# grantsrb/PyTorch-A2C

Measured on AMD Instinct MI355X. Metric: env-steps/sec (rollout+update), higher is better.
Workload: dtype f32

## Files before the change

### include/a2c_mi355x.h

```cpp
#ifndef A2C_MI355X_H
#define A2C_MI355X_H

#include <stddef.h>
#include <stdint.h>

#ifdef __cplusplus
extern "C" {
#endif

#define A2C_OK 0
#define A2C_ERR_ARG (-1)
#define A2C_ERR_LAUNCH (-2)
#define A2C_ERR_WORKSPACE (-3)

typedef void *a2c_stream_t;

int a2c_version(void);
const char *a2c_error_string(int code);

int a2c_discount_scan(const float *x, const float *dones, float *y, int64_t n_seg,
                      int64_t T, float g, int *err_flag, a2c_stream_t stream);
int a2c_gae_returns_fused(const float *deltas, const float *rewards, const float *dones,
                          float *advs, float *rets, int64_t n_seg, int64_t T, float g_adv,
                          float g_ret, int *err_flag, a2c_stream_t stream);
// ... 76 lines not shown
typedef struct {
  int B, C, H, W, n_actions;
  const float *prev; int64_t prev_stride;
  const float *frame_new;
  const float *reset_mask;
  float *out; int64_t out_stride;
  const float *wfrag1, *bias1, *wfrag2, *bias2, *Wc, *bc;
  float *heads; int64_t ldh;
  const float *u;
  int64_t *actions; int64_t act_stride;
  const float *rew, *done;
  float *val_prev, *rewards, *dones, *deltas;
  int64_t T, t_rec, slot0;
  float gamma;
  int pong, bootstrap;
  const uint8_t *frame_u8;
  int64_t frame_stride;
  float *a1_out; int64_t a1_stride;
  float *a2_out; int64_t a2_stride;
  float *heads_out; int64_t heads_out_stride;
} a2c_a3c_step_args;
int a2c_a3c_step_supported(int C, int H, int W, int n_actions);
int a2c_a3c_step(const a2c_a3c_step_args *args, a2c_stream_t stream);

typedef struct {
  int B, C, H, W, n_actions;
  float *states;
  float *bookmark;
  const float *wfrag1, *bias1, *wfrag2, *bias2, *Wc, *bc;
  float *heads; int64_t ldh;
  const float *u; int64_t u_stride;
  int64_t *actions;
  float *val_prev, *rewards, *dones, *deltas;
  int64_t T, slot0;
  float gamma;
  int pong;
  uint64_t *cmd;
  const uint64_t *rec;
  const uint8_t *frames; int64_t frame_stride;
  uint32_t seq0;
  int env0;
  int *err;
  int64_t timeout_ticks;
  float *a1_rows, *a2_rows;
  float *heads_rows; int64_t heads_rows_ld;
  uint8_t *frame_store; int64_t frame_store_slot_stride;
  int32_t *nvalid_rows, *nvalid_carry;
  int frame_bits;
  const float *conv1_weight;
  int states_lazy;
  const uint8_t *tagged; int64_t tagged_stride; int tagged_chunks;
  uint64_t *a1_lanemask_rows;
  uint8_t *a2_maskbit_rows;
} a2c_a3c_rollout_args;
int a2c_a3c_rollout(const a2c_a3c_rollout_args *args, a2c_stream_t stream);
int a2c_a3c_ring_supported(int B, int C, int H, int W, int n_actions, const float *conv1_weight);

int a2c_rollout_buffer_create(const char *shm_name, size_t bytes, void **host_out, void **dev_out);
int a2c_rollout_buffer_destroy(const char *shm_name, void *host, size_t bytes);
int a2c_pinned_register(void *host, size_t bytes, void **dev_out);
int a2c_pinned_unregister(void *host);
int a2c_push_buffer_alloc(size_t bytes, void **ptr_out);
int a2c_push_buffer_free(void *ptr);
int a2c_set_blocking_sync(int on);
int a2c_device_pci_bus_id(char *out, int len);
int a2c_store_u32_system(uint32_t *dev_ptr, uint32_t value, a2c_stream_t stream);
int a2c_memcpy_async(void *dst, const void *src, size_t bytes, int kind, a2c_stream_t stream);
int a2c_copy_rows(const float *src, int64_t src_stride, float *dst, int64_t dst_stride, int B,
                  int64_t n, a2c_stream_t stream);
int a2c_mask_rows(float *x, int64_t ld, const float *dones, int64_t done_stride, int B, int n,
                  a2c_stream_t stream);
int a2c_permute_rows(const float *src, float *dst, int64_t R, int64_t T, int64_t n,
                     a2c_stream_t stream);

int a2c_loss_fwd_bwd(const float *logits, int64_t ld_logits, const float *vals, int64_t val_stride,
                     const int64_t *actions, const float *advs, const float *returns,
                     const double *adv_sums, int64_t n_local, int64_t n_global, int A,
                     float pi_coef, float val_coef, float entr_coef, float *dlogits, int64_t ldd,
                     float *dvals, int64_t dval_stride, double *loss_sums, double *reduce_scratch,
                     a2c_stream_t stream);

#define A2C_GAUSS_MAX_N 64
int a2c_gauss_head(const float *heads, int64_t ld_heads, const float *eps, int64_t ld_eps, float *sigma,
                   int64_t ld_sigma, float *actions, int64_t ld_act, int64_t B, int n, a2c_stream_t stream);
int a2c_gauss_loss_sums(const float *heads, int64_t ld_heads, const float *vals, int64_t val_stride,
                        const float *actions, int64_t ld_act, const float *advs, const float *returns,
                        const double *adv_sums, int64_t n_local, int64_t n_global, int n, double *sums,
                        double *reduce_scratch, a2c_stream_t stream);
int a2c_gauss_loss_fwd_bwd(const float *heads, int64_t ld_heads, const float *vals, int64_t val_stride,
                           const float *actions, int64_t ld_act, const float *advs, const float *returns,
                           const double *adv_sums, const double *sums, int64_t n_local, int64_t n_global, int n,
                           float pi_coef, float val_coef, float entr_coef, float *dheads, int64_t ldd, float *dvals,
                           int64_t dval_stride, double *loss_sums, a2c_stream_t stream);

size_t a2c_gemm_ws_bytes(int64_t M, int64_t N, int splitk);
size_t a2c_gemm_x9_ws_bytes(int64_t M, int64_t N, int64_t K);
int a2c_gemm_f32(int transA, int transB, int64_t M, int64_t N, int64_t K, const float *A,
                 int64_t lda, const float *B, int64_t ldb, float *C, int64_t ldc,
                 const float *bias, int relu, const float *mask, int64_t ldmask, int accumulate,
                 int splitk, void *ws, size_t ws_bytes, a2c_stream_t stream);
size_t a2c_gemm_x6_image_bytes(int64_t rows, int64_t K);
int a2c_gemm_x6_split(const float *src, int64_t ld, int64_t rows, int64_t K, int k_contiguous, void *image,
                      a2c_stream_t stream);
int a2c_gemm_x6_images(int64_t M, int64_t N, int64_t K, const void *image_a, const void *image_b, float *C, int64_t ldc,
                       const float *bias, int relu, const float *mask, int64_t ldmask, int accumulate, int splitk, void *ws,
                       size_t ws_bytes, a2c_stream_t stream);
// ... 9 lines not shown
                    const float *W, const float *b, float *heads, int64_t ldh, int64_t M, int N,
                    int K, const float *u, int n_logits, int64_t *actions, int64_t act_stride,
                    a2c_stream_t stream);
int a2c_heads_fused_publish(const float *xs, int nslab, int64_t slab_stride, int64_t ldx,
                            const float *bias_in, int relu_in, float *emb_out, int64_t ld_emb,
                            const float *W, const float *b, float *heads, int64_t ldh, int64_t M,
                            int N, int K, const float *u, int n_logits, int64_t *actions,
                            int64_t act_stride, uint64_t *cmd, const uint32_t *seq_base,
                            uint32_t seq_off, a2c_stream_t stream);
int a2c_gemm_f32_nt(int64_t M, int64_t N, int64_t K, const float *A, int64_t lda, const float *B,
                    int64_t ldb, float *C, int64_t ldc, const float *bias, int relu,
                    a2c_stream_t stream);
int a2c_gemm_f32_nn(int64_t M, int64_t N, int64_t K, const float *A, int64_t lda, const float *B,
                    int64_t ldb, float *C, int64_t ldc, const float *mask, int64_t ldmask,
                    a2c_stream_t stream);
int a2c_gemm_f32_tn(int64_t M, int64_t N, int64_t K, const float *A, int64_t lda, const float *B,
                    int64_t ldb, float *C, int64_t ldc, int splitk, void *ws, size_t ws_bytes,
                    a2c_stream_t stream);
int a2c_compose_heads(const float *Wh, const float *bh, const float *Wp, const float *bp, float *Wc,
                      float *bc, int N, int H, int F, a2c_stream_t stream);
size_t a2c_colsum_ws_bytes(int64_t N);
int a2c_colsum(const float *x, int64_t ld, int64_t M, int64_t N, float *out, void *ws,
               size_t ws_bytes, a2c_stream_t stream);

typedef struct {
  int Cin, H, W;
  int Cout, ks, stride, pad;
  int OH, OW;
} a2c_conv_desc;
size_t a2c_conv2d_prep_floats(const a2c_conv_desc *d, int kind);
int a2c_conv2d_prep_weights(const a2c_conv_desc *d, int kind, const float *weight, float *wprep,
                            a2c_stream_t stream);
int a2c_conv2d_fwd(const a2c_conv_desc *d, const float *in, int64_t in_bstride,
                   const float *wprep_fwd, const float *bias, int relu, float *out,
                   int64_t out_bstride, int B, a2c_stream_t stream);
int a2c_conv2d_bwd_data(const a2c_conv_desc *d, const float *dout, const float *wprep_bwd,
                        const float *mask, float *din, int B, a2c_stream_t stream);
int64_t a2c_conv2d_sign_words(const a2c_conv_desc *d);
int a2c_conv2d_fwd_signs(const a2c_conv_desc *d, const float *in, int64_t in_bstride, const float *wprep_fwd,
                         const float *bias, int relu, float *out, int64_t out_bstride, uint32_t *signs,
                         int64_t signs_bstride, int B, a2c_stream_t stream);
int a2c_conv2d_bwd_data_signs_supported(const a2c_conv_desc *d);
int a2c_lanemask_from_act(const float *act, uint64_t *lanemask, int64_t n_floats, a2c_stream_t stream);
int a2c_conv2d_bwd_data_lanemask_supported(const a2c_conv_desc *d, int B);
int a2c_conv2d_bwd_data_lanemask(const a2c_conv_desc *d, const float *dout, const float *wprep_bwd, const uint64_t *lanemask,
                                 float *din, int B, a2c_stream_t stream);
int a2c_conv2d_bwd_rank_supported(const a2c_conv_desc *d, int n_logits, int B);
int a2c_conv2d_bwd_data_lanemask_rank(const a2c_conv_desc *d, const float *dl, int64_t ld_dl, int n_logits, const float *Wc,
                                      const uint8_t *maskbits, int64_t mask_row_bytes, const float *wprep_bwd,
                                      const uint64_t *lanemask, float *din, int B, a2c_stream_t stream);
int a2c_conv2d_bwd_weight_rank(const a2c_conv_desc *d, const float *in, int64_t in_bstride, const float *dl, int64_t ld_dl,
                               int n_logits, const float *Wc, const uint8_t *maskbits, int64_t mask_row_bytes, float *dW,
                               float *db, int B, void *ws, size_t ws_bytes, a2c_stream_t stream);
int a2c_conv2d_bwd_data_signs(const a2c_conv_desc *d, const float *dout, const float *wprep_bwd, const uint32_t *signs,
                              int64_t signs_bstride, float *din, int B, a2c_stream_t stream);
size_t a2c_conv2d_bwd_data_w1_frames_ws_bytes(const a2c_conv_desc *d2, const a2c_conv_desc *d1, int B);
int a2c_conv2d_bwd_data_w1_frames(const a2c_conv_desc *d2, const float *dout, const float *wprep_bwd, const uint32_t *signs,
                                  int64_t signs_bstride, const a2c_conv_desc *d1, const uint8_t *frame_store,
                                  int64_t slot_stride, int64_t T, const int32_t *nvalid, float *dW1, float *db1, int B,
                                  void *ws, size_t ws_bytes, a2c_stream_t stream);
size_t a2c_conv2d_bwd_data_w1_ws_bytes(const a2c_conv_desc *d2, const a2c_conv_desc *d1, int B);
int a2c_conv2d_bwd_data_w1(const a2c_conv_desc *d2, const float *dout, const float *wprep_bwd,
                           const float *mask, const a2c_conv_desc *d1, const float *x, int64_t x_bstride,
                           float *dW1, float *db1, int B, void *ws, size_t ws_bytes, a2c_stream_t stream);
size_t a2c_conv2d_bwd_weight_ws_bytes(const a2c_conv_desc *d, int B);
int a2c_conv2d_bwd_weight(const a2c_conv_desc *d, const float *in, int64_t in_bstride,
                          const float *dout, float *dW, float *db, int B, void *ws,
                          size_t ws_bytes, a2c_stream_t stream);
int a2c_conv2d_bwd_weight_frames(const a2c_conv_desc *d, const uint8_t *frame_store, int64_t slot_stride,
                                 int64_t T, const int32_t *nvalid, const float *dout, float *dW,
                                 float *db, int B, void *ws, size_t ws_bytes, a2c_stream_t stream);
#define A2C_CONV_CHAIN_MAX 8
int a2c_conv2d_fwd_chain_supported(const a2c_conv_desc *d, int n_layers);
int a2c_conv2d_fwd_chain(const a2c_conv_desc *d, int n_layers, const float *in, int64_t in_bstride,
                         const float *const *wprep_fwd, const float *const *bias, int relu, float *const *out,
                         const int64_t *out_bstride, uint32_t *const *signs, const int64_t *signs_bstride, int B,
                         a2c_stream_t stream);
int a2c_conv2d_fwd_frames_supported(const a2c_conv_desc *d);
int a2c_conv2d_fwd_frames(const a2c_conv_desc *d, const uint8_t *frame_store, int64_t sample_stride, int64_t T,
                          const int32_t *nvalid, int64_t nvalid_stride, const float *wprep_fwd, const float *bias,
                          int relu, float *out, int64_t out_bstride, uint32_t *signs, int64_t signs_bstride, int B,
                          a2c_stream_t stream);

int a2c_gru_gates(const float *gx, const float *gh, const float *b, const float *h, float *z,
                  float *r, float *rh, int B, int hdim, a2c_stream_t stream);
int a2c_gru_out(const float *gx, const float *rh_u, const float *b, const float *h,
                const float *z, float *c, float *h_new, int B, int hdim, a2c_stream_t stream);
int a2c_gru_cell_fwd(const float *x, int64_t ldx, const float *h, const float *WxC, const float *WhC,
                     const float *Wh2, const float *b, float *gx, float *z, float *r, float *rh, float *c,
                     float *h_new, int B, int xs, int hdim, a2c_stream_t stream);
int a2c_gru_out_bwd(const float *dh_new, const float *h, const float *z, const float *c,
                    float *dc_pre, float *dz, float *dh, int B, int hdim, a2c_stream_t stream);
int a2c_gru_out_bwd_carry(const float *dh_new, const float *carry, const float *dones, int64_t done_stride,
                          const float *h, const float *z, const float *c, float *dc_pre, float *dz, float *dh,
                          int B, int hdim, a2c_stream_t stream);
int a2c_gru_gates_bwd(const float *d_rh, const float *dz, const float *h, const float *z,
                      const float *r, float *dz_pre, float *dr_pre, float *dh, int B, int hdim,
                      a2c_stream_t stream);
int a2c_gru_cell_bwd(const float *dh_new, const float *carry, const float *dones, int64_t done_stride,
                     const float *h, const float *z, const float *r, const float *c, const float *Wh,
                     float *dc_pre, float *dz, float *dz_pre, float *dr_pre, float *dh, int B, int hdim,
                     a2c_stream_t stream);
int a2c_layernorm_fwd(const float *x, const float *w, const float *b, float *y, float *mean,
                      float *rstd, int64_t rows, int n, a2c_stream_t stream);
int a2c_layernorm_bwd(const float *dy, const float *x, const float *w, const float *mean,
                      const float *rstd, float *dx, float *dw_rows, int64_t rows, int n,
// ... 50 lines not shown
```

### pytorch-a2c_amd/a2c_amd/_lib.py

```python
import ctypes
import os
from ctypes import POINTER, Structure, c_char_p, c_double, c_float, c_int, c_int64, c_size_t, c_uint32, c_void_p

_HERE = os.path.dirname(os.path.abspath(__file__))
LIB_PATH = os.path.join(_HERE, "liba2c_mi355x.so")


class ConvDesc(Structure):
    _fields_ = [("Cin", c_int), ("H", c_int), ("W", c_int), ("Cout", c_int), ("ks", c_int),
                ("stride", c_int), ("pad", c_int), ("OH", c_int), ("OW", c_int)]


P = c_void_p
PD = POINTER(ConvDesc)


class A3CStepArgs(Structure):
    _fields_ = [("B", c_int), ("C", c_int), ("H", c_int), ("W", c_int), ("n_actions", c_int),
                ("prev", P), ("prev_stride", c_int64), ("frame_new", P), ("reset_mask", P),
                ("out", P), ("out_stride", c_int64),
                ("wfrag1", P), ("bias1", P), ("wfrag2", P), ("bias2", P), ("Wc", P), ("bc", P),
                ("heads", P), ("ldh", c_int64), ("u", P), ("actions", P), ("act_stride", c_int64),
                ("rew", P), ("done", P), ("val_prev", P), ("rewards", P), ("dones", P), ("deltas", P),
                ("T", c_int64), ("t_rec", c_int64), ("slot0", c_int64), ("gamma", c_float),
                ("pong", c_int), ("bootstrap", c_int), ("frame_u8", P), ("frame_stride", c_int64),
                ("a1_out", P), ("a1_stride", c_int64), ("a2_out", P), ("a2_stride", c_int64),
                ("heads_out", P), ("heads_out_stride", c_int64)]


class A3CRolloutArgs(Structure):
    _fields_ = [("B", c_int), ("C", c_int), ("H", c_int), ("W", c_int), ("n_actions", c_int),
                ("states", P), ("bookmark", P),
                ("wfrag1", P), ("bias1", P), ("wfrag2", P), ("bias2", P), ("Wc", P), ("bc", P),
                ("heads", P), ("ldh", c_int64), ("u", P), ("u_stride", c_int64), ("actions", P),
                ("val_prev", P), ("rewards", P), ("dones", P), ("deltas", P),
                ("T", c_int64), ("slot0", c_int64), ("gamma", c_float), ("pong", c_int),
                ("cmd", P), ("rec", P), ("frames", P), ("frame_stride", c_int64),
                ("seq0", c_uint32), ("env0", c_int), ("err", P), ("timeout_ticks", c_int64), ("a1_rows", P), ("a2_rows", P), ("heads_rows", P), ("heads_rows_ld", c_int64),
                ("frame_store", P), ("frame_store_slot_stride", c_int64), ("nvalid_rows", P), ("nvalid_carry", P),
                ("frame_bits", c_int), ("conv1_weight", P), ("states_lazy", c_int),
                ("tagged", P), ("tagged_stride", c_int64), ("tagged_chunks", c_int), ("a1_lanemask_rows", P),
                ("a2_maskbit_rows", P)]


PS = POINTER(A3CStepArgs)
PR = POINTER(A3CRolloutArgs)

SIGNATURES = {
    "a2c_version": (c_int, []),
    "a2c_error_string": (c_char_p, [c_int]),
    "a2c_discount_scan": (c_int, [P, P, P, c_int64, c_int64, c_float, P, P]),
    "a2c_gae_returns_fused": (c_int, [P, P, P, P, P, c_int64, c_int64, c_float, c_float, P, P]),
    "a2c_moments": (c_int, [P, c_int64, P, P, P]),
    "a2c_normalize": (c_int, [P, P, c_int64, P, c_int64, c_float, P]),
    "a2c_add": (c_int, [P, P, P, c_int64, P]),
    "a2c_frame_stack_push": (c_int, [P, P, P, c_int64, P, c_int64, c_int, c_int, c_int, P]),
    "a2c_frame_stack_push_u8": (c_int, [P, c_int64, P, P, c_int64, P, c_int64, c_int, c_int, c_int, P]),
    "a2c_pool_publish_actions": (c_int, [P, P, c_int64, c_int, P, ctypes.c_uint32, P]),
    "a2c_pool_ingest": (c_int, [P, P, c_int64, c_int, c_int, P, ctypes.c_uint32, c_int64, P, P, P, P, c_int64, P]),
    "a2c_pool_ingest_bits": (c_int, [P, P, c_int64, c_int, c_int, P, ctypes.c_uint32, c_int64, P, P, P, P, c_int64, P]),
    "a2c_unpack_bits": (c_int, [P, c_int64, P, c_int64, c_int, c_int, P]),
    "a2c_pool_ingest_post": (c_int, [c_int, P, P, c_int64, c_int, c_int, P, ctypes.c_uint32, c_int64, P, P, P, P, c_int64,
                                     P, c_int64, P, P, P, P, c_int64, c_int64, c_int64, c_float, c_int, P, P, c_int, P, c_int64, P,
                                     P, P, P]),
    "a2c_store_u32_system": (c_int, [P, ctypes.c_uint32, P]),
    "a2c_softmax_sample": (c_int, [P, c_int64, P, P, c_int64, P, c_int, c_int, P]),
    "a2c_sample_probs": (c_int, [P, P, P, c_int64, c_int, P]),
    "a2c_rollout_record": (c_int, [P, P, P, c_int64, P, P, P, P, P, P, c_int, c_int, c_int64, c_int64, c_int64,
                                    c_float, c_int, P]),
    "a2c_rollout_post": (c_int, [P, P, P, c_int64, P, P, P, P, c_int64, c_int64, c_int64, c_float, c_int, P, P, P, c_int64,
                                  P, c_int64, c_int, c_int, c_int, P]),
    "a2c_rollout_post_rec": (c_int, [P, P, P, c_int64, P, P, P, P, c_int64, c_int64, c_int64, c_float, c_int, P, P, c_int64, P, P,
                             c_int64, P, c_int64, c_int, c_int, c_int, P, P, c_int, P, c_int64, P, P]),
    "a2c_rollout_post_u8": (c_int, [P, P, P, c_int64, P, P, P, P, c_int64, c_int64, c_int64, c_float, c_int, P, c_int64, P, P,
                                     c_int64, P, c_int64, c_int, c_int, c_int, P]),
    "a2c_rollout_bootstrap": (c_int, [P, c_int64, P, P, P, P, c_int, c_int64, c_int64, c_float, P]),
    "a2c_copy_rows": (c_int, [P, c_int64, P, c_int64, c_int, c_int64, P]),
    "a2c_mask_rows": (c_int, [P, c_int64, P, c_int64, c_int, c_int, P]),
    "a2c_permute_rows": (c_int, [P, P, c_int64, c_int64, c_int64, P]),
    "a2c_loss_fwd_bwd": (c_int, [P, c_int64, P, c_int64, P, P, P, P, c_int64, c_int64, c_int, c_float, c_float,
                                  c_float, P, c_int64, P, c_int64, P, P, P]),
    "a2c_gauss_head": (c_int, [P, c_int64, P, c_int64, P, c_int64, P, c_int64, c_int64, c_int, P]),
    "a2c_gauss_loss_sums": (c_int, [P, c_int64, P, c_int64, P, c_int64, P, P, P, c_int64, c_int64, c_int, P, P, P]),
    "a2c_gauss_loss_fwd_bwd": (c_int, [P, c_int64, P, c_int64, P, c_int64, P, P, P, P, c_int64, c_int64, c_int, c_float,
                                        c_float, c_float, P, c_int64, P, c_int64, P, P]),
    "a2c_gemm_ws_bytes": (c_size_t, [c_int64, c_int64, c_int]),
    "a2c_gemm_x9_ws_bytes": (c_size_t, [c_int64, c_int64, c_int64]),
    "a2c_gemm_x6_image_bytes": (c_size_t, [c_int64, c_int64]),
    "a2c_gemm_x6_split": (c_int, [P, c_int64, c_int64, c_int64, c_int, P, P]),
    "a2c_gemm_x6_images": (c_int, [c_int64, c_int64, c_int64, P, P, P, c_int64, P, c_int, P, c_int64, c_int, c_int, P, c_size_t, P]),
    "a2c_gemm_f32": (c_int, [c_int, c_int, c_int64, c_int64, c_int64, P, c_int64, P, c_int64, P, c_int64,
                              P, c_int, P, c_int64, c_int, c_int, P, c_size_t, P]),
    "a2c_gemm_splits": (c_int, [c_int64, c_int]),
    "a2c_small_n_bwd_data_bits": (c_int, [P, c_int64, P, P, c_int64, P, c_int64, c_int64, c_int, c_int64, P]),
    "a2c_gemm_f32_partial": (c_int, [c_int, c_int, c_int64, c_int64, c_int64, P, c_int64, P, c_int64, c_int, P, c_size_t, P]),
    "a2c_heads_fused": (c_int, [P, c_int, c_int64, c_int64, P, c_int, P, c_int64, P, P, P, c_int64, c_int64, c_int, c_int,
                                 P, c_int, P, c_int64, P]),
    "a2c_heads_fused_publish": (c_int, [P, c_int, c_int64, c_int64, P, c_int, P, c_int64, P, P, P, c_int64, c_int64, c_int, c_int,
                                         P, c_int, P, c_int64, P, P, ctypes.c_uint32, P]),
    "a2c_gemm_f32_nt": (c_int, [c_int64, c_int64, c_int64, P, c_int64, P, c_int64, P, c_int64, P, c_int, P]),
    "a2c_gemm_f32_nn": (c_int, [c_int64, c_int64, c_int64, P, c_int64, P, c_int64, P, c_int64, P, c_int64, P]),
    "a2c_gemm_f32_tn": (c_int, [c_int64, c_int64, c_int64, P, c_int64, P, c_int64, P, c_int64, c_int, P,
                                 c_size_t, P]),
    "a2c_colsum_ws_bytes": (c_size_t, [c_int64]),
    "a2c_colsum": (c_int, [P, c_int64, c_int64, c_int64, P, P, c_size_t, P]),
    "a2c_conv2d_prep_floats": (c_size_t, [PD, c_int]),
    "a2c_compose_heads": (c_int, [P, P, P, P, P, P, c_int, c_int, c_int, P]),
    "a2c_a3c_step_supported": (c_int, [c_int, c_int, c_int, c_int]),
    "a2c_a3c_ring_supported": (c_int, [c_int, c_int, c_int, c_int, c_int, c_void_p]),
    "a2c_a3c_step": (c_int, [PS, P]),
    "a2c_a3c_rollout": (c_int, [PR, P]),
    "a2c_rollout_buffer_create": (c_int, [c_char_p, c_size_t, POINTER(c_void_p), POINTER(c_void_p)]),
    "a2c_rollout_buffer_destroy": (c_int, [c_char_p, P, c_size_t]),
    "a2c_pinned_register": (c_int, [P, c_size_t, POINTER(c_void_p)]),
    "a2c_pinned_unregister": (c_int, [P]),
    "a2c_push_buffer_alloc": (c_int, [c_size_t, POINTER(c_void_p)]),
    "a2c_push_buffer_free": (c_int, [P]),
    "a2c_memcpy_async": (c_int, [P, P, c_size_t, c_int, P]),
    "a2c_device_pci_bus_id": (c_int, [c_char_p, c_int]),
    "a2c_set_blocking_sync": (c_int, [c_int]),
    "a2c_pack_update_scalars": (c_int, [P, P, P, P, P]),
    "a2c_conv2d_prep_weights": (c_int, [PD, c_int, P, P, P]),
    "a2c_conv2d_fwd": (c_int, [PD, P, c_int64, P, P, c_int, P, c_int64, c_int, P]),
    "a2c_conv2d_bwd_data": (c_int, [PD, P, P, P, P, c_int, P]),
    "a2c_conv2d_sign_words": (c_int64, [PD]),
    "a2c_conv2d_fwd_signs": (c_int, [PD, P, c_int64, P, P, c_int, P, c_int64, P, c_int64, c_int, P]),
    "a2c_conv2d_bwd_data_signs_supported": (c_int, [PD]),
    "a2c_conv2d_bwd_data_w1_frames_ws_bytes": (c_size_t, [PD, PD, c_int]),
    "a2c_conv2d_bwd_data_w1_frames": (c_int, [PD, P, P, P, c_int64, PD, P, c_int64, c_int64, P, P, P, c_int, P, c_size_t, P]),
    "a2c_lanemask_from_act": (c_int, [P, P, c_int64, P]),
    "a2c_conv2d_bwd_data_lanemask_supported": (c_int, [PD, c_int]),
    "a2c_conv2d_bwd_rank_supported": (c_int, [PD, c_int, c_int]),
    "a2c_conv2d_bwd_data_lanemask_rank": (c_int, [PD, P, c_int64, c_int, P, P, c_int64, P, P, P, c_int, P]),
    "a2c_conv2d_bwd_weight_rank": (c_int, [PD, P, c_int64, P, c_int64, c_int, P, P, c_int64, P, P, c_int, P, c_size_t, P]),
    "a2c_conv2d_bwd_data_lanemask": (c_int, [PD, P, P, P, P, c_int, P]),
    "a2c_conv2d_bwd_data_signs": (c_int, [PD, P, P, P, c_int64, P, c_int, P]),
    "a2c_conv2d_bwd_weight_ws_bytes": (c_size_t, [PD, c_int]),
    "a2c_conv2d_bwd_data_w1_ws_bytes": (c_size_t, [PD, PD, c_int]),
    "a2c_conv2d_bwd_data_w1": (c_int, [PD, P, P, P, PD, P, c_int64, P, P, c_int, P, c_size_t, P]),
    "a2c_conv2d_bwd_weight": (c_int, [PD, P, c_int64, P, P, P, c_int, P, c_size_t, P]),
    "a2c_conv2d_bwd_weight_frames": (c_int, [PD, P, c_int64, c_int64, P, P, P, P, c_int, P, c_size_t, P]),
    "a2c_conv2d_fwd_frames_supported": (c_int, [PD]),
    "a2c_conv2d_fwd_chain_supported": (c_int, [PD, c_int]),
    "a2c_conv2d_fwd_chain": (c_int, [PD, c_int, P, c_int64, P, P, c_int, P, P, P, P, c_int, P]),
    "a2c_conv2d_fwd_frames": (c_int, [PD, P, c_int64, c_int64, P, c_int64, P, P, c_int, P, c_int64, P, c_int64, c_int, P]),
    "a2c_frame_prep_u8": (c_int, [P, c_int64, c_int, c_int, c_int, c_int, c_int, c_int, c_int, c_int, c_int, P, c_int64, c_int, P]),
    "a2c_frame_store_begin": (c_int, [P, c_int64, c_int64, c_int, c_int, P, P, c_int, P]),
    "a2c_rollout_post_frames": (c_int, [P, P, P, c_int64, P, P, P, P, c_int64, c_int64, c_int64, c_float, c_int, c_int, P, P,
                                        c_int, P, c_int64, P, P, P, P]),
    "a2c_frames_to_states": (c_int, [P, c_int64, P, c_int64, P, c_int64, c_int, c_int, c_int, c_int, P]),
    "a2c_gru_gates": (c_int, [P, P, P, P, P, P, P, c_int, c_int, P]),
    "a2c_gru_out": (c_int, [P, P, P, P, P, P, P, c_int, c_int, P]),
    "a2c_gru_cell_bwd": (c_int, [P, P, P, c_int64, P, P, P, P, P, P, P, P, P, P, c_int, c_int, P]),
    "a2c_gru_cell_fwd": (c_int, [P, c_int64, P, P, P, P, P, P, P, P, P, P, P, c_int, c_int, c_int, P]),
    "a2c_gru_out_bwd": (c_int, [P, P, P, P, P, P, P, c_int, c_int, P]),
    "a2c_gru_out_bwd_carry": (c_int, [P, P, P, c_int64, P, P, P, P, P, P, c_int, c_int, P]),
    "a2c_gru_gates_bwd": (c_int, [P, P, P, P, P, P, P, P, c_int, c_int, P]),
    "a2c_layernorm_fwd": (c_int, [P, P, P, P, P, P, c_int64, c_int, P]),
    "a2c_layernorm_bwd": (c_int, [P, P, P, P, P, P, P, c_int64, c_int, c_int, P]),
    "a2c_gradnorm_sq": (c_int, [P, c_int64, P, P, P]),
    "a2c_clip_rmsprop": (c_int, [P, P, P, c_int64, P, c_double, c_double, c_double, c_double, P, P]),
    "a2c_clip_adam": (c_int, [P, P, P, P, c_int64, P, c_double, c_double, c_double, c_double, c_double,
                               c_int64, P, P]),
    "a2c_clip_sgd": (c_int, [P, P, c_int64, P, c_double, c_double, P, P]),
    "a2c_clip_adagrad": (c_int, [P, P, P, c_int64, P, c_double, c_double, c_double, c_double, c_int64, P, P]),
    "a2c_clip_adadelta": (c_int, [P, P, P, P, c_int64, P, c_double, c_double, c_double, c_double, P, P]),
    "a2c_clip_rprop": (c_int, [P, P, P, P, c_int64, P, c_double, c_double, c_double, c_double, c_double, P, P]),
    "a2c_clip_adamw": (c_int, [P, P, P, P, c_int64, P, c_double, c_double, c_double, c_double, c_double, c_double,
                                c_int64, P, P]),
    "a2c_clip_adamax": (c_int, [P, P, P, P, c_int64, P, c_double, c_double, c_double, c_double, c_double, c_int64,
                                 P, P]),
    "a2c_clip_nadam": (c_int, [P, P, P, P, c_int64, P, c_double, c_double, c_double, c_double, c_double, c_double,
                                c_int64, c_double, P, P]),
    "a2c_clip_radam": (c_int, [P, P, P, P, c_int64, P, c_double, c_double, c_double, c_double, c_double, c_int64,
                                P, P]),
    "a2c_clip_asgd": (c_int, [P, P, P, c_int64, P, c_double, c_double, c_double, c_double, P, P]),
    "a2c_snake_state_bytes": (c_size_t, [c_int, c_int]),
    "a2c_snake_reset": (c_int, [P, c_int, c_int, c_uint32, c_int, c_int, c_int, P, P, P]),
    "a2c_snake_step": (c_int, [P, P, c_int64, c_int, c_int, c_int, c_uint32, c_int, c_int, c_int, P, P, P, P, P, P, P]),
}

_lib = None


class A2CKernelError(RuntimeError):
    pass

# ... 23 lines not shown
```

### pytorch-a2c_amd/a2c_amd/models.py

```python
import os

import numpy as np
import torch
import torch.nn as nn

from . import ops
from .engine import Arena, ConvLayer, linear_bwd_data, linear_bwd_weight, linear_fwd


def _conv_block(cin, cout, ks, stride, pad):
    return nn.Sequential(nn.Conv2d(cin, cout, ks, stride=stride, padding=pad), nn.ReLU())


def _sampler(sampler):
    return (*sampler[:3], sampler[3] if len(sampler) > 3 else None)


class _HipNet(nn.Module):

    is_recurrent = False
    _unused_params = ()
    _packed_after = ()

    def _post_init(self):
        self._arena = None
        self._ws = {}
        self._dirty = True
        self._saved = {}
        self._stash = None
        self._stash_frames = None

    def _arena_order(self):
        return [n for n, _ in self.named_parameters()]

    @property
    def _n_pi(self):
        return self.output_space if self.is_discrete else 2 * self.output_space

    def _ensure_device(self):
        if self._arena is not None:
            return
        if not torch.cuda.is_available():
            raise RuntimeError("a2c_amd models need a HIP device: there is no CPU fallback")
        named = dict(self.named_parameters())
        dev = torch.device("cuda", torch.cuda.current_device())
        for b_name, b in self.named_buffers():
            b.data = b.data.to(dev)
        order = self._arena_order()
        trainable = [n for n in order if n not in self._unused_params]
        self._arena = Arena([(n, named[n]) for n in order], set(trainable), dev, set(self._packed_after))
        self._dev = dev
        self._dirty = True
        self._bind_params()

    def _apply(self, fn, *a, **k):
        out = super()._apply(fn, *a, **k)
        self._arena = None
        self._ws = {}
        self.mark_dirty()
        return out

    def load_state_dict(self, *a, **k):
        out = super().load_state_dict(*a, **k)
        self.mark_dirty()
        return out

    def mark_dirty(self):
        self._dirty = True
        self._stash = None
        self._stash_frames = None
        self._stash_lm = False

    def _conv_chain(self):
        ch = getattr(self, "_chain", 0)
        if ch == 0:
            ch = None
            if len(self._cl) >= 2 and not any(l.padded for l in self._cl[1:]):
                c = ops.ConvChain([l.d for l in self._cl[1:]])
                ch = c if c.ok else None
            self._chain = ch
        if ch is not None and os.environ.get("A2C_NO_CHAIN") == "1":
            return None
        return ch

    def stash_rows(self, states, n_rows, T=None):
        return None

    def stash_commit(self, states, n_rows, frames=None):
        self._stash = (states.data_ptr(), int(n_rows))
        self._stash_frames = frames

    def _stash_valid(self, x_ptr, n_rows):
        return getattr(self, "_stash", None) == (x_ptr, int(n_rows))

    _ROUTE_SWITCHES = ("A2C_NO_STASH", "A2C_NO_LANEMASK", "A2C_NO_EMB_STASH", "A2C_NO_CELL_STASH", "A2C_NO_HEADS_STASH",
                       "A2C_NO_FRAME_STORE")

    def _route_state(self):
        return (self._stash, self._stash_frames, getattr(self, "_stash_lm", False), getattr(self, "_cells_done", None))

    def _set_route_state(self, rs):
        self._stash, self._stash_frames, self._stash_lm, cells = rs
        if cells is not None:
            self._cells_done = cells

    def _route_sig(self):
        st, fr, lm, cells = self._route_state()
        return (st, None if fr is None else (fr[0].data_ptr(), fr[1].data_ptr(), int(fr[2])), bool(lm), cells,
                tuple(os.environ.get(k) == "1" for k in self._ROUTE_SWITCHES))

    def _need_states(self):
        cb = getattr(self, "_materialize_states", None)
        if cb is not None:
            cb()

    def ws(self, tag):
        w = self._ws.get(tag)
        if w is None:
            w = self._ws[tag] = ops.Workspace(self._dev)
        return w

    def _refresh(self, st):
        if self._dirty:
            self._prep(st)
            self._dirty = False

    def _prep(self, st):
        pass

    def _prep_sig(self):
        return ""

    def P(self, name):
        return self._pd[name]

    def _bind_params(self):
        self._pd = dict(self.named_parameters())

    def G(self, name):
        return self._arena.grad(name)

    def req_grads(self, calc_bool):
        for p in self.parameters():
            p.requires_grad = calc_bool

    def check_grads(self):
        for p in self.parameters():
            if torch.sum(p.data != p.data) > 0:
                print("NaNs in Grad!")

    def _to_dev(self, t):
        self._ensure_device()
        return t.detach().to(device=self._dev, dtype=torch.float32).contiguous()

    def forward(self, x, old_h=None):
        self._ensure_device()
        need_grad = torch.is_grad_enabled() and any(p.requires_grad for p in self.parameters())
        xd = self._to_dev(x)
        hd = self._to_dev(old_h) if self.is_recurrent else None
        if self.is_recurrent and old_h is None:
            raise TypeError("recurrent model: forward(x, old_h)")
# ... 93 lines not shown
        self.input_space, self.output_space, self.h_size, self.is_discrete = input_space, output_space, h_size, True
        C, H, W = input_space[-3:]
        self.convs = nn.ModuleList([])
        self.conv1 = _conv_block(C, 16, 8, 4, 0)
        self.convs.append(self.conv1)
        self.conv2 = _conv_block(16, 32, 4, 2, 0)
        self.convs.append(self.conv2)
        self.features = nn.Sequential(*self.convs)
        self._c1 = ConvLayer(C, H, W, 16, 8, 4, 0, need_bwd_data=False, name="conv1")
        _, h1, w1 = self._c1.out_shape
        self._c2 = ConvLayer(16, h1, w1, 32, 4, 2, 0, need_bwd_data=True, name="conv2")
        self.flat_size = int(np.prod(self._c2.out_shape))
        self.proj_matrx = nn.Linear(self.flat_size, h_size)
        self.emb_bnorm = nn.BatchNorm1d(h_size)
        self.pi = nn.Linear(h_size, output_space)
        self.value = nn.Linear(h_size, 1)
        self._post_init()

    def _arena_order(self):
        return ["convs.0.0.weight", "convs.0.0.bias", "convs.1.0.weight", "convs.1.0.bias", "proj_matrx.weight",
                "proj_matrx.bias", "pi.weight", "value.weight", "pi.bias", "value.bias", "emb_bnorm.weight",
                "emb_bnorm.bias"]

    def _prep(self, st):
        with ops.side_branch(1):
            self._c1.prep(self.P("convs.0.0.weight"), ops.stream())
            self._c2.prep(self.P("convs.1.0.weight"), ops.stream())
        try:
            self._prep_heads(st)
        finally:
            ops.join_branches()

    def _prep_heads(self, st):
        A, h, F = self.output_space, self.h_size, self.flat_size
        ar = self._arena
        Wh = ar.params[ar.offsets["pi.weight"][0]:][:(A + 1) * h].view(A + 1, h)
        bh = ar.params[ar.offsets["pi.bias"][0]:][:A + 1]
        if A + 1 > 8:
            return
        if getattr(self, "_Wc", None) is None:
            self._Wc = torch.empty(A + 1, F, device=self._dev)
            self._bc = torch.empty(A + 1, device=self._dev)
        ops.compose_heads(Wh, bh, self.P("proj_matrx.weight").data, self.P("proj_matrx.bias").data, self._Wc, self._bc, st)

    @property
    def _fused_sampling(self):
        return self.output_space + 1 <= 8

    def stash_rows(self, states, n_rows, T=None):
        if os.environ.get("A2C_NO_STASH") == "1" or not self._step_supported():
            return None
        ws = self.ws("train")
        return (ws.get("a1", (n_rows,) + self._c1.out_shape), ws.get("a2", (n_rows,) + self._c2.out_shape),
                self._heads("train", n_rows)[0], self._a1_lanemask_rows(n_rows), self._a2_maskbit_rows(n_rows))

    def _a2_maskbit_rows(self, n_rows):
        F = self.flat_size
        if os.environ.get("A2C_NO_LANEMASK") == "1" or F % 8 or self.output_space + 1 > 8:
            return None
        return self.ws("train").get("a2_mb", (n_rows, F // 8), dtype=torch.uint8)

    def _a1_lanemask_rows(self, n_rows):
        n = int(np.prod(self._c1.out_shape))
        if os.environ.get("A2C_NO_LANEMASK") == "1" or n % 256 or not ops.conv_bwd_data_lanemask_supported(self._c2.d, n_rows):
            return None
        return self.ws("train").get("a1_lm", (n_rows, n // 64), dtype=torch.int64)

    def stash_commit(self, states, n_rows, frames=None, lanemask=False):
        super().stash_commit(states, n_rows, frames=frames)
        self._stash_lm = bool(lanemask)

    def _fwd(self, x_ptr, bstride, B, tag, st, save, sampler=None):
        ws, P = self.ws(tag), self.P
        A, h = self.output_space, self.h_size
        a1 = ws.get("a1", (B,) + self._c1.out_shape)
        a2 = ws.get("a2", (B,) + self._c2.out_shape)
        emb = ws.get("emb", (B, h))
        stashed = save and tag == "train" and self._stash_valid(x_ptr, B)
        hb, logits, vals = self._heads(tag, B)
        self._emb_free = False
        self._bwd_frames = self._stash_frames if (stashed and os.environ.get("A2C_NO_FRAME_STORE") != "1") else None
        if stashed and os.environ.get("A2C_NO_HEADS_STASH") != "1":
            self._emb_free = True
            return dict(logits=logits, vals=vals, sampled=False)
        if not stashed:
            if save and tag == "train":
                self._need_states()
            self._c1.fwd(x_ptr, bstride, P("convs.0.0.bias"), a1, B, st)
            self._c2.fwd(a1.data_ptr(), a1[0].numel(), P("convs.1.0.bias"), a2, B, st)
        Wh = self._arena.params[self._arena.offsets["pi.weight"][0]:][:(A + 1) * h].view(A + 1, h)
        bh = self._arena.params[self._arena.offsets["pi.bias"][0]:][:A + 1]
        u, a_ptr, a_stride, pub = _sampler(sampler) if sampler is not None else (None, 0, 0, None)
        if A + 1 > 8:
            linear_fwd(ws, a2.data_ptr(), self.flat_size, P("proj_matrx.weight"), P("proj_matrx.bias"), emb, B, st)
            linear_fwd(ws, emb.data_ptr(), h, Wh, bh, hb, B, st)
            return dict(logits=logits, vals=vals, sampled=False)
        if sampler is not None and not save and os.environ.get("A2C_NO_COMPOSED_HEADS") != "1":
            ops.heads_fused(a2.data_ptr(), 1, 0, self.flat_size, None, False, None, self._Wc, self._bc, hb, B, u, A,
                            a_ptr, a_stride, st, publish=pub)
            return dict(logits=logits, vals=vals, sampled=True, published=pub is not None)
        Wp = P("proj_matrx.weight")
        sk = ops.pick_splitk(B, h, self.flat_size)
        if sk > 1 and os.environ.get("A2C_NO_FUSED_TAIL") != "1":
            buf = ws.bytes("gemm_ws", ops.gemm_ws_bytes(B, h, sk))
            with ops.span(f"linear.fwd {h}x{self.flat_size}"):
                nslab = ops.gemm_partial(0, 1, B, h, self.flat_size, a2.data_ptr(), self.flat_size, Wp.data_ptr(),
                                         self.flat_size, sk, buf, st)
            ops.heads_fused(buf.data_ptr(), nslab, B * h, h, P("proj_matrx.bias"), False, emb, Wh, bh, hb, B, u, A,
                            a_ptr, a_stride, st, publish=pub if u is not None else None)
        else:
            linear_fwd(ws, a2.data_ptr(), self.flat_size, Wp, P("proj_matrx.bias"), emb, B, st)
            if u is None:
                linear_fwd(ws, emb.data_ptr(), h, Wh, bh, hb, B, st)
            else:
                ops.heads_fused(emb.data_ptr(), 1, 0, h, None, False, None, Wh, bh, hb, B, u, A, a_ptr, a_stride, st, publish=pub)
        return dict(logits=logits, vals=vals, sampled=u is not None, published=u is not None and pub is not None)

    def _step_supported(self):
        if os.environ.get("A2C_NO_FUSED_STEP") == "1" or os.environ.get("A2C_NO_COMPOSED_HEADS") == "1":
            return False
        C, H, W = self.input_space[-3:]
        return self.output_space + 1 <= 8 and ops.a3c_step_supported(C, H, W, self.output_space)

# ... 19 lines not shown
        dbh = ar.grads[ar.offsets["pi.bias"][0]:][:A + 1]
        F = self.flat_size
        Wp = P("proj_matrx.weight")
        emb_free = getattr(self, "_emb_free", False)
        rank_bwd = A + 1 <= 8 and getattr(self, "_Wc", None) is not None and os.environ.get("A2C_NO_RANK_BWD") != "1"
        da2 = ws.get("da2", (B,) + self._c2.out_shape)

        def head_grads(st):
            if emb_free or rank_bwd:
                S = ws.get("dWh_S", (A + 1, F))
                linear_bwd_weight(ws, db, a2.data_ptr(), F, S, dbh if emb_free else None, B, st)
            if emb_free:
                nch = next(n for n in range(max(1, -(-F // 1024)), F + 1) if F % n == 0 and (F // n) % 8 == 0)
                Kc = F // nch
                for c in range(nch):
                    ops.gemm(0, 1, A + 1, h, Kc, S.data_ptr() + 4 * c * Kc, F, Wp.data_ptr() + 4 * c * Kc, F, dWh.data_ptr(), h,
                             accumulate=(c > 0), st=st)
                ops.gemm(0, 0, A + 1, h, 1, dbh.data_ptr(), 1, P("proj_matrx.bias").data_ptr(), h, dWh.data_ptr(), h,
                         accumulate=True, st=st)
            else:
                linear_bwd_weight(ws, db, emb.data_ptr(), h, dWh, dbh, B, st)
            if rank_bwd:
                Wpi, dWp = P("pi.weight"), G("proj_matrx.weight")
                with ops.span("rank_bwd proj_matrx grads"):
                    ops.gemm(1, 0, h, F, A, Wpi.data_ptr(), h, S.data_ptr(), F, dWp.data_ptr(), F, st=st)
                    ops.gemm(1, 0, h, 1, A, Wpi.data_ptr(), h, dbh.data_ptr(), 1, G("proj_matrx.bias").data_ptr(), 1, st=st)

        fuse_da2, mb = False, None
        try:
            if rank_bwd:
                with ops.side_branch(0):
                    head_grads(ops.stream())
                mb = None
                if (tag == "train" and getattr(self, "_stash_lm", False) and self._stash_valid(x_ptr, B)
                        and os.environ.get("A2C_NO_LANEMASK") != "1"):
                    mb = self._a2_maskbit_rows(B)
                fuse_da2 = (mb is not None and os.environ.get("A2C_NO_RANK_FUSE") != "1" and a1[0].numel() % 4 == 0
                            and ops.conv_bwd_rank_supported(self._c2.d, A, B))
                if not fuse_da2:
                    with ops.span("rank_bwd da2"):
                        if mb is not None:
                            ops.small_n_bwd_data_bits(dl, dl.stride(0), self._Wc, da2, F, mb, B, A, F, st)
                        else:
                            ops.gemm(0, 0, B, F, A, dl.data_ptr(), dl.stride(0), self._Wc.data_ptr(), F, da2.data_ptr(), F,
                                     mask_ptr=a2.data_ptr(), ldmask=F, st=st)
            else:
                head_grads(st)
                demb = ws.get("demb", (B, h))
                linear_bwd_data(ws, db, P("pi.weight"), demb, B, st, n_cols=A)
                linear_bwd_weight(ws, demb, a2.data_ptr(), F, G("proj_matrx.weight"), G("proj_matrx.bias"), B, st)
                linear_bwd_data(ws, demb, Wp, da2.view(B, -1), B, st, mask=a2)
            if fuse_da2:
                buf = ws.bytes("conv_wgrad_ws", ops.conv_bwd_weight_ws_bytes(self._c2.d, B))
                with ops.span("conv2.bwd_weight"):
                    ops.conv_bwd_weight_rank(self._c2.d, a1.data_ptr(), a1[0].numel(), dl, dl.stride(0), A, self._Wc, mb, mb.stride(0),
                                             G("convs.1.0.weight"), G("convs.1.0.bias"), B, buf, st)
            else:
                self._c2.bwd_weight(a1.data_ptr(), a1[0].numel(), da2, G("convs.1.0.weight"), G("convs.1.0.bias"), B, ws, st)
            da1 = ws.get("da1", (B,) + self._c1.out_shape)
            lm = None
            if tag == "train" and getattr(self, "_stash_lm", False) and self._stash_valid(x_ptr, B) and os.environ.get("A2C_NO_LANEMASK") != "1":
                lm = self._a1_lanemask_rows(B)
            if fuse_da2 and lm is not None:
                with ops.span("conv2.bwd_data"):
                    ops.conv_bwd_data_lanemask_rank(self._c2.d, dl, dl.stride(0), A, self._Wc, mb, mb.stride(0), self._c2.wb, lm, da1, B, st)
            else:
                if fuse_da2:
                    ops.small_n_bwd_data_bits(dl, dl.stride(0), self._Wc, da2, F, mb, B, A, F, st)
                self._c2.bwd_data(da2, a1, da1, B, st, lanemask=lm)
            fr = getattr(self, "_bwd_frames", None)
            if fr is not None:
                fstore, nvalid, T = fr
                buf = ws.bytes("conv_wgrad_ws", ops.conv_bwd_weight_ws_bytes(self._c1.d, B))
                with ops.span("conv1.bwd_weight"):
                    ops.conv_bwd_weight_frames(self._c1.d, fstore, fstore.stride(0), T, nvalid, da1, G("convs.0.0.weight"),
                                               G("convs.0.0.bias"), B, buf, st)
            else:
                if tag == "train":
                    self._need_states()
                self._c1.bwd_weight(x_ptr, bstride, da1, G("convs.0.0.weight"), G("convs.0.0.bias"), B, ws, st)
        finally:
            ops.join_branches()


def h_is_lockstep(stash, B, R, T):
    return B == R and stash[2] == T and 0 <= stash[1] < T


class _ConvStackNet(_HipNet):

    def _build_convs(self, input_space, specs):
        C, H, W = input_space[-3:]
        self.convs = nn.ModuleList([])
        self._cl = []
        for i, (co, ks, s, p) in enumerate(specs):
            self.convs.append(_conv_block(C, co, ks, s, p))
            layer = ConvLayer(C, H, W, co, ks, s, p, need_bwd_data=(i > 0), name=f"conv{i+1}")
            self._cl.append(layer)
            C, H, W = layer.out_shape
        self.features = nn.Sequential(*self.convs)
        self.flat_size = C * H * W

    def _prep(self, st):
        for i, l in enumerate(self._cl):
            l.prep(self.P(f"convs.{i}.0.weight"), st)
        if hasattr(self, "gru"):
            self._gru_prep(st)

    def _sign_layers(self):
# ... 802 lines not shown
```

### pytorch-a2c_amd/a2c_amd/ops.py

```python
import ctypes
import os

import torch

from . import _lib
from ._lib import ConvDesc, check

_F32 = torch.float32


def lib():
    if _TORCH_ABI_ON():
        return torch_abi()
    return _lib.load()


def _TORCH_ABI_ON():
    import os
    return os.environ.get("A2C_TORCH_OPS") == "1"


class TorchAbi:

    def __init__(self):
# ... 772 lines not shown
                                             st if st is not None else stream()), "a2c_conv2d_bwd_data_lanemask")


def conv_bwd_data_w1_frames_ws_bytes(d2, d1, B):
    return lib().a2c_conv2d_bwd_data_w1_frames_ws_bytes(ctypes.byref(d2), ctypes.byref(d1), B)


def conv_bwd_data_w1_frames(d2, dout, wprep_bwd, signs, d1, fstore, slot_stride, T, nvalid, dW1, db1, B, ws, st=None):
    _chk(fstore, "frame_store", torch.uint8); _chk(nvalid, "nvalid", torch.int32); _chk(signs, "signs", torch.int32)
    check(lib().a2c_conv2d_bwd_data_w1_frames(ctypes.byref(d2), _p(dout), _p(wprep_bwd), _p(signs), signs.stride(0), ctypes.byref(d1),
                                              _p(fstore), slot_stride, T, _p(nvalid), _p(dW1), _p(db1), B, ws.data_ptr(),
                                              ws.numel() * ws.element_size(), st if st is not None else stream()),
          "a2c_conv2d_bwd_data_w1_frames")


def conv_bwd_weight_ws_bytes(d, B):
    return lib().a2c_conv2d_bwd_weight_ws_bytes(ctypes.byref(d), B)


def conv_bwd_data_w1_ws_bytes(d2, d1, B):
    return lib().a2c_conv2d_bwd_data_w1_ws_bytes(ctypes.byref(d2), ctypes.byref(d1), B)


def conv_bwd_data_w1(d2, dout, wprep_bwd, mask, d1, x_ptr, x_bstride, dW1, db1, B, ws, st=None):
    check(lib().a2c_conv2d_bwd_data_w1(ctypes.byref(d2), _p(dout), _p(wprep_bwd), _p(mask), ctypes.byref(d1), x_ptr,
                                       x_bstride, _p(dW1), _p(db1), B, ws.data_ptr(), ws.numel() * ws.element_size(),
                                       st if st is not None else stream()), "a2c_conv2d_bwd_data_w1")


def conv_bwd_weight(d, in_ptr, in_bstride, dout, dW, db, B, ws, st=None):
    check(lib().a2c_conv2d_bwd_weight(ctypes.byref(d), in_ptr, in_bstride, _p(dout), _p(dW), _p(db), B,
                                      ws.data_ptr(), ws.numel() * ws.element_size(),
                                      st if st is not None else stream()), "a2c_conv2d_bwd_weight")


def conv_bwd_rank_supported(d, n_logits, B):
    return bool(lib().a2c_conv2d_bwd_rank_supported(ctypes.byref(d), n_logits, B))


def conv_bwd_data_lanemask_rank(d, dl, ld_dl, n_logits, Wc, maskbits, mask_row_bytes, wprep_bwd, lanemask, din, B, st=None):
    _chk(maskbits, "maskbits", torch.uint8); _chk(lanemask, "lanemask", torch.int64)
    check(lib().a2c_conv2d_bwd_data_lanemask_rank(ctypes.byref(d), _p(dl), ld_dl, n_logits, _p(Wc), _p(maskbits), mask_row_bytes,
                                                  _p(wprep_bwd), _p(lanemask), _p(din), B, st if st is not None else stream()),
          "a2c_conv2d_bwd_data_lanemask_rank")


def conv_bwd_weight_rank(d, in_ptr, in_bstride, dl, ld_dl, n_logits, Wc, maskbits, mask_row_bytes, dW, db, B, ws, st=None):
    _chk(maskbits, "maskbits", torch.uint8)
    check(lib().a2c_conv2d_bwd_weight_rank(ctypes.byref(d), in_ptr, in_bstride, _p(dl), ld_dl, n_logits, _p(Wc), _p(maskbits),
                                           mask_row_bytes, _p(dW), _p(db), B, ws.data_ptr(), ws.numel() * ws.element_size(),
                                           st if st is not None else stream()), "a2c_conv2d_bwd_weight_rank")


def conv_bwd_weight_frames(d, fstore, slot_stride, T, nvalid, dout, dW, db, B, ws, st=None):
    _chk(fstore, "frame_store", torch.uint8); _chk(nvalid, "nvalid", torch.int32)
    check(lib().a2c_conv2d_bwd_weight_frames(ctypes.byref(d), _p(fstore), slot_stride, T, _p(nvalid), _p(dout), _p(dW), _p(db),
                                             B, ws.data_ptr(), ws.numel() * ws.element_size(),
                                             st if st is not None else stream()), "a2c_conv2d_bwd_weight_frames")


def conv_fwd_frames_supported(d):
    return bool(lib().a2c_conv2d_fwd_frames_supported(ctypes.byref(d)))


def conv_fwd_frames(d, fstore_ptr, sample_stride, T, nvalid_ptr, nvalid_stride, wprep, bias, relu, out, B, st=None,
                    out_bstride=None, signs=None):
    out_ptr = out if isinstance(out, int) else _p(out)
    sg, sgs = signs if signs is not None else (0, 0)
    check(lib().a2c_conv2d_fwd_frames(ctypes.byref(d), fstore_ptr, sample_stride, T, nvalid_ptr, nvalid_stride, _p(wprep), _p(bias),
                                      int(bool(relu)), out_ptr, d.Cout * d.OH * d.OW if out_bstride is None else out_bstride,
                                      sg, sgs, B, st if st is not None else stream()), "a2c_conv2d_fwd_frames")


class ConvChain:

    def __init__(self, descs):
        n = len(descs)
        self.n = n
        self.descs = (ConvDesc * n)(*descs)
        self.ok = bool(lib().a2c_conv2d_fwd_chain_supported(self.descs, n))
        self.wprep, self.bias, self.out = (ctypes.c_void_p * n)(), (ctypes.c_void_p * n)(), (ctypes.c_void_p * n)()
        self.obs, self.sg, self.sgs = (ctypes.c_int64 * n)(), (ctypes.c_void_p * n)(), (ctypes.c_int64 * n)()

    def fwd(self, in_ptr, in_bstride, wpreps, biases, outs, out_bstrides, B, st=None, relu=True, signs=None):
        for i in range(self.n):
            self.wprep[i], self.bias[i], self.out[i], self.obs[i] = _p(wpreps[i]), _p(biases[i]), outs[i], out_bstrides[i]
            self.sg[i], self.sgs[i] = (signs or {}).get(i, (0, 0))
        check(lib().a2c_conv2d_fwd_chain(self.descs, self.n, in_ptr, in_bstride, self.wprep, self.bias, int(bool(relu)), self.out,
                                         self.obs, self.sg, self.sgs, B, st if st is not None else stream()), "a2c_conv2d_fwd_chain")


PREP_SPECS = {"pong_prep": (35, 195, 0, None, 2, 1), "breakout_prep": (35, 195, 8, -8, 2, 0)}


def prep_out_shape(name, H, W):
    y0, y1, x0, x1, step, _ = PREP_SPECS[name]
    x1 = W if x1 is None else (W + x1 if x1 < 0 else x1)
    return (1, (y1 - y0 + step - 1) // step, (x1 - x0 + step - 1) // step)


def frame_prep_u8(name, raw_ptr, raw_stride, H, W, C, out_ptr, out_stride, n, st=None):
    y0, y1, x0, x1, step, binarise = PREP_SPECS[name]
    x1 = W if x1 is None else (W + x1 if x1 < 0 else x1)
    check(lib().a2c_frame_prep_u8(raw_ptr, raw_stride, H, W, C, y0, y1, x0, x1, step, binarise, out_ptr, out_stride, n,
                                  st if st is not None else stream()), "a2c_frame_prep_u8")

# ... 167 lines not shown
```

### pytorch-a2c_amd/a2c_amd/runner.py

```python
import os
import queue
import warnings
import time
from collections import deque

import numpy as np
import torch
import torch.nn.functional as F

from . import ops
from .utils import cuda_if, next_state, sample_action, try_key


class SequentialEnvironment:

    def __init__(self, env_type, preprocessor, seed=time.time(), float_params=dict(), env_fn=None, **kwargs):
        self.env_type, self.preprocessor, self.seed, self.float_params = env_type, preprocessor, seed, float_params
        if env_fn is not None:
            self.env = env_fn()
        else:
            try:
                import gym
                self.env = gym.make(env_type)
                self.env.seed(self.seed)
# ... 202 lines not shown
                    idxs.append(tok)
                self.rollout(net, sorted(idxs), self.hyps)
                self.finish()
                for i in idxs:
                    self.stop_q.put(i)
                if stop:
                    return
        except BaseException as e:
            self.error = e
            for _ in range(int(try_key(self.hyps, "n_rollouts", 1))):
                try:
                    self.stop_q.put_nowait(None)
                except Exception:
                    break
            raise

    def finish(self):
        torch.cuda.current_stream().synchronize()
        if getattr(self, "proc_pool", False):
            if not (self.env_pool.dev_phase and self.datas["actions"].is_cuda):
                self.env_pool.set_phase(0)
            self.check()
            if self.rew_q is not None:
                self.rew_q.get()
                self.rew_q.put(self.env_pool.rew_ema())
        elif getattr(self, "device_pool", False) and self.rew_q is not None and hasattr(self.env_pool, "episode_stats"):
            k, total = self.env_pool.episode_stats()
            if k:
                self.rew_q.put(.99 ** k * self.rew_q.get() + (1 - .99 ** k) * total / k)

    def check(self):
        if getattr(self, "proc_pool", False) and int(self.rollout_err.item()):
            self.env_pool._check_workers()
            raise TimeoutError("a2c_a3c_rollout: an env worker did not answer within the time-out")

    def close(self):
        if getattr(self, "proc_pool", False):
            self.env_pool.close()

    def rollout(self, net, idx, hyps):
        if not self._ready:
            self.start(net)
        idxs = [idx] if isinstance(idx, int) else list(idx)
        N = self.datas["states"].shape[0]
        T_ = int(hyps["n_tsteps"])
        if getattr(self, "_states_stale", False):
            if idxs == list(range(N // T_)):
                self._states_stale = False
            else:
                self.materialize_states()
        net._stash = None
        net._stash_frames = None
        net._stash_lm = False
        self._lm_written = False
        if hasattr(net, "_cells_done"):
            net._cells_done = -1
        self._stash_bufs = None
        self._frames_written = None
        if idxs == list(range(N // T_)) and N % T_ == 0:
            self._stash_bufs = net.stash_rows(self.datas["states"], N, T=T_)
        stash_all = self._stash_bufs is not None
        seqs = self.env_pool.seq_env if self.proc_pool else None
        dev_phase = self.env_pool.dev_phase if (self.proc_pool and self.datas["actions"].is_cuda) else 0
        if dev_phase:
            ops.store_u32_system(dev_phase, 1)
        elif self.proc_pool:
            self.env_pool.set_phase(1)
        try:
            for r0 in range(0, len(idxs), self.B):
                rnd = idxs[r0:r0 + self.B]
                j = 0
                while j < len(rnd):
                    k = j
                    while k + 1 < len(rnd) and rnd[k + 1] == rnd[k] + 1 and (seqs is None or seqs[k + 1] == seqs[j]):
                        k += 1
                    self._rollout_block(net, rnd[j], j, k - j + 1, hyps)
                    stash_all = stash_all and self._stash_used
                    if self.proc_pool:
                        self.env_pool.advance(j, k - j + 1, T_)
                    j = k + 1
        except BaseException:
            if self.proc_pool:
                try:
                    self.env_pool.set_phase(0)
                except Exception:
                    pass
            raise
        if dev_phase:
            ops.store_u32_system(dev_phase, 0)
        if stash_all:
            if getattr(self, "_lm_written", False):
                net.stash_commit(self.datas["states"], N, frames=getattr(self, "_frames_written", None), lanemask=True)
            else:
                net.stash_commit(self.datas["states"], N, frames=getattr(self, "_frames_written", None))

    def _uniforms(self, t, B, env0):
        if self.uniform_fn is not None:
            return self.uniform_fn(t, B, env0)
        return torch.rand(B, device=self.net._dev, dtype=torch.float32)

    def _normals(self, t, B, env0):
        if self.normal_fn is not None:
            return self.normal_fn(t, B, env0).reshape(B, self.n_act)
        return torch.randn((B, self.n_act), device=self.net._dev, dtype=torch.float32)

    def _act_row(self, slot0, T, t):
        if self.cont:
            n = self.n_act
            return self.datas["actions"].data_ptr() + 4 * n * (slot0 * T + t), T * n
        return self.datas["actions"].data_ptr() + 8 * (slot0 * T + t), T

    def _sample(self, net, logits, u, eps, a_ptr, a_stride, B, st):
        if self.cont:
            ops.gauss_head(logits, self.n_act, B, eps=eps, actions_ptr=a_ptr, act_ld=a_stride, st=st)
        else:
            ops.softmax_sample(logits, u, a_ptr, a_stride, B, net.output_space, st=st)

    def _env_action(self, na_j, shift):
        if self.cont:
            return na_j + np.float32(shift)
        return int(na_j) + shift

    def _forward(self, net, x_ptr, bstride, B, env0, st, sampler=None, stash=None):
        kw = dict(stash=stash) if (stash is not None and isinstance(stash[0], list)) else {}
        if sampler is not None and getattr(net, "_fused_sampling", False):
            kw["sampler"] = sampler
        if net.is_recurrent:
            return net._fwd(x_ptr, bstride, B, "roll", st, False, h_in=self.h[env0:env0 + B], **kw)
        return net._fwd(x_ptr, bstride, B, "roll", st, False, **kw)

    def _zero_copy_ok(self, net):
        if not self.proc_pool or self.h is not None or self.ingest in ("memcpy", "relay") or getattr(self, "dev_prep", None):
            return False
        ok = (getattr(net, "_step_supported", lambda: False)() and self.u8 and self.HW % 16 == 0 and self.HW <= 8192
              and self.env_pool.dev_ptr != 0)
        if self.ingest == "zero-copy" and not ok:
            raise ValueError("ingest='zero-copy' needs an A3CModel-shaped net (a2c_a3c_step_supported) and a registered "
                             "process env pool with uint8 frames")
        return ok

    def _rollout_block(self, net, slot0, env0, B, hyps):
        D, pool = self.datas, self.env_pool
        T, S, C, HW = int(hyps["n_tsteps"]), self.S, self.C, self.HW
        gamma = hyps["gamma"]
        pong = "Pong" in hyps["env_type"]
# ... 419 lines not shown

    def _host_env_step(self, pool, env0, B, t, slot0, T, shift, acts_host_out, pong):
        na = self.np_act[env0:env0 + B]
        if acts_host_out is not None:
            acts_host_out[slot0 * T + t:(slot0 + B) * T:T] = self.h_act[env0:env0 + B]
        if self.proc_pool:
            k = pool.seq_of(env0, B) + t
            pool.post_actions(na, env0=env0, seq=k)
            pool.wait_frames(k + 1, env0=env0, n=B, timeout=float(try_key(self.hyps, "env_timeout_s", 20.0)))
            pool.unpack(self.np_rew[env0:env0 + B], self.np_done[env0:env0 + B], env0=env0)
            return
        nf, nr, nd = (x[env0:env0 + B] for x in (self.np_frames, self.np_rew, self.np_done))
        for j in range(B):
            obs, rew, done = pool.step(env0 + j, self._env_action(na[j], shift))
            self.ep_rew[env0 + j] += rew
            reset = done
            if pong and rew != 0:
                done = True
            if done and self.rew_q is not None:
                self.rew_q.put(.99 * self.rew_q.get() + .01 * self.ep_rew[env0 + j])
            if done:
                self.ep_rew[env0 + j] = 0
            if reset:
                obs = pool.reset(env0 + j)
            nf[j] = np.asarray(obs, dtype=np.float32).reshape(-1)
            nr[j], nd[j] = rew, float(reset)

    def _rollout_block_persistent(self, net, slot0, env0, B, hyps, bm, val_prev, acts_host_out, st):
        D, pool = self.datas, self.env_pool
        T, S = int(hyps["n_tsteps"]), self.S
        dev = net._dev
        if self.uniform_fn is not None:
            u = torch.stack([self.uniform_fn(t, B, env0).reshape(B) for t in range(T)]).contiguous()
        else:
            u = torch.rand((T, B), device=dev, dtype=torch.float32)
        ops._chk(u, "uniforms")
        if acts_host_out is None:
            acts = D["actions"]
        else:
            if getattr(self, "_acts_dev", None) is None or self._acts_dev.numel() != D["actions"].numel():
                self._acts_dev = torch.zeros(D["actions"].numel(), dtype=torch.int64, device=dev)
            acts = self._acts_dev
        C, H, W = net.input_space[-3:]
        hb, _, _ = net._heads("roll", self.B)
        hb = hb[env0:env0 + B]
        P = net.P
        self._u_keep = u
        timeout_s = float(try_key(hyps, "env_timeout_s", 20.0))
        fs = self._frame_store(T, D["states"].shape[0] // T, dev)
        ring = ops.a3c_ring_supported(B, C, H, W, net.output_space, P("convs.0.0.weight").data_ptr())
        lazy = fs is not None and bool(try_key(hyps, "lazy_states", False)) and ring
        lm = self._stash_bufs[3] if (ring and self._stash_bufs is not None and len(self._stash_bufs) > 3) else None
        mb = self._stash_bufs[4] if (lm is not None and len(self._stash_bufs) > 4) else None
        ops.a3c_rollout(st, B=B, C=C, H=H, W=W, n_actions=net.output_space, states=D["states"].data_ptr(),
                        bookmark=bm.data_ptr(), wfrag1=net._c1.wf.data_ptr(), bias1=P("convs.0.0.bias").data_ptr(),
                        wfrag2=net._c2.wf.data_ptr(), bias2=P("convs.1.0.bias").data_ptr(), Wc=net._Wc.data_ptr(),
                        bc=net._bc.data_ptr(), heads=hb.data_ptr(), ldh=hb.stride(0), u=u.data_ptr(), u_stride=B,
                        actions=acts.data_ptr(), val_prev=val_prev.data_ptr(), rewards=D["rewards"].data_ptr(),
                        dones=D["dones"].data_ptr(), deltas=D["deltas"].data_ptr(), T=T, slot0=slot0,
                        gamma=float(hyps["gamma"]), pong=int("Pong" in hyps["env_type"]), cmd=pool.dev_cmd, rec=pool.dev_rec,
                        frames=pool.dev_frames, frame_stride=self.fstride, frame_bits=int(self.bits),
                        conv1_weight=P("convs.0.0.weight").data_ptr(),
                        seq0=pool.seq_of(env0, B) & 0xffffffff, env0=env0,
                        err=self.rollout_err.data_ptr(), timeout_ticks=int(timeout_s * 1e8),
                        a1_rows=0 if self._stash_bufs is None else self._stash_bufs[0].data_ptr(),
                        a2_rows=0 if self._stash_bufs is None else self._stash_bufs[1].data_ptr(),
                        heads_rows=0 if self._stash_bufs is None else self._stash_bufs[2].data_ptr(),
                        heads_rows_ld=0 if self._stash_bufs is None else self._stash_bufs[2].stride(0),
                        frame_store=0 if fs is None else fs[0].data_ptr(),
                        frame_store_slot_stride=0 if fs is None else fs[0].stride(0),
                        nvalid_rows=0 if fs is None else fs[1].data_ptr(),
                        nvalid_carry=0 if fs is None else fs[2][env0:env0 + B].data_ptr(), states_lazy=int(lazy),
                        tagged=getattr(pool, "dev_tagged", 0), tagged_stride=int(pool.header.tagged_stride),
                        tagged_chunks=int(pool.header.tagged_chunks), a1_lanemask_rows=0 if lm is None else lm.data_ptr(),
                        a2_maskbit_rows=0 if mb is None else mb.data_ptr())
        self._lm_written = (lm is not None) and (getattr(self, "_lm_written", False) or slot0 == 0)
        if lazy:
            self._states_stale = True
            net._materialize_states = self.materialize_states
        if fs is not None and self._stash_bufs is not None:
            self._frames_written = (fs[0], fs[1], T)
        self._stash_used = self._stash_bufs is not None
        if acts_host_out is not None:
            acts_host_out[slot0 * T:(slot0 + B) * T].copy_(acts[slot0 * T:(slot0 + B) * T])

    def materialize_states(self):
        if not getattr(self, "_states_stale", False):
            return
        F_, nv_rows, _ = self._fstore
        R, T = F_.shape[0], F_.shape[1] - 4
        st = self.datas["states"]
        ops.frames_to_states(F_.data_ptr(), F_.stride(0), nv_rows.data_ptr(), T, st.data_ptr(), T * self.S, R, T, self.C, self.HW)
        self._states_stale = False

    def _frame_store(self, T, R, dev):
        on = os.environ.get("A2C_FRAME_STORE") == "1" or bool(try_key(self.hyps, "frame_store", False))
        if not on or os.environ.get("A2C_NO_FRAME_STORE") == "1" or T < 4 or self.HW % 16 or \
                not getattr(self, "_fstore_ok", True):
            return None
        fs = getattr(self, "_fstore", None)
        if fs is None:
            if (self.env_pool.seq_env != self.env_pool.seq_start).any() or R != self.B:
                self._fstore_ok = False
                return None
            F_ = torch.zeros((R, T + 4, self.HW), dtype=torch.uint8, device=dev)
            F_[:, T + 3] = self.d_frames[:, :self.HW]
            fs = self._fstore = (F_, torch.zeros(R * T, dtype=torch.int32, device=dev),
                                 torch.ones(self.B, dtype=torch.int32, device=dev))
        return fs

    def _env_step(self, pool, act, a_ptr, a_stride, env0, B, t, slot0, T, shift, acts_host_out, pong):
        if self.device_pool:
            if getattr(pool, "needs_actions", False):
                frames, rew, done, reset = pool.device_step(t, env0, B, actions=(a_ptr, a_stride))
                if acts_host_out is not None:
                    acts_host_out[slot0 * T + t:(slot0 + B) * T:T] = act.cpu()
            else:
                frames, rew, done, reset = pool.device_step(t, env0, B)
            ops._chk(frames, "frames")
            return _Frames(ptr32=frames.data_ptr()), rew, done, reset
        if self.proc_pool:
            return self._pool_step(pool, act, a_stride, env0, B, t, slot0, T, acts_host_out)
        return self._host_step(pool, act, a_ptr, a_stride, env0, B, t, slot0, T, shift, acts_host_out, pong)

    def _actions_to_host(self, act, a_stride, env0, B, t, slot0, T):
        ha = self.h_act[env0:env0 + B]
        if (not self.datas["actions"].is_cuda) if self.cont else a_stride == 1:
            ha.copy_(act, non_blocking=True)
# ... 200 lines not shown
```

### pytorch-a2c_amd/csrc/conv.hip

```cpp
#include <stdlib.h>
#include <algorithm>
#include <map>
#include <mutex>
#include "a2c_common.h"

bool c3_supported(const a2c_conv_desc* d, int kind);
size_t c3_prep_floats(const a2c_conv_desc* d, int kind);
int c3_prep(const a2c_conv_desc* d, int kind, const float* weight, float* out, hipStream_t st);
int c3_fwd(const a2c_conv_desc* d, const float* in, long in_bs, const float* frag, const float* bias, int relu, float* out,
           long out_bs, unsigned* signs, long signs_bs, int B, hipStream_t st);
int c3_bwd_data(const a2c_conv_desc* d, const float* dout, const float* frag, const float* mask, const unsigned* signs,
                long signs_bs, float* din, int B, hipStream_t st);
long c3_sign_words(const a2c_conv_desc* d);
bool c3_bwd_signs_supported(const a2c_conv_desc* d);
bool c3_bwd_mask_supported(const a2c_conv_desc* d);
bool c3w_supported(const a2c_conv_desc* d);
size_t c3w_ws_bytes(const a2c_conv_desc* d);
int c3w_bwd_weight(const a2c_conv_desc* d, const float* in, long in_bs, const float* dout, float* dW, float* db, int B, void* ws,
                   size_t ws_bytes, hipStream_t st);
bool c3_fwd_frames_supported(const a2c_conv_desc* d);
bool c3_chain_supported(const a2c_conv_desc* d, int n);
int c3_chain_fwd(const a2c_conv_desc* d, int n, const float* in, long in_bs, const float* const* frag, const float* const* bias,
                 int relu, float* const* out, const long* out_bs, unsigned* const* signs, const long* signs_bs, int B, hipStream_t st);
int c3_fwd_frames(const a2c_conv_desc* d, const unsigned char* f, long bs, long T, const int* nv, long nv_s, const float* frag,
// ... 2482 lines not shown
#pragma unroll
        for (int q = 0; q < RGW; ++q) {
          const float* src = brow + boff[q] + 4 * c4 * S;
          if (S == 4) {
            const float4 t = *reinterpret_cast<const float4*>(src);
            bv[c4][q][0] = t.x; bv[c4][q][1] = t.y; bv[c4][q][2] = t.z; bv[c4][q][3] = t.w;
          } else {
            const float2 t = *reinterpret_cast<const float2*>(src);
            bv[c4][q][0] = t.x; bv[c4][q][1] = t.y;
          }
        }
      }
#pragma unroll
      for (int c4 = 0; c4 < C4N; ++c4)
#pragma unroll
        for (int q = 0; q < RGW; ++q)
#pragma unroll
          for (int x = 0; x < S; ++x)
#pragma unroll
            for (int m = 0; m < MT; ++m)
              acc[m][q][x] = __builtin_amdgcn_mfma_f32_16x16x4f32(av[c4][m], bv[c4][q][x], acc[m][q][x], 0, 0, 0);
    }
  }
  float* sl = p.slab + (long)blockIdx.x * ((long)p.Cout * p.K + p.Cout);
#pragma unroll
  for (int m = 0; m < MT; ++m)
#pragma unroll
    for (int q = 0; q < RGW; ++q)
#pragma unroll
      for (int x = 0; x < S; ++x)
#pragma unroll
        for (int rr = 0; rr < 4; ++rr) {
          const int co = m * 16 + 4 * kk + rr;
          if (co < p.Cout) sl[(long)co * p.K + knat[q] + x] = acc[m][q][x][rr];
        }
  __syncthreads();
  float* red = lds;
  if (bpart < nparts) red[bpart * Cm + bco] = dbacc;
  __syncthreads();
  if (tid < p.Cout) {
    float s = 0.f;
    for (int q = 0; q < nparts; ++q) s += red[q * Cm + tid];
    sl[(long)p.Cout * p.K + tid] = s;
  }
}

namespace wx {
constexpr int NT = 512;
constexpr int SCR_A1 = 0, SCR_DO = 25600, SCR_BYTES = SCR_DO + 16384;
constexpr int P0 = 0, PQ = 15360, PBLK = 48;
constexpr int C2_0 = P0 + 3 * PQ, CQ = 4096, X2_0 = C2_0 + 3 * CQ;
constexpr int A_0 = X2_0 + 3 * CQ, AQ = 6656, AROW = 208;
constexpr int ZERO = A_0 + 3 * AQ, LDS_BYTES = ZERO + 32;
}
struct WgradX6P {
  const float* in; long in_bs; const float* dout; float* slab; int B;
  const float* dl; long ldl; int nlog; const float* Wc; const unsigned char* a2b; long a2b_row;
};
__device__ __forceinline__ void wx_split2(float a, float b, unsigned int o[3]) {
  const __bf16 a0 = (__bf16)a, b0 = (__bf16)b;
  const float ra = a - (float)a0, rb = b - (float)b0;
  const __bf16 a1 = (__bf16)ra, b1 = (__bf16)rb;
  const float sa = ra - (float)a1, sb = rb - (float)b1;
  const __bf16 a2 = (__bf16)sa, b2 = (__bf16)sb;
  o[0] = (unsigned int)__builtin_bit_cast(unsigned short, a0) | ((unsigned int)__builtin_bit_cast(unsigned short, b0) << 16);
  o[1] = (unsigned int)__builtin_bit_cast(unsigned short, a1) | ((unsigned int)__builtin_bit_cast(unsigned short, b1) << 16);
  o[2] = (unsigned int)__builtin_bit_cast(unsigned short, a2) | ((unsigned int)__builtin_bit_cast(unsigned short, b2) << 16);
}
template <bool RANK>
__global__ __launch_bounds__(wx::NT) void wgrad_x6_kernel(WgradX6P p) {
  using namespace wx;
  typedef const void __attribute__((address_space(1)))* gptr_t;
  typedef void __attribute__((address_space(3)))* lptr_t;
  __shared__ __attribute__((aligned(16))) unsigned char scrw[SCR_BYTES];
  extern __shared__ __attribute__((aligned(16))) unsigned char ldsw[];
  const int tid = threadIdx.x, lane = tid & 63, w = tid >> 6;
  const int l16 = lane & 15, g = lane >> 4;
  const int wq = w & 3, th = w >> 2;
  const float* __restrict__ sa1 = reinterpret_cast<const float*>(scrw + SCR_A1);
  const float* __restrict__ sdo = reinterpret_cast<const float*>(scrw + SCR_DO);
  for (int i = tid; i < LDS_BYTES / 16; i += NT) *reinterpret_cast<u32x4x*>(ldsw + i * 16) = (u32x4x){0u, 0u, 0u, 0u};
  int b0[2], b2[2], t0[2], t2[2], ncol[2];
  const int qs2 = g == 0 ? PQ : (g == 3 ? 0 : CQ);
#pragma unroll
  for (int tt = 0; tt < 2; ++tt) {
    const int ci = 2 * (2 * wq + th) + (l16 >> 3), ky = (l16 >> 1) & 3, kxl = l16 & 1;
    const int n = (ci * 4 + ky) * 4 + 2 * tt + kxl;
    ncol[tt] = n;
    b0[tt] = P0 + (ci * 20 + 2 * g + ky) * PBLK + 16 * kxl;
    b2[tt] = g == 0 ? P0 + (ci * 20 + 16 + ky) * PBLK + 16 * kxl : g == 1 ? C2_0 + n * 16 : g == 2 ? X2_0 + n * 16 : ZERO;
    t0[tt] = P0 + (ci * 20 + 2 * g + ky) * PBLK + 32 + 4 * kxl;
    t2[tt] = g == 0 ? P0 + (ci * 20 + 16 + ky) * PBLK + 32 + 4 * kxl : ZERO;
  }
  const int aaddr = A_0 + l16 * AROW + g * 16;
  f32x4 acc[2][2], acs[2][2];
#pragma unroll
  for (int mt = 0; mt < 2; ++mt)
#pragma unroll
    for (int tt = 0; tt < 2; ++tt) acc[mt][tt] = acs[mt][tt] = (f32x4){0.f, 0.f, 0.f, 0.f};
  float dbacc = 0.f;
  const int bco = tid & 31, bpart = tid >> 5;
  auto dma = [&](long b) {
    const float* __restrict__ ga = p.in + b * p.in_bs;
    const float* __restrict__ gd = p.dout + b * 2592L;
#pragma unroll
    for (int i = 0; i < 4; ++i) {
      if (i < 3 || w == 0)
        __builtin_amdgcn_global_load_lds((gptr_t)(ga + (long)(i * NT + tid) * 4), (lptr_t)(scrw + SCR_A1 + (i * NT + w * 64) * 16), 16, 0, 0);
    }
    if (!RANK) {
#pragma unroll
      for (int i = 0; i < 2; ++i) {
        const int c = min(i * NT + tid, 647);
        __builtin_amdgcn_global_load_lds((gptr_t)(gd + (long)c * 4), (lptr_t)(scrw + SCR_DO + (i * NT + w * 64) * 16), 16, 0, 0);
      }
    }
  };
  float wc[RANK ? 6 : 1][4], gl[4] = {0.f, 0.f, 0.f, 0.f};
  unsigned int mbv[RANK ? 6 : 1];
  if (RANK) {
#pragma unroll
    for (int j = 0; j < 6; ++j)
#pragma unroll
      for (int n = 0; n < 4; ++n) wc[RANK ? j : 0][n] = (tid + 512 * j < 2592 && n < p.nlog) ? p.Wc[(long)n * 2592 + tid + 512 * j] : 0.f;
  }
  auto raw = [&](long bn) {
#pragma unroll
    for (int n = 0; n < 4; ++n) gl[n] = n < p.nlog ? p.dl[bn * p.ldl + n] : 0.f;
#pragma unroll
    for (int j = 0; j < 6; ++j) mbv[RANK ? j : 0] = p.a2b[bn * p.a2b_row + (min(tid + 512 * j, 2591) >> 3)];
  };
  auto form = [&]() {
    float* __restrict__ dst = reinterpret_cast<float*>(scrw + SCR_DO);
#pragma unroll
    for (int j = 0; j < 6; ++j) {
      const int e = tid + 512 * j;
      float a = 0.f;
#pragma unroll
      for (int n = 0; n < 4; ++n) a += gl[n] * wc[RANK ? j : 0][n];
      if (!((mbv[RANK ? j : 0] >> (e & 7)) & 1u)) a = 0.f;
      if (e < 2592) dst[e] = a;
    }
  };
  auto half_row = [&](int h) {
    const int ci = h / 40, rem = h - ci * 40, y = rem >> 1, par = rem & 1;
    const float* __restrict__ row = sa1 + ci * 400 + y * 20 + par;
    unsigned int o[5][3];
#pragma unroll
    for (int i = 0; i < 5; ++i) wx_split2(row[4 * i], row[4 * i + 2], o[i]);
#pragma unroll
    for (int q = 0; q < 3; ++q) {
      unsigned char* dst = ldsw + P0 + q * PQ + (h >> 1) * PBLK;
      *reinterpret_cast<u32x4x*>(dst + 16 * par) = (u32x4x){o[0][q], o[1][q], o[2][q], o[3][q]};
      *reinterpret_cast<unsigned int*>(dst + 32 + 4 * par) = o[4][q];
    }
  };
  long b = blockIdx.x;
  if (RANK && b < p.B) {
    raw(b);
    form();
    raw(b + gridDim.x < p.B ? b + gridDim.x : b);
  }
  if (b < p.B) dma(b);
  for (; b < p.B; b += gridDim.x) {
    asm volatile("s_waitcnt vmcnt(0)" ::: "memory");
    __syncthreads();
    {
      half_row(tid);
      if (tid < 128) half_row(512 + tid);
      if (tid >= 256) {
        const int n = tid - 256, ci = n >> 4, ky = (n >> 2) & 3, kx = n & 3;
        const float* __restrict__ col = sa1 + ci * 400 + ky * 20 + 16 + kx;
        unsigned int o[4][3], oc[3];
#pragma unroll
        for (int i = 0; i < 4; ++i) wx_split2(col[80 * i], col[80 * i + 40], o[i]);
        wx_split2(col[320], 0.f, oc);
#pragma unroll
        for (int q = 0; q < 3; ++q) {
          *reinterpret_cast<u32x4x*>(ldsw + C2_0 + q * CQ + n * 16) = (u32x4x){o[0][q], o[1][q], o[2][q], o[3][q]};
          *reinterpret_cast<unsigned int*>(ldsw + X2_0 + q * CQ + n * 16) = oc[q];
        }
      }
    }
    if (tid >= 128 && tid < 480) {
      const int id = tid - 128, co = id / 11, gi = id - co * 11;
      const float* __restrict__ src = sdo + co * 81;
      float e[8];
#pragma unroll
      for (int i = 0; i < 8; ++i) {
        const int idx = gi < 9 ? gi * 9 + i : gi == 9 ? i * 9 + 8 : 80;
        e[i] = (gi == 10 && i > 0) ? 0.f : src[idx];
      }
      u32x4x o[3];
      bx_split8(e, o);
#pragma unroll
      for (int q = 0; q < 3; ++q) *reinterpret_cast<u32x4x*>(ldsw + A_0 + q * AQ + co * AROW + gi * 16) = o[q];
    }
    {
      const float* __restrict__ src = sdo + bco * 81;
      float s0 = 0.f;
      for (int i = bpart; i < 81; i += 16) s0 += src[i];
      dbacc += s0;
    }
    __syncthreads();
    if (RANK && b + gridDim.x < p.B) {
      form();
      const long b2 = b + 2L * gridDim.x;
      raw(b2 < p.B ? b2 : b);
    }
    if (b + gridDim.x < p.B) dma(b + gridDim.x);
#pragma unroll
    for (int s = 0; s < 3; ++s) {
      bf16x8x a[2][3], bf[2][3];
      u32x4x ra[2][3], rb[2][3];
      unsigned int rt[3] = {0u, 0u, 0u};
#pragma unroll
      for (int mt = 0; mt < 2; ++mt)
#pragma unroll
        for (int q = 0; q < 3; ++q)
          asm volatile("ds_read_b128 %0, %1" : "=v"(ra[mt][q]) : "v"((unsigned)(unsigned long)(lptr_t)(ldsw + aaddr + mt * 16 * AROW + s * 64 + q * AQ)));
#pragma unroll
      for (int tt = 0; tt < 2; ++tt) {
        const int base = s == 0 ? b0[tt] : s == 1 ? b0[tt] + 8 * PBLK : b2[tt];
        const int tail = s == 0 ? t0[tt] : s == 1 ? t0[tt] + 8 * PBLK : t2[tt];
        const int qs = s == 2 ? qs2 : PQ;
#pragma unroll
        for (int q = 0; q < 3; ++q) {
          asm volatile("ds_read_b128 %0, %1" : "=v"(rb[tt][q]) : "v"((unsigned)(unsigned long)(lptr_t)(ldsw + base + q * qs)));
          if (tt == 1) asm volatile("ds_read_b32 %0, %1" : "=v"(rt[q]) : "v"((unsigned)(unsigned long)(lptr_t)(ldsw + tail + q * qs)));
        }
      }
      asm volatile("s_waitcnt lgkmcnt(0)"
                   : "+v"(ra[0][0]), "+v"(ra[0][1]), "+v"(ra[0][2]), "+v"(ra[1][0]), "+v"(ra[1][1]), "+v"(ra[1][2]), "+v"(rb[0][0]), "+v"(rb[0][1]),
                     "+v"(rb[0][2]), "+v"(rb[1][0]), "+v"(rb[1][1]), "+v"(rb[1][2]), "+v"(rt[0]), "+v"(rt[1]), "+v"(rt[2])
                   :: "memory");
#pragma unroll
      for (int mt = 0; mt < 2; ++mt)
#pragma unroll
        for (int q = 0; q < 3; ++q) a[mt][q] = __builtin_bit_cast(bf16x8x, ra[mt][q]);
#pragma unroll
      for (int q = 0; q < 3; ++q) {
        bf[0][q] = __builtin_bit_cast(bf16x8x, rb[0][q]);
        u32x4x v = rb[1][q];
        const u32x4x sh = (u32x4x){__builtin_amdgcn_alignbit(v[1], v[0], 16), __builtin_amdgcn_alignbit(v[2], v[1], 16),
                                   __builtin_amdgcn_alignbit(v[3], v[2], 16), __builtin_amdgcn_alignbit(rt[q], v[3], 16)};
        if (s < 2 || g == 0) v = sh;
        bf[1][q] = __builtin_bit_cast(bf16x8x, v);
      }
#define WX_MM(AC, QA, QB)                                                                                               \
      _Pragma("unroll") for (int mt = 0; mt < 2; ++mt)                                                                  \
        _Pragma("unroll") for (int tt = 0; tt < 2; ++tt)                                                                \
          AC[mt][tt] = __builtin_amdgcn_mfma_f32_16x16x32_bf16(a[mt][QA], bf[tt][QB], AC[mt][tt], 0, 0, 0);
      WX_MM(acs, 2, 0) WX_MM(acs, 1, 1) WX_MM(acs, 0, 2) WX_MM(acs, 1, 0) WX_MM(acs, 0, 1) WX_MM(acc, 0, 0)
#undef WX_MM
    }
  }
  float* sl = p.slab + (long)blockIdx.x * (32 * 256 + 32);
#pragma unroll
  for (int mt = 0; mt < 2; ++mt)
#pragma unroll
    for (int tt = 0; tt < 2; ++tt)
#pragma unroll
      for (int r = 0; r < 4; ++r) sl[(mt * 16 + 4 * g + r) * 256 + ncol[tt]] = acc[mt][tt][r] + acs[mt][tt][r];
  __syncthreads();
  float* red = reinterpret_cast<float*>(scrw);
  red[bpart * 32 + bco] = dbacc;
  __syncthreads();
  if (tid < 32) {
    float sdb = 0.f;
    for (int q = 0; q < 16; ++q) sdb += red[q * 32 + tid];
    sl[32 * 256 + tid] = sdb;
  }
}

struct WstreamP {
  const float* in; long in_bs;
  const float* dout;
  float* slab;
  int B, H, W, OH, OW, Cout, K, PLANE1, PLANEo, WP;
  const unsigned char* fstore; long fs_slot_stride; int T; const int* nvalid;
};
typedef unsigned int u32x4w __attribute__((ext_vector_type(4)));
__device__ __forceinline__ float4 ws_u8x4(unsigned int w) {
  return make_float4((float)(w & 0xffu), (float)((w >> 8) & 0xffu), (float)((w >> 16) & 0xffu), (float)(w >> 24));
}
#define WS_LDU(var, u, src) var = reinterpret_cast<const unsigned int*>(src)[min(tid + (u) * ST_NT, tot4 - 1)];
#define WS_STU(var, u, nv)                                                                     \
  {                                                                                            \
    const int idx_ = min(tid + (u) * ST_NT, tot4 - 1);                                          \
    const int c_ = (idx_ >= per4) + (idx_ >= 2 * per4) + (idx_ >= 3 * per4);                   \
    const float4 e_ = ws_u8x4(var);                                                            \
    *reinterpret_cast<float4*>(img + c_ * p.PLANE1 + ((idx_ - c_ * per4) << 2)) =               \
        c_ < 4 - (nv) ? make_float4(0.f, 0.f, 0.f, 0.f) : e_;                                  \
  }
#define WS_LDI(var, u, src) var = *reinterpret_cast<const float4*>((src) + (min(tid + (u) * ST_NT, tot4 - 1) << 2));
#define WS_LDD(var, u, src) var = *reinterpret_cast<const float4*>((src) + (min(tid + (u) * ST_NT, dtot4 - 1) << 2));
#define WS_STI(var, u)                                                                         \
  {                                                                                            \
    const int idx_ = min(tid + (u) * ST_NT, tot4 - 1);                                          \
    const int c_ = (idx_ >= per4) + (idx_ >= 2 * per4) + (idx_ >= 3 * per4);                   \
    const int rem_ = idx_ - c_ * per4, row_ = rem_ / w4;                                       \
    *reinterpret_cast<float4*>(img + c_ * p.PLANE1 + row_ * p.WP + ((rem_ - row_ * w4) << 2)) = var; \
  }
#define WS_STD(var, u)                                                                         \
  {                                                                                            \
    const int idx_ = min(tid + (u) * ST_NT, dtot4 - 1);                                         \
    const int co_ = idx_ / dper4;                                                              \
    float* d_ = ldo + co_ * p.PLANEo + ((idx_ - co_ * dper4) << 2);         \
// ... 1377 lines not shown
    if (!a2c_env_on("A2C_WGRAD_F32") && plan_wstream_bf16(d, wp, gq, ldsb)) {
      static bool attrb = false;
      if (!attrb) {
        if (hipFuncSetAttribute((const void*)wgrad_stream_bf16_kernel<0>, hipFuncAttributeMaxDynamicSharedMemorySize, 160 * 1024) != hipSuccess)
          return A2C_ERR_LAUNCH;
        attrb = true;
      }
      const int gb = grid < B ? grid : B;
      hipLaunchKernelGGL(wgrad_stream_bf16_kernel<0>, dim3(gb), dim3(ST_NT), ldsb, st, wp, gq);
      A2C_CHECK_LAUNCH();
      const long nWb = (long)wp.Cout * wp.K, perb = nWb + wp.Cout;
      hipLaunchKernelGGL(wgrad_reduce_kernel, dim3(a2c_grid_1d(perb, 256)), dim3(256), 0, st, (const float*)ws, gb, perb, nWb, dW, db);
      A2C_CHECK_LAUNCH();
      return A2C_OK;
    }
  }
  const size_t lds = 4 * (size_t)(4 * wp.PLANE1 + 16 * wp.PLANEo);
  static bool attr = false;
  if (!attr) {
    if (hipFuncSetAttribute((const void*)wgrad_stream_kernel<true>, hipFuncAttributeMaxDynamicSharedMemorySize, 160 * 1024) != hipSuccess)
      return A2C_ERR_LAUNCH;
    attr = true;
  }
  hipLaunchKernelGGL(wgrad_stream_kernel<true>, dim3(grid < B ? grid : B), dim3(ST_NT), lds, st, wp);
  A2C_CHECK_LAUNCH();
  const int g = grid < B ? grid : B;
  const long nWs = (long)wp.Cout * wp.K, pers = nWs + wp.Cout;
  hipLaunchKernelGGL(wgrad_reduce_kernel, dim3(a2c_grid_1d(pers, 256)), dim3(256), 0, st, (const float*)ws, g, pers, nWs, dW, db);
  A2C_CHECK_LAUNCH();
  return A2C_OK;
}

int a2c_conv2d_bwd_weight_rank(const a2c_conv_desc* d, const float* in, int64_t in_bstride, const float* dl, int64_t ld_dl,
                               int n_logits, const float* Wc, const uint8_t* maskbits, int64_t mask_row_bytes, float* dW, float* db,
                               int B, void* ws, size_t ws_bytes, a2c_stream_t stream) {
  if (!desc_ok(d) || B < 1 || !in || !dl || !Wc || !maskbits || !dW || !db) return A2C_ERR_ARG;
  if (in_bstride % 4 || ((uintptr_t)in % 16) || ld_dl < n_logits || mask_row_bytes < (int64_t)d->Cout * d->OH * d->OW / 8 ||
      in_bstride < (int64_t)d->Cin * d->H * d->W || !a2c_conv2d_bwd_rank_supported(d, n_logits, B))
    return A2C_ERR_ARG;
  if (!ws || ws_bytes < a2c_conv2d_bwd_weight_ws_bytes(d, B)) return A2C_ERR_WORKSPACE;
  WgradPlan pl;
  if (!plan_wgrad(d, B, pl, true)) return A2C_ERR_ARG;
  const int grid = stream_grid() < pl.grid ? stream_grid() : pl.grid;
  hipStream_t st = a2c_s(stream);
  static bool attrr = false;
  if (!attrr) {
    if (hipFuncSetAttribute((const void*)wgrad_x6_kernel<true>, hipFuncAttributeMaxDynamicSharedMemorySize, wx::LDS_BYTES) != hipSuccess)
      return A2C_ERR_LAUNCH;
    attrr = true;
  }
  WgradX6P xp;
  xp.in = in; xp.in_bs = (long)in_bstride; xp.dout = nullptr; xp.slab = (float*)ws; xp.B = B;
  xp.dl = dl; xp.ldl = (long)ld_dl; xp.nlog = n_logits; xp.Wc = Wc; xp.a2b = maskbits; xp.a2b_row = (long)mask_row_bytes;
  hipLaunchKernelGGL(wgrad_x6_kernel<true>, dim3(grid), dim3(wx::NT), wx::LDS_BYTES, st, xp);
  A2C_CHECK_LAUNCH();
  const long nWx = 32L * 256, perx = nWx + 32;
  hipLaunchKernelGGL(wgrad_reduce_kernel, dim3(a2c_grid_1d(perx, 256)), dim3(256), 0, st, (const float*)ws, grid, perx, nWx, dW, db);
  A2C_CHECK_LAUNCH();
  return A2C_OK;
}

int a2c_conv2d_bwd_weight(const a2c_conv_desc* d, const float* in, int64_t in_bstride, const float* dout, float* dW,
                          float* db, int B, void* ws, size_t ws_bytes, a2c_stream_t stream) {
  WgradPlan pl;
  if (!desc_ok(d) || B < 1 || !in || !dout || !dW) return A2C_ERR_ARG;
  const bool aligned = (in_bstride % 4 == 0) && ((uintptr_t)in % 16 == 0) && ((uintptr_t)dout % 8 == 0);
  if (!plan_wgrad(d, B, pl, aligned)) return A2C_ERR_ARG;
  if (!ws || ws_bytes < a2c_conv2d_bwd_weight_ws_bytes(d, B)) return A2C_ERR_WORKSPACE;
  hipStream_t st = a2c_s(stream);
  if (c3w_supported(d) && aligned && ((uintptr_t)dout % 16 == 0) && ((uintptr_t)dW % 16 == 0) && ((uintptr_t)ws % 16 == 0))
    return c3w_bwd_weight(d, in, (long)in_bstride, dout, dW, db, B, ws, ws_bytes, st);
  {
    WstreamP wp;
    const int grid = stream_grid();
    if (aligned && B >= 8 * grid && ((uintptr_t)dout % 16 == 0) && !a2c_env_on("A2C_NO_STREAM") &&
        plan_wstream(d, wp)) {
      wp.in = in; wp.in_bs = in_bstride; wp.dout = dout; wp.slab = (float*)ws; wp.B = B;
      wp.fstore = nullptr; wp.fs_slot_stride = 0; wp.T = 1; wp.nvalid = nullptr;
      const size_t lds = 4 * (size_t)(4 * wp.PLANE1 + 16 * wp.PLANEo);
      static bool attr = false;
      if (!attr) {
        if (hipFuncSetAttribute((const void*)wgrad_stream_kernel<false>, hipFuncAttributeMaxDynamicSharedMemorySize, 160 * 1024) != hipSuccess)
          return A2C_ERR_LAUNCH;
        attr = true;
      }
      hipLaunchKernelGGL(wgrad_stream_kernel<false>, dim3(grid), dim3(ST_NT), lds, st, wp);
      A2C_CHECK_LAUNCH();
      const long nWs = (long)wp.Cout * wp.K, pers = nWs + wp.Cout;
      hipLaunchKernelGGL(wgrad_reduce_kernel, dim3(a2c_grid_1d(pers, 256)), dim3(256), 0, st, (const float*)ws, grid, pers, nWs,
                         dW, db);
      A2C_CHECK_LAUNCH();
      return A2C_OK;
    }
  }
  {
    const int grid = stream_grid() < pl.grid ? stream_grid() : pl.grid;
    if (pl.run == 2 && d->Cin == 16 && d->Cout == 32 && d->H == 20 && d->W == 20 && d->ks == 4 && d->stride == 2 && d->pad == 0 &&
        aligned && ((uintptr_t)dout % 16 == 0) && B >= 8 * grid && a2c_env_int("A2C_WGRAD_X6", 1) != 0) {
      static bool attrx = false;
      if (!attrx) {
        if (hipFuncSetAttribute((const void*)wgrad_x6_kernel<false>, hipFuncAttributeMaxDynamicSharedMemorySize, wx::LDS_BYTES) != hipSuccess ||
            hipFuncSetAttribute((const void*)wgrad_x6_kernel<true>, hipFuncAttributeMaxDynamicSharedMemorySize, wx::LDS_BYTES) != hipSuccess)
          return A2C_ERR_LAUNCH;
        attrx = true;
      }
      WgradX6P xp;
      xp.in = in; xp.in_bs = (long)in_bstride; xp.dout = dout; xp.slab = (float*)ws; xp.B = B;
      xp.dl = nullptr; xp.ldl = 0; xp.nlog = 0; xp.Wc = nullptr; xp.a2b = nullptr; xp.a2b_row = 0;
      hipLaunchKernelGGL(wgrad_x6_kernel<false>, dim3(grid), dim3(wx::NT), wx::LDS_BYTES, st, xp);
      A2C_CHECK_LAUNCH();
      const long nWx = 32L * 256, perx = nWx + 32;
      hipLaunchKernelGGL(wgrad_reduce_kernel, dim3(a2c_grid_1d(perx, 256)), dim3(256), 0, st, (const float*)ws, grid, perx, nWx, dW, db);
      A2C_CHECK_LAUNCH();
      return A2C_OK;
    }
  }
  if (pl.run) {
    WrunP q;
    fill_stage(q.st, pl.t, in, in_bstride);
    q.dout = dout; q.slab = (float*)ws;
    q.Cout = d->Cout; q.K = d->Cin * d->ks * d->ks; q.ks = d->ks; q.OH = d->OH; q.OW = d->OW; q.OWp = pl.OWp;
    q.TPH = pl.t.TPH; q.tiles = pl.t.tiles; q.B = B; q.PLANEo = pl.PLANEo;
    if (pl.run == 1) hipLaunchKernelGGL((wgrad_run_kernel<1, 4, 1, 5>), dim3(pl.grid), dim3(256), pl.lds, st, q);
    else hipLaunchKernelGGL((wgrad_run_kernel<2, 2, 2, 3>), dim3(pl.grid), dim3(256), pl.lds, st, q);
    A2C_CHECK_LAUNCH();
    const long nWr = (long)q.Cout * q.K, perr = nWr + q.Cout;
    hipLaunchKernelGGL(wgrad_reduce_kernel, dim3(a2c_grid_1d(perr, 256)), dim3(256), 0, st, (const float*)ws, pl.grid,
                       perr, nWr, dW, db);
    A2C_CHECK_LAUNCH();
    return A2C_OK;
  }
  WgradP p;
  fill_stage(p.st, pl.t, in, in_bstride);
  p.dout = dout; p.slab = (float*)ws;
  p.Cout = d->Cout; p.K = d->Cin * d->ks * d->ks; p.ks = d->ks; p.OH = d->OH; p.OW = d->OW; p.OWp = pl.OWp;
  p.S = d->stride; p.sy0 = pl.t.sy0; p.TPH = pl.t.TPH; p.tiles = pl.t.tiles; p.B = B;
  p.PLANEo = pl.PLANEo; p.nkt = ceil_div(p.K, 16);
  p.dvec = ((d->OW % 4 == 0) && ((uintptr_t)dout % 16 == 0)) ? 4 : ((d->OW % 2 == 0) && ((uintptr_t)dout % 8 == 0)) ? 2 : 0;
  p.dflat = (pl.t.tiles == 1 && ((long)d->Cout * d->OH * d->OW) % 4 == 0 && ((uintptr_t)dout % 16 == 0)) ? 1 : 0;
#define WGRAD_LAUNCH(...) launch_wgrad_t<__VA_ARGS__>(p, pl.grid, pl.lds, st)
  WGRAD_VARIANTS(WGRAD_LAUNCH)
#undef WGRAD_LAUNCH
  A2C_CHECK_LAUNCH();
  const long nW = (long)p.Cout * p.K, per = nW + p.Cout;
  hipLaunchKernelGGL(wgrad_reduce_kernel, dim3(a2c_grid_1d(per, 256)), dim3(256), 0, st, (const float*)ws, pl.grid, per,
                     nW, dW, db);
  A2C_CHECK_LAUNCH();
  return A2C_OK;
}
}
```

### pytorch-a2c_amd/csrc/step.hip

```cpp
#include <stdlib.h>
#include "a2c_common.h"

namespace {
typedef float f32x4 __attribute__((ext_vector_type(4)));
typedef unsigned int u32x4 __attribute__((ext_vector_type(4)));
constexpr int NT = 512;
constexpr int NCH = 3;
constexpr int SL0 = 6, SL1 = 5, SL2 = 5;
constexpr int HN = 8;
constexpr int NF1 = 64 * 64;
constexpr int NF2 = 64 * 2 * 64;
constexpr int NF1B = 8 * 3 * 64 * 4;
typedef __bf16 bf16x8 __attribute__((ext_vector_type(8)));

#ifdef A2C_STEP_TIMING
__device__ unsigned long long a2c_step_ts[16];
__device__ int a2c_step_skip;
#define TS(i) do { if (blockIdx.x == 0 && threadIdx.x == 0) a2c_step_ts[i] = wall_clock64(); } while (0)
#define SKIP(bit) (a2c_step_skip & (1 << (bit)))
#else
#define TS(i)
#define SKIP(bit) false
#endif

struct RolloutX {
  float* states;
  float* bookmark;
  const float* u; long u_stride;
  int64_t* actions;
  unsigned long long* cmd;
  const unsigned long long* rec;
  unsigned int seq0;
  int env0;
  int* err;
  long timeout_ticks;
  float* a1_rows;
  float* a2_rows;
  unsigned long long* a1_lm;
  unsigned char* a2_mb;
  float* heads_rows; long heads_rows_ld;
  unsigned char* fstore; long fs_slot_stride;
  int* nvalid; int* nvalid_carry;
  int states_lazy;
  const unsigned char* tagged; long tagged_stride; int tagged_nd;
  int frame_bits;
  unsigned long long* dbg;
  int poll_gap;
  int early_poll;
  int bstride, boff;
};

struct StepP {
  a2c_a3c_step_args a;
  int OH1, OW1, OH2, OW2, PLANE1, PLANE2, F, F4;
  int row_end[NCH];
  int tile_end[NCH];
  RolloutX x;
};

struct It {
  const float* prev;
  const float* frame32;
  bool frame8;
  float* out;
  float* a1o;
  float* a2o;
  float* ho;
};

template <int N>
__device__ __forceinline__ void issue_chunk(float4 (&pf)[N], const It& it, int r0, int q4, int HW, int W, int tid) {
  const bool has_frame = it.frame32 != nullptr || it.frame8;
  const float* __restrict__ pb = it.prev + (has_frame ? HW : 0);
  const float* __restrict__ p3 = it.frame32 ? it.frame32 : pb + (it.frame8 ? 2L : 3L) * HW;
#pragma unroll
  for (int u = 0; u < N; ++u) {
    const int idx = min(tid + u * NT, 4 * q4 - 1);
    const int c = (idx >= q4) + (idx >= 2 * q4) + (idx >= 3 * q4);
    const int rem = idx - c * q4;
    const long off = (c == 3) ? (long)(p3 - pb) : (long)c * HW;
    const f32x4 t_ = __builtin_nontemporal_load(reinterpret_cast<const f32x4*>(pb + off + r0 * W + (rem << 2)));
    pf[u] = SKIP(4) ? make_float4(0.f, 0.f, 0.f, 0.f) : make_float4(t_[0], t_[1], t_[2], t_[3]);
  }
}

template <int N>
__device__ __forceinline__ void commit_chunk(const float4 (&pf)[N], const It& it, int r0, int q4, int W, int tid,
                                             bool zero_old, float* __restrict__ img, int PLANE1) {
#pragma unroll
  for (int u = 0; u < N; ++u) {
    const int idx = min(tid + u * NT, 4 * q4 - 1);
    const int c = (idx >= q4) + (idx >= 2 * q4) + (idx >= 3 * q4);
    const int rem = idx - c * q4;
    float4 v = pf[u];
    if (zero_old && c != 3) v = make_float4(0.f, 0.f, 0.f, 0.f);
    if (!(it.frame8 && c == 3)) *reinterpret_cast<float4*>(img + c * PLANE1 + r0 * W + (rem << 2)) = v;
  }
}

template <int N>
__device__ __forceinline__ void store_chunk(const float4 (&pf)[N], const It& it, int r0, int q4, int HW, int W, int tid,
                                            bool zero_old) {
#pragma unroll
  for (int u = 0; u < N; ++u) {
    const int idx = min(tid + u * NT, 4 * q4 - 1);
    const int c = (idx >= q4) + (idx >= 2 * q4) + (idx >= 3 * q4);
    const int rem = idx - c * q4;
    float4 v = pf[u];
    if (zero_old && c != 3) v = make_float4(0.f, 0.f, 0.f, 0.f);
    if (!SKIP(0) && !(it.frame8 && c == 3))
      __builtin_nontemporal_store((f32x4){v.x, v.y, v.z, v.w},
                                  reinterpret_cast<f32x4*>(it.out + (long)c * HW + r0 * W + (rem << 2)));
  }
}

__device__ __forceinline__ float4 u8x4(unsigned int w) {
  return make_float4((float)(w & 0xffu), (float)((w >> 8) & 0xffu), (float)((w >> 16) & 0xffu), (float)(w >> 24));
}

__device__ __forceinline__ unsigned int bf16_pair_exact(float a, float b) {
  return __builtin_amdgcn_perm(__float_as_uint(b), __float_as_uint(a), 0x07060302u);
}
__device__ __forceinline__ bf16x8 u8x8_bf16(unsigned int lo, unsigned int hi) {
  u32x4 r;
  r[0] = bf16_pair_exact((float)(lo & 0xffu), (float)((lo >> 8) & 0xffu));
  r[1] = bf16_pair_exact((float)((lo >> 16) & 0xffu), (float)(lo >> 24));
  r[2] = bf16_pair_exact((float)(hi & 0xffu), (float)((hi >> 8) & 0xffu));
  r[3] = bf16_pair_exact((float)((hi >> 16) & 0xffu), (float)(hi >> 24));
  return __builtin_bit_cast(bf16x8, r);
}
__device__ __forceinline__ unsigned short bf16_bits(float x) { return __builtin_bit_cast(unsigned short, (__bf16)x); }

template <bool OUT, bool U8, bool PERSIST, int HNT = HN>
__global__ __launch_bounds__(NT) __attribute__((amdgpu_waves_per_eu(2, 2))) void a3c_step_kernel(StepP p) {
  extern __shared__ __attribute__((aligned(16))) float lds[];
  if (SKIP(6)) return;
  const a2c_a3c_step_args& a = p.a;
  float* __restrict__ fr1 = lds;
  float* __restrict__ img = fr1 + NF1;
  float* __restrict__ a1 = img + 4 * p.PLANE1;
  float* __restrict__ red = a1 + 16 * p.PLANE2;
  float* __restrict__ a2 = img + NF2;
  const int tid = threadIdx.x, lane = tid & 63;
  const int g = lane >> 4;
  const int HW = a.H * a.W, W = a.W;
  const int N = a.n_actions + 1;
  const bool tail = tid == NT - 64;
  asm volatile("" ::"s"(a.prev), "s"(a.prev_stride), "s"(a.frame_new), "s"(a.reset_mask), "s"(a.out), "s"(a.out_stride),
               "s"(a.wfrag1), "s"(a.bias1), "s"(a.bias2), "s"(a.heads), "s"(a.ldh), "s"(a.rew), "s"(a.done),
               "s"(a.val_prev), "s"(a.rewards), "s"(a.dones), "s"(a.T), "s"(a.t_rec), "s"(a.slot0), "s"(a.H), "s"(a.W),
               "s"(a.n_actions), "s"(p.PLANE1), "s"(p.row_end[0]), "s"(p.row_end[1]), "s"(p.row_end[2]));
  TS(0);

  const float4 b1v = *reinterpret_cast<const float4*>(a.bias1 + 4 * g);
  const float b1[4] = {b1v.x, b1v.y, b1v.z, b1v.w};
  const float ld_b2 = a.bias2[tid & 31];
  const float4* __restrict__ wf1v = reinterpret_cast<const float4*>(a.wfrag1);
  const int q0 = (p.row_end[0] * W) >> 2, q1 = ((p.row_end[1] - p.row_end[0]) * W) >> 2, q2 = ((p.row_end[2] - p.row_end[1]) * W) >> 2;
  const int NP1 = p.OH1 * p.OW1;
  const float* __restrict__ la1 = fr1 + lane;
  if (PERSIST) {
    float4* __restrict__ fv = reinterpret_cast<float4*>(fr1);
    fv[tid] = wf1v[tid]; fv[tid + NT] = wf1v[tid + NT];
    if (tid < 32) red[HN + tid] = ld_b2;
    if (tid == 0) reinterpret_cast<unsigned int*>(red)[HN + 37] = 0u;
  }

  const int nb = PERSIST ? (a.B - (int)blockIdx.x + (int)gridDim.x - 1) / (int)gridDim.x : 1;
  const int n_it = PERSIST ? ((int)a.T + 1) * nb : 1;
  const long S = 4L * HW;
  for (int iter = 0; iter < n_it; ++iter) {
    const int t = PERSIST ? iter / nb : 0;
    const int b = PERSIST ? (int)blockIdx.x + (iter - t * nb) * (int)gridDim.x : (int)blockIdx.x;
    int tid_op = tid;
    if (PERSIST && HNT > 4) asm volatile("" : "+v"(tid_op));
    const int tid = tid_op, lane = tid & 63, w = tid >> 6, g = lane >> 4, j = lane & 15;
    It it;
    bool rec, boot, sample;
    long t_rec;
    const float* u_ptr;
    int64_t* act_ptr;
    if (PERSIST) {
      const long row = (a.slot0 + b) * a.T;
      it.prev = t == 0 ? p.x.bookmark + (long)b * S : p.x.states + (row + t - 1) * S;
// ... 873 lines not shown
      else if (pf) {
        early = p.x.early_poll && (unsigned int)(gr_e >> 33) == want_n;
        if (early) {
          gr_pf = gr_e;
          f_pf = __builtin_amdgcn_raw_buffer_load_b128(fr_pf, lane * 16, 0, 1 | 16);
        } else {
          gr_pf = __hip_atomic_load(p.x.rec + p.x.env0 + b, __ATOMIC_RELAXED, __HIP_MEMORY_SCOPE_SYSTEM);
        }
      }
      conv1_planes(nbase, 2, 3);
      if (pf && !tg) {
        pre_ok = (unsigned int)(gr_pf >> 33) == want_n;
        if (pre_ok && !early) f_pf = __builtin_amdgcn_raw_buffer_load_b128(fr_pf, lane * 16, 0, 1 | 16);
      }
    }
    RING_TS(6);
    if (pf && tg) {
      pre_ok = tg_ok(f_pf, p.x.seq0 + (unsigned int)(t + 1));
      if (pre_ok) tg_unpack(f_pf, (nbase + 3) % 5);
    } else if (pf) {
    } else {
      const bool dealt = t < T && p.x.frame_bits != 0;
      const int sid = dealt ? (w == 0 ? tid : tid - 64) : tid, sn = dealt ? NT - 64 : NT;
      float* __restrict__ out = t == T ? p.x.bookmark + (long)b * S : p.x.states + (row + t) * S;
      const int hw4 = HW >> 2;
      if (t == T || !p.x.states_lazy)
        for (int q = sid; q < 4 * hw4; q += sn) {
          const int pl = q / hw4, o = q - pl * hw4;
          const unsigned int x = reinterpret_cast<const unsigned int*>(ring + ((base + pl) % 5) * HW)[o];
          const float4 v = u8x4(x);
          __builtin_nontemporal_store((f32x4){v.x, v.y, v.z, v.w}, reinterpret_cast<f32x4*>(out) + q);
        }
      if (fs_slot != nullptr && t > 0) {
        const u32x4* __restrict__ src = reinterpret_cast<const u32x4*>(ring + ((base + 3) % 5) * HW);
        u32x4* __restrict__ dst = reinterpret_cast<u32x4*>(fs_slot + (long)(t + 3) * HW);
        for (int q = sid; q < (HW >> 4); q += sn) dst[q] = src[q];
      }
      if (p.x.a1_rows != nullptr && t < T) {
        float* __restrict__ a1o = p.x.a1_rows + (row + t) * (16L * NP1);
        const int n4 = NP1 >> 2;
        unsigned char* __restrict__ lmo = (p.x.a1_lm != nullptr && (16 * n4) % 64 == 0)
                                              ? reinterpret_cast<unsigned char*>(p.x.a1_lm) + (row + t) * (long)(16 * n4 / 2) : nullptr;
        for (int q = sid; q < 16 * n4; q += sn) {
          const int ch = q / n4, o4 = q - ch * n4;
          const float4 v = *reinterpret_cast<const float4*>(a1 + ch * p.PLANE2 + (o4 << 2));
          __builtin_nontemporal_store((f32x4){v.x, v.y, v.z, v.w}, reinterpret_cast<f32x4*>(a1o) + q);
          if (lmo != nullptr) {
            const unsigned int nib = (v.x > 0.f ? 1u : 0u) | (v.y > 0.f ? 2u : 0u) | (v.z > 0.f ? 4u : 0u) | (v.w > 0.f ? 8u : 0u);
            const unsigned int hi = __shfl_xor(nib, 1);
            if (!(q & 1)) lmo[q >> 1] = (unsigned char)(nib | (hi << 4));
          }
        }
      }
      if (p.x.a2_rows != nullptr && t < T) {
        float* __restrict__ a2o = p.x.a2_rows + (row + t) * (long)p.F;
        unsigned char* __restrict__ mbo = (p.x.a2_mb != nullptr && (p.F & 7) == 0) ? p.x.a2_mb + (row + t) * (long)(p.F >> 3) : nullptr;
        for (int q = sid; q < (p.F >> 2); q += sn) {
          const float4 v = *reinterpret_cast<const float4*>(a2 + (q << 2));
          __builtin_nontemporal_store((f32x4){v.x, v.y, v.z, v.w}, reinterpret_cast<f32x4*>(a2o) + q);
          if (mbo != nullptr) {
            const unsigned int nib = (v.x > 0.f ? 1u : 0u) | (v.y > 0.f ? 2u : 0u) | (v.z > 0.f ? 4u : 0u) | (v.w > 0.f ? 8u : 0u);
            const unsigned int hi = __shfl_xor(nib, 1);
            if (!(q & 1)) mbo[q >> 1] = (unsigned char)(nib | (hi << 4));
          }
        }
      }
    }
    if (pf && pre_ok && !tg) {
      unsigned char* __restrict__ dst = ring + ((nbase + 3) % 5) * HW + lane * 128;
#pragma unroll
      for (int q = 0; q < 8; ++q) {
        const unsigned int bits = f_pf[q >> 1] >> (16 * (q & 1));
        u32x4 v;
#pragma unroll
        for (int e = 0; e < 4; ++e) {
          const unsigned int wq = bits >> (4 * e);
          v[e] = (wq & 1u) | ((wq & 2u) << 7) | ((wq & 4u) << 14) | ((wq & 8u) << 21);
        }
        if (lane * 128 + q * 16 < HW) *reinterpret_cast<u32x4*>(dst + q * 16) = v;
      }
      if (lane == 0) {
        reinterpret_cast<unsigned int*>(red)[HN + 32] = (unsigned int)gr_pf;
        reinterpret_cast<unsigned int*>(red)[HN + 33] = (unsigned int)(gr_pf >> 32);
        reinterpret_cast<unsigned int*>(red)[HN + 36] = 1u;
      }
    }
    if (t < T) base = nbase;
    RING_TS(7);
  }
  if (stamp)
    for (int q = 0; q < 10; ++q) p.x.dbg[q] = ts_sum[q];
#undef RING_TS
}

static bool ring_bf16() { return !a2c_env_on("A2C_RING_F32"); }
static size_t ring_lds(const StepP& p, int hnt) {
  const int ntile2 = (p.OH2 * p.OW2 + 15) / 16;
  const size_t part = (size_t)ntile2 * 1024 > (size_t)hnt * NT ? (size_t)ntile2 * 1024 : (size_t)hnt * NT;
  const size_t nf1 = ring_bf16() ? (size_t)NF1B : (size_t)NF1;
  return 4 * (nf1 + NF2 + (size_t)16 * p.PLANE2 + p.F4 + part + HN + 32 + 8) + (size_t)5 * p.a.H * p.a.W + 64;
}

static inline int plane_pad(int n, int mod64) {
  int p = ((n + 63) / 64) * 64 + mod64;
  if (p - 64 >= n) p -= 64;
  return p;
// ... 83 lines not shown
  StepP p;
  p.a = *args;
  p.x = RolloutX{};
  const a2c_a3c_step_args& a = p.a;
  if (a.B < 0) return A2C_ERR_ARG;
  if (a.B == 0) return A2C_OK;
  if (!step_shapes(a.C, a.H, a.W, a.n_actions, p) || step_lds(p) > 160 * 1024) return A2C_ERR_ARG;
  if (!a.prev) return A2C_ERR_ARG;
  if (!a.wfrag1 || !a.bias1 || !a.wfrag2 || !a.bias2 || !a.Wc || !a.bc || !a.heads) return A2C_ERR_ARG;
  if (a.u && !a.actions) return A2C_ERR_ARG;
  if (a.rew && (!a.done || !a.val_prev || !a.rewards || !a.dones || !a.deltas || a.T < 1 || a.t_rec < 0 || a.t_rec >= a.T))
    return A2C_ERR_ARG;
  if (a.bootstrap && (!a.rew || a.t_rec != a.T - 1)) return A2C_ERR_ARG;
  if (a.prev_stride % 4 || (a.out && a.out_stride % 4) || a.ldh < a.n_actions + 1) return A2C_ERR_ARG;
  if ((((uintptr_t)a.prev | (uintptr_t)a.frame_new | (uintptr_t)a.out | (uintptr_t)a.wfrag2 | (uintptr_t)a.Wc) % 16)) return A2C_ERR_ARG;
  if (a.frame_u8 && (a.frame_new || !u8_shapes(a.H, a.W) || a.frame_stride % 16 || (uintptr_t)a.frame_u8 % 16 ||
                     a.frame_stride < a.H * a.W))
    return A2C_ERR_ARG;
  if ((a.a1_out || a.a2_out) && ((p.OH1 * p.OW1) % 4 || a.a1_stride % 4 || a.a2_stride % 4 ||
                                 (((uintptr_t)a.a1_out | (uintptr_t)a.a2_out) % 16)))
    return A2C_ERR_ARG;
  const size_t lds = step_lds(p);
  if (!set_lds_attr()) return A2C_ERR_LAUNCH;
  if (a.frame_u8) {
    if (a.out) hipLaunchKernelGGL((a3c_step_kernel<true, true, false>), dim3(a.B), dim3(NT), lds, a2c_s(stream), p);
    else hipLaunchKernelGGL((a3c_step_kernel<false, true, false>), dim3(a.B), dim3(NT), lds, a2c_s(stream), p);
  } else {
    if (a.out) hipLaunchKernelGGL((a3c_step_kernel<true, false, false>), dim3(a.B), dim3(NT), lds, a2c_s(stream), p);
    else hipLaunchKernelGGL((a3c_step_kernel<false, false, false>), dim3(a.B), dim3(NT), lds, a2c_s(stream), p);
  }
  A2C_CHECK_LAUNCH();
  return A2C_OK;
}

int a2c_a3c_rollout(const a2c_a3c_rollout_args* r, a2c_stream_t stream) {
  if (!r) return A2C_ERR_ARG;
  if (r->B < 0) return A2C_ERR_ARG;
  if (r->B == 0) return A2C_OK;
  StepP p;
  p.a = a2c_a3c_step_args{};
  a2c_a3c_step_args& a = p.a;
  a.B = r->B; a.C = r->C; a.H = r->H; a.W = r->W; a.n_actions = r->n_actions;
  a.wfrag1 = r->wfrag1; a.bias1 = r->bias1; a.wfrag2 = r->wfrag2; a.bias2 = r->bias2; a.Wc = r->Wc; a.bc = r->bc;
  a.heads = r->heads; a.ldh = r->ldh;
  a.val_prev = r->val_prev; a.rewards = r->rewards; a.dones = r->dones; a.deltas = r->deltas;
  a.T = r->T; a.slot0 = r->slot0; a.gamma = r->gamma; a.pong = r->pong;
  a.frame_u8 = r->frames; a.frame_stride = r->frame_stride;
  p.x.states = r->states; p.x.bookmark = r->bookmark; p.x.u = r->u; p.x.u_stride = (long)r->u_stride;
  p.x.actions = r->actions; p.x.cmd = (unsigned long long*)r->cmd; p.x.rec = (const unsigned long long*)r->rec;
  p.x.seq0 = r->seq0; p.x.env0 = r->env0; p.x.err = r->err; p.x.timeout_ticks = (long)r->timeout_ticks;
  p.x.a1_rows = r->a1_rows; p.x.a2_rows = r->a2_rows;
  p.x.a1_lm = (r->a1_rows != nullptr) ? (unsigned long long*)r->a1_lanemask_rows : nullptr;
  p.x.a2_mb = (r->a2_rows != nullptr) ? r->a2_maskbit_rows : nullptr;
  p.x.heads_rows = r->heads_rows; p.x.heads_rows_ld = (long)r->heads_rows_ld;
  p.x.fstore = r->frame_store; p.x.fs_slot_stride = (long)r->frame_store_slot_stride;
  p.x.nvalid = r->nvalid_rows; p.x.nvalid_carry = r->nvalid_carry;
  p.x.states_lazy = (r->states_lazy && r->frame_store) ? 1 : 0;
  {
    const bool ok = r->tagged && r->frame_bits && r->tagged_chunks >= 2 && r->tagged_chunks <= 64 &&
                    r->tagged_stride >= 16 * (int64_t)r->tagged_chunks && r->tagged_stride % 16 == 0 && ((uintptr_t)r->tagged % 16) == 0 &&
                    (r->tagged_chunks - 1) * 112 >= r->H * r->W;
    p.x.tagged = ok ? r->tagged : nullptr;
    p.x.tagged_stride = ok ? (long)r->tagged_stride : 0;
    p.x.tagged_nd = ok ? r->tagged_chunks - 1 : 0;
  }
  p.x.frame_bits = r->frame_bits ? 1 : 0;
  p.x.dbg = g_ring_dbg;
  p.x.poll_gap = 4;
  p.x.early_poll = 1;
  if (r->frame_store && (!r->nvalid_rows || !r->nvalid_carry || r->T < 4 || ((uintptr_t)r->frame_store % 16) ||
                         r->frame_store_slot_stride % 16 || r->frame_store_slot_stride < (r->T + 4) * (int64_t)r->H * r->W))
    return A2C_ERR_ARG;
  if (r->heads_rows && r->heads_rows_ld < r->n_actions + 1) return A2C_ERR_ARG;
  if (!step_shapes(a.C, a.H, a.W, a.n_actions, p) || step_lds(p) > 160 * 1024 || !u8_shapes(a.H, a.W)) return A2C_ERR_ARG;
  if (!r->states || !r->bookmark || !r->u || !r->actions || !r->cmd || !r->rec || !r->frames || !r->err) return A2C_ERR_ARG;
  if (!a.wfrag1 || !a.bias1 || !a.wfrag2 || !a.bias2 || !a.Wc || !a.bc || !a.heads) return A2C_ERR_ARG;
  if (!a.val_prev || !a.rewards || !a.dones || !a.deltas || a.T < 1 || a.ldh < a.n_actions + 1) return A2C_ERR_ARG;
  if (r->frame_stride % 16 || r->frame_stride < (r->frame_bits ? (a.H * a.W + 7) / 8 : a.H * a.W) || r->timeout_ticks < 1 ||
      r->env0 < 0)
    return A2C_ERR_ARG;
  if ((r->a1_rows || r->a2_rows) && ((p.OH1 * p.OW1) % 4 || (((uintptr_t)r->a1_rows | (uintptr_t)r->a2_rows) % 16))) return A2C_ERR_ARG;
  if (r->a1_lanemask_rows && (!r->a1_rows || ((uintptr_t)r->a1_lanemask_rows % 8) || (16 * p.OH1 * p.OW1) % 256)) return A2C_ERR_ARG;
  if (r->a2_maskbit_rows && (!r->a2_rows || p.F % 8)) return A2C_ERR_ARG;
  if ((((uintptr_t)r->states | (uintptr_t)r->bookmark | (uintptr_t)r->frames | (uintptr_t)a.wfrag2 | (uintptr_t)a.Wc) % 16) ||
      (((uintptr_t)r->cmd | (uintptr_t)r->rec) % 8))
    return A2C_ERR_ARG;
  if (!set_lds_attr()) return A2C_ERR_LAUNCH;
  int dev = 0, cus = 256;
  if (hipGetDevice(&dev) != hipSuccess || hipDeviceGetAttribute(&cus, hipDeviceAttributeMultiprocessorCount, dev) != hipSuccess || cus < 1) cus = 256;
  const int hnt = a.n_actions + 1 <= 4 ? 4 : 8;
  p.x.bstride = 1; p.x.boff = 0;
  if (ring_applies(p, a.B, cus, hnt, r->conv1_weight)) {
    const size_t rl = ring_lds(p, hnt);
    const bool bf = ring_bf16();
    const int nblk = (a.B + cus - 1) / cus;
    p.x.bstride = nblk;
    for (int k = 0; k < nblk; ++k) {
      p.x.boff = k;
      const int cnt = (a.B - k + nblk - 1) / nblk;
      if (bf) {
        if (hnt == 4) hipLaunchKernelGGL((a3c_ring_kernel<4, true>), dim3(cnt), dim3(NT), rl, a2c_s(stream), p, r->conv1_weight);
        else hipLaunchKernelGGL((a3c_ring_kernel<8, true>), dim3(cnt), dim3(NT), rl, a2c_s(stream), p, r->conv1_weight);
      } else {
        if (hnt == 4) hipLaunchKernelGGL((a3c_ring_kernel<4, false>), dim3(cnt), dim3(NT), rl, a2c_s(stream), p, r->conv1_weight);
        else hipLaunchKernelGGL((a3c_ring_kernel<8, false>), dim3(cnt), dim3(NT), rl, a2c_s(stream), p, r->conv1_weight);
      }
      A2C_CHECK_LAUNCH();
    }
    return A2C_OK;
  }
  if (p.x.states_lazy || p.x.a1_lm || p.x.a2_mb) return A2C_ERR_ARG;
  const size_t lds = step_lds(p);
  const int grid = a.B < cus ? a.B : cus;
  if (a.n_actions + 1 <= 4) hipLaunchKernelGGL((a3c_step_kernel<true, true, true, 4>), dim3(grid), dim3(NT), lds, a2c_s(stream), p);
  else hipLaunchKernelGGL((a3c_step_kernel<true, true, true, 8>), dim3(grid), dim3(NT), lds, a2c_s(stream), p);
  A2C_CHECK_LAUNCH();
  return A2C_OK;
}
}
```

### pytorch-a2c_amd/csrc/torch_ops_abi.inc

```
namespace {
inline void* abi_ptr(at::TensorList bufs, at::IntArrayRef offs, size_t k, const char* what) {
  const at::Tensor& t = bufs[k];
  if (!t.defined() || t.numel() == 0) return nullptr;
  TORCH_CHECK(t.is_cuda(), what, ": buffer ", k, " must be a HIP tensor (there is no CPU kernel)");
  const int64_t room = (int64_t)t.storage().nbytes() - (int64_t)t.storage_offset() * (int64_t)t.element_size();
  TORCH_CHECK(offs[k] >= 0 && offs[k] < room, what, ": offset ", offs[k], " outside buffer ", k, " (", room, " bytes)");
  return (char*)t.data_ptr() + offs[k];
}
inline void abi_counts(at::TensorList bufs, at::IntArrayRef offs, at::IntArrayRef ints, at::ArrayRef<double> flts,
                       size_t np, size_t ni, size_t nf, const char* what) {
  TORCH_CHECK(bufs.size() == np && offs.size() == np && ints.size() == ni && flts.size() == nf, what,
              ": expected ", np, " buffers/offsets, ", ni, " ints, ", nf, " floats");
}
void abi_discount_scan(at::TensorList bufs, at::IntArrayRef offs, at::IntArrayRef ints, at::ArrayRef<double> flts) {
  abi_counts(bufs, offs, ints, flts, 4, 2, 1, "a2c_discount_scan");
  ok(a2c_discount_scan((const float *)abi_ptr(bufs, offs, 0, "a2c_discount_scan"), (const float *)abi_ptr(bufs, offs, 1, "a2c_discount_scan"), (float *)abi_ptr(bufs, offs, 2, "a2c_discount_scan"), (int64_t)ints[0], (int64_t)ints[1], (float)flts[0], (int *)abi_ptr(bufs, offs, 3, "a2c_discount_scan"), cur_stream()), "a2c_discount_scan");
}
void abi_gae_returns_fused(at::TensorList bufs, at::IntArrayRef offs, at::IntArrayRef ints, at::ArrayRef<double> flts) {
  abi_counts(bufs, offs, ints, flts, 6, 2, 2, "a2c_gae_returns_fused");
  ok(a2c_gae_returns_fused((const float *)abi_ptr(bufs, offs, 0, "a2c_gae_returns_fused"), (const float *)abi_ptr(bufs, offs, 1, "a2c_gae_returns_fused"), (const float *)abi_ptr(bufs, offs, 2, "a2c_gae_returns_fused"), (float *)abi_ptr(bufs, offs, 3, "a2c_gae_returns_fused"), (float *)abi_ptr(bufs, offs, 4, "a2c_gae_returns_fused"), (int64_t)ints[0], (int64_t)ints[1], (float)flts[0], (float)flts[1], (int *)abi_ptr(bufs, offs, 5, "a2c_gae_returns_fused"), cur_stream()), "a2c_gae_returns_fused");
}
void abi_moments(at::TensorList bufs, at::IntArrayRef offs, at::IntArrayRef ints, at::ArrayRef<double> flts) {
  abi_counts(bufs, offs, ints, flts, 3, 1, 0, "a2c_moments");
  ok(a2c_moments((const float *)abi_ptr(bufs, offs, 0, "a2c_moments"), (int64_t)ints[0], (double *)abi_ptr(bufs, offs, 1, "a2c_moments"), (double *)abi_ptr(bufs, offs, 2, "a2c_moments"), cur_stream()), "a2c_moments");
// ... 213 lines not shown
  d0.Cout = (int)ints[3];
  d0.ks = (int)ints[4];
  d0.stride = (int)ints[5];
  d0.pad = (int)ints[6];
  d0.OH = (int)ints[7];
  d0.OW = (int)ints[8];
  ok(a2c_conv2d_fwd_signs(&d0, (const float *)abi_ptr(bufs, offs, 0, "a2c_conv2d_fwd_signs"), (int64_t)ints[9], (const float *)abi_ptr(bufs, offs, 1, "a2c_conv2d_fwd_signs"), (const float *)abi_ptr(bufs, offs, 2, "a2c_conv2d_fwd_signs"), (int)ints[10], (float *)abi_ptr(bufs, offs, 3, "a2c_conv2d_fwd_signs"), (int64_t)ints[11], (uint32_t *)abi_ptr(bufs, offs, 4, "a2c_conv2d_fwd_signs"), (int64_t)ints[12], (int)ints[13], cur_stream()), "a2c_conv2d_fwd_signs");
}
void abi_lanemask_from_act(at::TensorList bufs, at::IntArrayRef offs, at::IntArrayRef ints, at::ArrayRef<double> flts) {
  abi_counts(bufs, offs, ints, flts, 2, 1, 0, "a2c_lanemask_from_act");
  ok(a2c_lanemask_from_act((const float *)abi_ptr(bufs, offs, 0, "a2c_lanemask_from_act"), (uint64_t *)abi_ptr(bufs, offs, 1, "a2c_lanemask_from_act"), (int64_t)ints[0], cur_stream()), "a2c_lanemask_from_act");
}
void abi_conv2d_bwd_data_lanemask(at::TensorList bufs, at::IntArrayRef offs, at::IntArrayRef ints, at::ArrayRef<double> flts) {
  abi_counts(bufs, offs, ints, flts, 4, 10, 0, "a2c_conv2d_bwd_data_lanemask");
  a2c_conv_desc d0;
  d0.Cin = (int)ints[0];
  d0.H = (int)ints[1];
  d0.W = (int)ints[2];
  d0.Cout = (int)ints[3];
  d0.ks = (int)ints[4];
  d0.stride = (int)ints[5];
  d0.pad = (int)ints[6];
  d0.OH = (int)ints[7];
  d0.OW = (int)ints[8];
  ok(a2c_conv2d_bwd_data_lanemask(&d0, (const float *)abi_ptr(bufs, offs, 0, "a2c_conv2d_bwd_data_lanemask"), (const float *)abi_ptr(bufs, offs, 1, "a2c_conv2d_bwd_data_lanemask"), (const uint64_t *)abi_ptr(bufs, offs, 2, "a2c_conv2d_bwd_data_lanemask"), (float *)abi_ptr(bufs, offs, 3, "a2c_conv2d_bwd_data_lanemask"), (int)ints[9], cur_stream()), "a2c_conv2d_bwd_data_lanemask");
}
void abi_conv2d_bwd_data_lanemask_rank(at::TensorList bufs, at::IntArrayRef offs, at::IntArrayRef ints, at::ArrayRef<double> flts) {
  abi_counts(bufs, offs, ints, flts, 6, 13, 0, "a2c_conv2d_bwd_data_lanemask_rank");
  a2c_conv_desc d0;
  d0.Cin = (int)ints[0];
  d0.H = (int)ints[1];
  d0.W = (int)ints[2];
  d0.Cout = (int)ints[3];
  d0.ks = (int)ints[4];
  d0.stride = (int)ints[5];
  d0.pad = (int)ints[6];
  d0.OH = (int)ints[7];
  d0.OW = (int)ints[8];
  ok(a2c_conv2d_bwd_data_lanemask_rank(&d0, (const float *)abi_ptr(bufs, offs, 0, "a2c_conv2d_bwd_data_lanemask_rank"), (int64_t)ints[9], (int)ints[10], (const float *)abi_ptr(bufs, offs, 1, "a2c_conv2d_bwd_data_lanemask_rank"), (const uint8_t *)abi_ptr(bufs, offs, 2, "a2c_conv2d_bwd_data_lanemask_rank"), (int64_t)ints[11], (const float *)abi_ptr(bufs, offs, 3, "a2c_conv2d_bwd_data_lanemask_rank"), (const uint64_t *)abi_ptr(bufs, offs, 4, "a2c_conv2d_bwd_data_lanemask_rank"), (float *)abi_ptr(bufs, offs, 5, "a2c_conv2d_bwd_data_lanemask_rank"), (int)ints[12], cur_stream()), "a2c_conv2d_bwd_data_lanemask_rank");
}
void abi_conv2d_bwd_weight_rank(at::TensorList bufs, at::IntArrayRef offs, at::IntArrayRef ints, at::ArrayRef<double> flts) {
  abi_counts(bufs, offs, ints, flts, 7, 15, 0, "a2c_conv2d_bwd_weight_rank");
  a2c_conv_desc d0;
  d0.Cin = (int)ints[0];
  d0.H = (int)ints[1];
  d0.W = (int)ints[2];
  d0.Cout = (int)ints[3];
  d0.ks = (int)ints[4];
  d0.stride = (int)ints[5];
  d0.pad = (int)ints[6];
  d0.OH = (int)ints[7];
  d0.OW = (int)ints[8];
  ok(a2c_conv2d_bwd_weight_rank(&d0, (const float *)abi_ptr(bufs, offs, 0, "a2c_conv2d_bwd_weight_rank"), (int64_t)ints[9], (const float *)abi_ptr(bufs, offs, 1, "a2c_conv2d_bwd_weight_rank"), (int64_t)ints[10], (int)ints[11], (const float *)abi_ptr(bufs, offs, 2, "a2c_conv2d_bwd_weight_rank"), (const uint8_t *)abi_ptr(bufs, offs, 3, "a2c_conv2d_bwd_weight_rank"), (int64_t)ints[12], (float *)abi_ptr(bufs, offs, 4, "a2c_conv2d_bwd_weight_rank"), (float *)abi_ptr(bufs, offs, 5, "a2c_conv2d_bwd_weight_rank"), (int)ints[13], (void *)abi_ptr(bufs, offs, 6, "a2c_conv2d_bwd_weight_rank"), (size_t)ints[14], cur_stream()), "a2c_conv2d_bwd_weight_rank");
}
void abi_conv2d_bwd_data_signs(at::TensorList bufs, at::IntArrayRef offs, at::IntArrayRef ints, at::ArrayRef<double> flts) {
  abi_counts(bufs, offs, ints, flts, 4, 11, 0, "a2c_conv2d_bwd_data_signs");
  a2c_conv_desc d0;
  d0.Cin = (int)ints[0];
  d0.H = (int)ints[1];
  d0.W = (int)ints[2];
  d0.Cout = (int)ints[3];
  d0.ks = (int)ints[4];
  d0.stride = (int)ints[5];
  d0.pad = (int)ints[6];
  d0.OH = (int)ints[7];
  d0.OW = (int)ints[8];
  ok(a2c_conv2d_bwd_data_signs(&d0, (const float *)abi_ptr(bufs, offs, 0, "a2c_conv2d_bwd_data_signs"), (const float *)abi_ptr(bufs, offs, 1, "a2c_conv2d_bwd_data_signs"), (const uint32_t *)abi_ptr(bufs, offs, 2, "a2c_conv2d_bwd_data_signs"), (int64_t)ints[9], (float *)abi_ptr(bufs, offs, 3, "a2c_conv2d_bwd_data_signs"), (int)ints[10], cur_stream()), "a2c_conv2d_bwd_data_signs");
}
void abi_conv2d_bwd_data_w1_frames(at::TensorList bufs, at::IntArrayRef offs, at::IntArrayRef ints, at::ArrayRef<double> flts) {
  abi_counts(bufs, offs, ints, flts, 8, 23, 0, "a2c_conv2d_bwd_data_w1_frames");
  a2c_conv_desc d0;
  d0.Cin = (int)ints[0];
  d0.H = (int)ints[1];
  d0.W = (int)ints[2];
  d0.Cout = (int)ints[3];
  d0.ks = (int)ints[4];
  d0.stride = (int)ints[5];
  d0.pad = (int)ints[6];
  d0.OH = (int)ints[7];
  d0.OW = (int)ints[8];
  a2c_conv_desc d1;
  d1.Cin = (int)ints[10];
  d1.H = (int)ints[11];
  d1.W = (int)ints[12];
  d1.Cout = (int)ints[13];
  d1.ks = (int)ints[14];
  d1.stride = (int)ints[15];
  d1.pad = (int)ints[16];
  d1.OH = (int)ints[17];
  d1.OW = (int)ints[18];
  ok(a2c_conv2d_bwd_data_w1_frames(&d0, (const float *)abi_ptr(bufs, offs, 0, "a2c_conv2d_bwd_data_w1_frames"), (const float *)abi_ptr(bufs, offs, 1, "a2c_conv2d_bwd_data_w1_frames"), (const uint32_t *)abi_ptr(bufs, offs, 2, "a2c_conv2d_bwd_data_w1_frames"), (int64_t)ints[9], &d1, (const uint8_t *)abi_ptr(bufs, offs, 3, "a2c_conv2d_bwd_data_w1_frames"), (int64_t)ints[19], (int64_t)ints[20], (const int32_t *)abi_ptr(bufs, offs, 4, "a2c_conv2d_bwd_data_w1_frames"), (float *)abi_ptr(bufs, offs, 5, "a2c_conv2d_bwd_data_w1_frames"), (float *)abi_ptr(bufs, offs, 6, "a2c_conv2d_bwd_data_w1_frames"), (int)ints[21], (void *)abi_ptr(bufs, offs, 7, "a2c_conv2d_bwd_data_w1_frames"), (size_t)ints[22], cur_stream()), "a2c_conv2d_bwd_data_w1_frames");
}
void abi_conv2d_bwd_data_w1(at::TensorList bufs, at::IntArrayRef offs, at::IntArrayRef ints, at::ArrayRef<double> flts) {
  abi_counts(bufs, offs, ints, flts, 7, 21, 0, "a2c_conv2d_bwd_data_w1");
  a2c_conv_desc d0;
  d0.Cin = (int)ints[0];
  d0.H = (int)ints[1];
  d0.W = (int)ints[2];
  d0.Cout = (int)ints[3];
  d0.ks = (int)ints[4];
  d0.stride = (int)ints[5];
  d0.pad = (int)ints[6];
  d0.OH = (int)ints[7];
  d0.OW = (int)ints[8];
  a2c_conv_desc d1;
  d1.Cin = (int)ints[9];
// ... 150 lines not shown
#define A2C_ABI_OPS_DEF(m) \
  m.def("abi_discount_scan(Tensor(a!)[] bufs, int[] offs, int[] ints, float[] floats) -> ()"); \
  m.def("abi_gae_returns_fused(Tensor(a!)[] bufs, int[] offs, int[] ints, float[] floats) -> ()"); \
  m.def("abi_moments(Tensor(a!)[] bufs, int[] offs, int[] ints, float[] floats) -> ()"); \
  m.def("abi_normalize(Tensor(a!)[] bufs, int[] offs, int[] ints, float[] floats) -> ()"); \
  m.def("abi_add(Tensor(a!)[] bufs, int[] offs, int[] ints, float[] floats) -> ()"); \
  m.def("abi_frame_stack_push(Tensor(a!)[] bufs, int[] offs, int[] ints, float[] floats) -> ()"); \
  m.def("abi_frame_stack_push_u8(Tensor(a!)[] bufs, int[] offs, int[] ints, float[] floats) -> ()"); \
  m.def("abi_pool_publish_actions(Tensor(a!)[] bufs, int[] offs, int[] ints, float[] floats) -> ()"); \
  m.def("abi_pool_ingest(Tensor(a!)[] bufs, int[] offs, int[] ints, float[] floats) -> ()"); \
  m.def("abi_pool_ingest_bits(Tensor(a!)[] bufs, int[] offs, int[] ints, float[] floats) -> ()"); \
  m.def("abi_unpack_bits(Tensor(a!)[] bufs, int[] offs, int[] ints, float[] floats) -> ()"); \
  m.def("abi_pool_ingest_post(Tensor(a!)[] bufs, int[] offs, int[] ints, float[] floats) -> ()"); \
  m.def("abi_frame_prep_u8(Tensor(a!)[] bufs, int[] offs, int[] ints, float[] floats) -> ()"); \
  m.def("abi_frame_store_begin(Tensor(a!)[] bufs, int[] offs, int[] ints, float[] floats) -> ()"); \
  m.def("abi_rollout_post_frames(Tensor(a!)[] bufs, int[] offs, int[] ints, float[] floats) -> ()"); \
  m.def("abi_frames_to_states(Tensor(a!)[] bufs, int[] offs, int[] ints, float[] floats) -> ()"); \
  m.def("abi_softmax_sample(Tensor(a!)[] bufs, int[] offs, int[] ints, float[] floats) -> ()"); \
  m.def("abi_sample_probs(Tensor(a!)[] bufs, int[] offs, int[] ints, float[] floats) -> ()"); \
  m.def("abi_rollout_record(Tensor(a!)[] bufs, int[] offs, int[] ints, float[] floats) -> ()"); \
  m.def("abi_rollout_post(Tensor(a!)[] bufs, int[] offs, int[] ints, float[] floats) -> ()"); \
  m.def("abi_rollout_post_u8(Tensor(a!)[] bufs, int[] offs, int[] ints, float[] floats) -> ()"); \
  m.def("abi_rollout_post_rec(Tensor(a!)[] bufs, int[] offs, int[] ints, float[] floats) -> ()"); \
  m.def("abi_rollout_bootstrap(Tensor(a!)[] bufs, int[] offs, int[] ints, float[] floats) -> ()"); \
  m.def("abi_store_u32_system(Tensor(a!)[] bufs, int[] offs, int[] ints, float[] floats) -> ()"); \
  m.def("abi_memcpy_async(Tensor(a!)[] bufs, int[] offs, int[] ints, float[] floats) -> ()"); \
  m.def("abi_copy_rows(Tensor(a!)[] bufs, int[] offs, int[] ints, float[] floats) -> ()"); \
  m.def("abi_mask_rows(Tensor(a!)[] bufs, int[] offs, int[] ints, float[] floats) -> ()"); \
  m.def("abi_permute_rows(Tensor(a!)[] bufs, int[] offs, int[] ints, float[] floats) -> ()"); \
  m.def("abi_loss_fwd_bwd(Tensor(a!)[] bufs, int[] offs, int[] ints, float[] floats) -> ()"); \
  m.def("abi_gauss_head(Tensor(a!)[] bufs, int[] offs, int[] ints, float[] floats) -> ()"); \
  m.def("abi_gauss_loss_sums(Tensor(a!)[] bufs, int[] offs, int[] ints, float[] floats) -> ()"); \
  m.def("abi_gauss_loss_fwd_bwd(Tensor(a!)[] bufs, int[] offs, int[] ints, float[] floats) -> ()"); \
  m.def("abi_gemm_f32(Tensor(a!)[] bufs, int[] offs, int[] ints, float[] floats) -> ()"); \
  m.def("abi_gemm_x6_split(Tensor(a!)[] bufs, int[] offs, int[] ints, float[] floats) -> ()"); \
  m.def("abi_gemm_x6_images(Tensor(a!)[] bufs, int[] offs, int[] ints, float[] floats) -> ()"); \
  m.def("abi_small_n_bwd_data_bits(Tensor(a!)[] bufs, int[] offs, int[] ints, float[] floats) -> ()"); \
  m.def("abi_gemm_f32_partial(Tensor(a!)[] bufs, int[] offs, int[] ints, float[] floats) -> ()"); \
  m.def("abi_heads_fused(Tensor(a!)[] bufs, int[] offs, int[] ints, float[] floats) -> ()"); \
  m.def("abi_heads_fused_publish(Tensor(a!)[] bufs, int[] offs, int[] ints, float[] floats) -> ()"); \
  m.def("abi_gemm_f32_nt(Tensor(a!)[] bufs, int[] offs, int[] ints, float[] floats) -> ()"); \
  m.def("abi_gemm_f32_nn(Tensor(a!)[] bufs, int[] offs, int[] ints, float[] floats) -> ()"); \
  m.def("abi_gemm_f32_tn(Tensor(a!)[] bufs, int[] offs, int[] ints, float[] floats) -> ()"); \
  m.def("abi_compose_heads(Tensor(a!)[] bufs, int[] offs, int[] ints, float[] floats) -> ()"); \
  m.def("abi_colsum(Tensor(a!)[] bufs, int[] offs, int[] ints, float[] floats) -> ()"); \
  m.def("abi_conv2d_prep_weights(Tensor(a!)[] bufs, int[] offs, int[] ints, float[] floats) -> ()"); \
  m.def("abi_conv2d_fwd(Tensor(a!)[] bufs, int[] offs, int[] ints, float[] floats) -> ()"); \
  m.def("abi_conv2d_bwd_data(Tensor(a!)[] bufs, int[] offs, int[] ints, float[] floats) -> ()"); \
  m.def("abi_conv2d_fwd_signs(Tensor(a!)[] bufs, int[] offs, int[] ints, float[] floats) -> ()"); \
  m.def("abi_lanemask_from_act(Tensor(a!)[] bufs, int[] offs, int[] ints, float[] floats) -> ()"); \
  m.def("abi_conv2d_bwd_data_lanemask(Tensor(a!)[] bufs, int[] offs, int[] ints, float[] floats) -> ()"); \
  m.def("abi_conv2d_bwd_data_lanemask_rank(Tensor(a!)[] bufs, int[] offs, int[] ints, float[] floats) -> ()"); \
  m.def("abi_conv2d_bwd_weight_rank(Tensor(a!)[] bufs, int[] offs, int[] ints, float[] floats) -> ()"); \
  m.def("abi_conv2d_bwd_data_signs(Tensor(a!)[] bufs, int[] offs, int[] ints, float[] floats) -> ()"); \
  m.def("abi_conv2d_bwd_data_w1_frames(Tensor(a!)[] bufs, int[] offs, int[] ints, float[] floats) -> ()"); \
  m.def("abi_conv2d_bwd_data_w1(Tensor(a!)[] bufs, int[] offs, int[] ints, float[] floats) -> ()"); \
  m.def("abi_conv2d_bwd_weight(Tensor(a!)[] bufs, int[] offs, int[] ints, float[] floats) -> ()"); \
  m.def("abi_conv2d_bwd_weight_frames(Tensor(a!)[] bufs, int[] offs, int[] ints, float[] floats) -> ()"); \
  m.def("abi_conv2d_fwd_frames(Tensor(a!)[] bufs, int[] offs, int[] ints, float[] floats) -> ()"); \
  m.def("abi_gru_gates(Tensor(a!)[] bufs, int[] offs, int[] ints, float[] floats) -> ()"); \
  m.def("abi_gru_out(Tensor(a!)[] bufs, int[] offs, int[] ints, float[] floats) -> ()"); \
  m.def("abi_gru_cell_fwd(Tensor(a!)[] bufs, int[] offs, int[] ints, float[] floats) -> ()"); \
  m.def("abi_gru_out_bwd(Tensor(a!)[] bufs, int[] offs, int[] ints, float[] floats) -> ()"); \
  m.def("abi_gru_out_bwd_carry(Tensor(a!)[] bufs, int[] offs, int[] ints, float[] floats) -> ()"); \
  m.def("abi_gru_gates_bwd(Tensor(a!)[] bufs, int[] offs, int[] ints, float[] floats) -> ()"); \
  m.def("abi_gru_cell_bwd(Tensor(a!)[] bufs, int[] offs, int[] ints, float[] floats) -> ()"); \
  m.def("abi_layernorm_fwd(Tensor(a!)[] bufs, int[] offs, int[] ints, float[] floats) -> ()"); \
  m.def("abi_layernorm_bwd(Tensor(a!)[] bufs, int[] offs, int[] ints, float[] floats) -> ()"); \
  m.def("abi_gradnorm_sq(Tensor(a!)[] bufs, int[] offs, int[] ints, float[] floats) -> ()"); \
  m.def("abi_clip_rmsprop(Tensor(a!)[] bufs, int[] offs, int[] ints, float[] floats) -> ()"); \
  m.def("abi_clip_adam(Tensor(a!)[] bufs, int[] offs, int[] ints, float[] floats) -> ()"); \
  m.def("abi_clip_sgd(Tensor(a!)[] bufs, int[] offs, int[] ints, float[] floats) -> ()"); \
  m.def("abi_clip_adagrad(Tensor(a!)[] bufs, int[] offs, int[] ints, float[] floats) -> ()"); \
  m.def("abi_clip_adadelta(Tensor(a!)[] bufs, int[] offs, int[] ints, float[] floats) -> ()"); \
  m.def("abi_clip_rprop(Tensor(a!)[] bufs, int[] offs, int[] ints, float[] floats) -> ()"); \
  m.def("abi_clip_adamw(Tensor(a!)[] bufs, int[] offs, int[] ints, float[] floats) -> ()"); \
  m.def("abi_clip_adamax(Tensor(a!)[] bufs, int[] offs, int[] ints, float[] floats) -> ()"); \
  m.def("abi_clip_nadam(Tensor(a!)[] bufs, int[] offs, int[] ints, float[] floats) -> ()"); \
  m.def("abi_clip_radam(Tensor(a!)[] bufs, int[] offs, int[] ints, float[] floats) -> ()"); \
  m.def("abi_clip_asgd(Tensor(a!)[] bufs, int[] offs, int[] ints, float[] floats) -> ()"); \
  m.def("abi_pack_update_scalars(Tensor(a!)[] bufs, int[] offs, int[] ints, float[] floats) -> ()"); \
  m.def("abi_snake_reset(Tensor(a!)[] bufs, int[] offs, int[] ints, float[] floats) -> ()"); \
  m.def("abi_snake_step(Tensor(a!)[] bufs, int[] offs, int[] ints, float[] floats) -> ()"); \
  (void)0
#define A2C_ABI_OPS_IMPL(m) \
  m.impl("abi_discount_scan", &abi_discount_scan); \
  m.impl("abi_gae_returns_fused", &abi_gae_returns_fused); \
  m.impl("abi_moments", &abi_moments); \
  m.impl("abi_normalize", &abi_normalize); \
  m.impl("abi_add", &abi_add); \
  m.impl("abi_frame_stack_push", &abi_frame_stack_push); \
  m.impl("abi_frame_stack_push_u8", &abi_frame_stack_push_u8); \
  m.impl("abi_pool_publish_actions", &abi_pool_publish_actions); \
  m.impl("abi_pool_ingest", &abi_pool_ingest); \
  m.impl("abi_pool_ingest_bits", &abi_pool_ingest_bits); \
  m.impl("abi_unpack_bits", &abi_unpack_bits); \
  m.impl("abi_pool_ingest_post", &abi_pool_ingest_post); \
  m.impl("abi_frame_prep_u8", &abi_frame_prep_u8); \
  m.impl("abi_frame_store_begin", &abi_frame_store_begin); \
  m.impl("abi_rollout_post_frames", &abi_rollout_post_frames); \
  m.impl("abi_frames_to_states", &abi_frames_to_states); \
  m.impl("abi_softmax_sample", &abi_softmax_sample); \
  m.impl("abi_sample_probs", &abi_sample_probs); \
  m.impl("abi_rollout_record", &abi_rollout_record); \
  m.impl("abi_rollout_post", &abi_rollout_post); \
  m.impl("abi_rollout_post_u8", &abi_rollout_post_u8); \
  m.impl("abi_rollout_post_rec", &abi_rollout_post_rec); \
  m.impl("abi_rollout_bootstrap", &abi_rollout_bootstrap); \
  m.impl("abi_store_u32_system", &abi_store_u32_system); \
  m.impl("abi_memcpy_async", &abi_memcpy_async); \
  m.impl("abi_copy_rows", &abi_copy_rows); \
  m.impl("abi_mask_rows", &abi_mask_rows); \
  m.impl("abi_permute_rows", &abi_permute_rows); \
  m.impl("abi_loss_fwd_bwd", &abi_loss_fwd_bwd); \
  m.impl("abi_gauss_head", &abi_gauss_head); \
  m.impl("abi_gauss_loss_sums", &abi_gauss_loss_sums); \
  m.impl("abi_gauss_loss_fwd_bwd", &abi_gauss_loss_fwd_bwd); \
  m.impl("abi_gemm_f32", &abi_gemm_f32); \
  m.impl("abi_gemm_x6_split", &abi_gemm_x6_split); \
  m.impl("abi_gemm_x6_images", &abi_gemm_x6_images); \
  m.impl("abi_small_n_bwd_data_bits", &abi_small_n_bwd_data_bits); \
  m.impl("abi_gemm_f32_partial", &abi_gemm_f32_partial); \
  m.impl("abi_heads_fused", &abi_heads_fused); \
  m.impl("abi_heads_fused_publish", &abi_heads_fused_publish); \
  m.impl("abi_gemm_f32_nt", &abi_gemm_f32_nt); \
  m.impl("abi_gemm_f32_nn", &abi_gemm_f32_nn); \
  m.impl("abi_gemm_f32_tn", &abi_gemm_f32_tn); \
  m.impl("abi_compose_heads", &abi_compose_heads); \
  m.impl("abi_colsum", &abi_colsum); \
  m.impl("abi_conv2d_prep_weights", &abi_conv2d_prep_weights); \
  m.impl("abi_conv2d_fwd", &abi_conv2d_fwd); \
  m.impl("abi_conv2d_bwd_data", &abi_conv2d_bwd_data); \
  m.impl("abi_conv2d_fwd_signs", &abi_conv2d_fwd_signs); \
  m.impl("abi_lanemask_from_act", &abi_lanemask_from_act); \
  m.impl("abi_conv2d_bwd_data_lanemask", &abi_conv2d_bwd_data_lanemask); \
  m.impl("abi_conv2d_bwd_data_lanemask_rank", &abi_conv2d_bwd_data_lanemask_rank); \
  m.impl("abi_conv2d_bwd_weight_rank", &abi_conv2d_bwd_weight_rank); \
  m.impl("abi_conv2d_bwd_data_signs", &abi_conv2d_bwd_data_signs); \
  m.impl("abi_conv2d_bwd_data_w1_frames", &abi_conv2d_bwd_data_w1_frames); \
  m.impl("abi_conv2d_bwd_data_w1", &abi_conv2d_bwd_data_w1); \
  m.impl("abi_conv2d_bwd_weight", &abi_conv2d_bwd_weight); \
  m.impl("abi_conv2d_bwd_weight_frames", &abi_conv2d_bwd_weight_frames); \
  m.impl("abi_conv2d_fwd_frames", &abi_conv2d_fwd_frames); \
  m.impl("abi_gru_gates", &abi_gru_gates); \
  m.impl("abi_gru_out", &abi_gru_out); \
  m.impl("abi_gru_cell_fwd", &abi_gru_cell_fwd); \
  m.impl("abi_gru_out_bwd", &abi_gru_out_bwd); \
  m.impl("abi_gru_out_bwd_carry", &abi_gru_out_bwd_carry); \
  m.impl("abi_gru_gates_bwd", &abi_gru_gates_bwd); \
  m.impl("abi_gru_cell_bwd", &abi_gru_cell_bwd); \
  m.impl("abi_layernorm_fwd", &abi_layernorm_fwd); \
  m.impl("abi_layernorm_bwd", &abi_layernorm_bwd); \
  m.impl("abi_gradnorm_sq", &abi_gradnorm_sq); \
  m.impl("abi_clip_rmsprop", &abi_clip_rmsprop); \
  m.impl("abi_clip_adam", &abi_clip_adam); \
  m.impl("abi_clip_sgd", &abi_clip_sgd); \
  m.impl("abi_clip_adagrad", &abi_clip_adagrad); \
  m.impl("abi_clip_adadelta", &abi_clip_adadelta); \
  m.impl("abi_clip_rprop", &abi_clip_rprop); \
  m.impl("abi_clip_adamw", &abi_clip_adamw); \
  m.impl("abi_clip_adamax", &abi_clip_adamax); \
  m.impl("abi_clip_nadam", &abi_clip_nadam); \
  m.impl("abi_clip_radam", &abi_clip_radam); \
  m.impl("abi_clip_asgd", &abi_clip_asgd); \
  m.impl("abi_pack_update_scalars", &abi_pack_update_scalars); \
  m.impl("abi_snake_reset", &abi_snake_reset); \
  m.impl("abi_snake_step", &abi_snake_step); \
  (void)0
```

Measured before the change: 8.748 million.

## Stash pre-split bf16 pieces of conv1 activations during rollout for conv2 wgrad

During the rollout step kernel, conv1 activations are split into three bf16 pieces (a 3-term bf16 split of f32) in the layout the conv2 weight-gradient kernel uses, and written to a per-row stash buffer. A new PIECES variant of the wgrad_x6 kernel DMAs these pieces straight into LDS, skipping the in-kernel f32 load and bf16 split of a1. This removes split arithmetic and LDS staging work from the update phase. In exchange the rollout does extra work and writes 46KB per row, and the piece buffer is roughly triple the size of the f32 activations it replaces as input.

New measurement: 8.129 million. 7.1% lower.

```diff
diff --git a/include/a2c_mi355x.h b/include/a2c_mi355x.h
--- a/include/a2c_mi355x.h
+++ b/include/a2c_mi355x.h
@@ -152,6 +152,7 @@
   const uint8_t *tagged; int64_t tagged_stride; int tagged_chunks;
   uint64_t *a1_lanemask_rows;
   uint8_t *a2_maskbit_rows;
+  uint8_t *a1_piece_rows;
 } a2c_a3c_rollout_args;
 int a2c_a3c_rollout(const a2c_a3c_rollout_args *args, a2c_stream_t stream);
 int a2c_a3c_ring_supported(int B, int C, int H, int W, int n_actions, const float *conv1_weight);
@@ -267,6 +268,10 @@
 int a2c_conv2d_bwd_weight_rank(const a2c_conv_desc *d, const float *in, int64_t in_bstride, const float *dl, int64_t ld_dl,
                                int n_logits, const float *Wc, const uint8_t *maskbits, int64_t mask_row_bytes, float *dW,
                                float *db, int B, void *ws, size_t ws_bytes, a2c_stream_t stream);
+int a2c_conv2d_bwd_weight_rank_pieces(const a2c_conv_desc *d, const float *in, int64_t in_bstride, const uint8_t *pieces,
+                                      int64_t pieces_bstride, const float *dl, int64_t ld_dl, int n_logits, const float *Wc,
+                                      const uint8_t *maskbits, int64_t mask_row_bytes, float *dW, float *db, int B, void *ws,
+                                      size_t ws_bytes, a2c_stream_t stream);
 int a2c_conv2d_bwd_data_signs(const a2c_conv_desc *d, const float *dout, const float *wprep_bwd, const uint32_t *signs,
                               int64_t signs_bstride, float *din, int B, a2c_stream_t stream);
 size_t a2c_conv2d_bwd_data_w1_frames_ws_bytes(const a2c_conv_desc *d2, const a2c_conv_desc *d1, int B);
diff --git a/pytorch-a2c_amd/a2c_amd/_lib.py b/pytorch-a2c_amd/a2c_amd/_lib.py
--- a/pytorch-a2c_amd/a2c_amd/_lib.py
+++ b/pytorch-a2c_amd/a2c_amd/_lib.py
@@ -40,7 +40,7 @@
                 ("frame_store", P), ("frame_store_slot_stride", c_int64), ("nvalid_rows", P), ("nvalid_carry", P),
                 ("frame_bits", c_int), ("conv1_weight", P), ("states_lazy", c_int),
                 ("tagged", P), ("tagged_stride", c_int64), ("tagged_chunks", c_int), ("a1_lanemask_rows", P),
-                ("a2_maskbit_rows", P)]
+                ("a2_maskbit_rows", P), ("a1_piece_rows", P)]
 
 
 PS = POINTER(A3CStepArgs)
@@ -133,6 +133,8 @@
     "a2c_conv2d_bwd_rank_supported": (c_int, [PD, c_int, c_int]),
     "a2c_conv2d_bwd_data_lanemask_rank": (c_int, [PD, P, c_int64, c_int, P, P, c_int64, P, P, P, c_int, P]),
     "a2c_conv2d_bwd_weight_rank": (c_int, [PD, P, c_int64, P, c_int64, c_int, P, P, c_int64, P, P, c_int, P, c_size_t, P]),
+    "a2c_conv2d_bwd_weight_rank_pieces": (c_int, [PD, P, c_int64, P, c_int64, P, c_int64, c_int, P, P, c_int64, P, P, c_int, P, c_size_t,
+                                                  P]),
     "a2c_conv2d_bwd_data_lanemask": (c_int, [PD, P, P, P, P, c_int, P]),
     "a2c_conv2d_bwd_data_signs": (c_int, [PD, P, P, P, c_int64, P, c_int, P]),
     "a2c_conv2d_bwd_weight_ws_bytes": (c_size_t, [PD, c_int]),
diff --git a/pytorch-a2c_amd/a2c_amd/models.py b/pytorch-a2c_amd/a2c_amd/models.py
--- a/pytorch-a2c_amd/a2c_amd/models.py
+++ b/pytorch-a2c_amd/a2c_amd/models.py
@@ -70,6 +70,7 @@
         self._stash = None
         self._stash_frames = None
         self._stash_lm = False
+        self._stash_pc = False
 
     def _conv_chain(self):
         ch = getattr(self, "_chain", 0)
@@ -94,19 +95,20 @@
         return getattr(self, "_stash", None) == (x_ptr, int(n_rows))
 
     _ROUTE_SWITCHES = ("A2C_NO_STASH", "A2C_NO_LANEMASK", "A2C_NO_EMB_STASH", "A2C_NO_CELL_STASH", "A2C_NO_HEADS_STASH",
-                       "A2C_NO_FRAME_STORE")
+                       "A2C_NO_FRAME_STORE", "A2C_NO_PIECE_STASH")
 
     def _route_state(self):
-        return (self._stash, self._stash_frames, getattr(self, "_stash_lm", False), getattr(self, "_cells_done", None))
+        return (self._stash, self._stash_frames, getattr(self, "_stash_lm", False), getattr(self, "_cells_done", None),
+                getattr(self, "_stash_pc", False))
 
     def _set_route_state(self, rs):
-        self._stash, self._stash_frames, self._stash_lm, cells = rs
+        self._stash, self._stash_frames, self._stash_lm, cells, self._stash_pc = rs
         if cells is not None:
             self._cells_done = cells
 
     def _route_sig(self):
-        st, fr, lm, cells = self._route_state()
-        return (st, None if fr is None else (fr[0].data_ptr(), fr[1].data_ptr(), int(fr[2])), bool(lm), cells,
+        st, fr, lm, cells, pc = self._route_state()
+        return (st, None if fr is None else (fr[0].data_ptr(), fr[1].data_ptr(), int(fr[2])), bool(lm), cells, bool(pc),
                 tuple(os.environ.get(k) == "1" for k in self._ROUTE_SWITCHES))
 
     def _need_states(self):
@@ -306,7 +308,8 @@
             return None
         ws = self.ws("train")
         return (ws.get("a1", (n_rows,) + self._c1.out_shape), ws.get("a2", (n_rows,) + self._c2.out_shape),
-                self._heads("train", n_rows)[0], self._a1_lanemask_rows(n_rows), self._a2_maskbit_rows(n_rows))
+                self._heads("train", n_rows)[0], self._a1_lanemask_rows(n_rows), self._a2_maskbit_rows(n_rows),
+                self._a1_piece_rows(n_rows))
 
     def _a2_maskbit_rows(self, n_rows):
         F = self.flat_size
@@ -320,9 +323,16 @@
             return None
         return self.ws("train").get("a1_lm", (n_rows, n // 64), dtype=torch.int64)
 
-    def stash_commit(self, states, n_rows, frames=None, lanemask=False):
+    def _a1_piece_rows(self, n_rows):
+        if (os.environ.get("A2C_NO_PIECE_STASH") == "1" or os.environ.get("A2C_NO_LANEMASK") == "1" or os.environ.get("A2C_NO_RANK_FUSE") == "1"
+                or tuple(self._c1.out_shape) != (16, 20, 20) or not ops.conv_bwd_rank_supported(self._c2.d, self.output_space, n_rows)):
+            return None
+        return self.ws("train").get("a1_pc", (n_rows, ops.A1_PIECE_ROW_BYTES), dtype=torch.uint8)
+
+    def stash_commit(self, states, n_rows, frames=None, lanemask=False, pieces=False):
         super().stash_commit(states, n_rows, frames=frames)
         self._stash_lm = bool(lanemask)
+        self._stash_pc = bool(pieces) and bool(lanemask)
 
     def _fwd(self, x_ptr, bstride, B, tag, st, save, sampler=None):
         ws, P = self.ws(tag), self.P
@@ -448,9 +458,16 @@
                 linear_bwd_data(ws, demb, Wp, da2.view(B, -1), B, st, mask=a2)
             if fuse_da2:
                 buf = ws.bytes("conv_wgrad_ws", ops.conv_bwd_weight_ws_bytes(self._c2.d, B))
+                pc = None
+                if getattr(self, "_stash_pc", False) and os.environ.get("A2C_NO_PIECE_STASH") != "1":
+                    pc = self._a1_piece_rows(B)
                 with ops.span("conv2.bwd_weight"):
-                    ops.conv_bwd_weight_rank(self._c2.d, a1.data_ptr(), a1[0].numel(), dl, dl.stride(0), A, self._Wc, mb, mb.stride(0),
-                                             G("convs.1.0.weight"), G("convs.1.0.bias"), B, buf, st)
+                    if pc is not None:
+                        ops.conv_bwd_weight_rank_pieces(self._c2.d, a1.data_ptr(), a1[0].numel(), pc, dl, dl.stride(0), A, self._Wc, mb,
+                                                        mb.stride(0), G("convs.1.0.weight"), G("convs.1.0.bias"), B, buf, st)
+                    else:
+                        ops.conv_bwd_weight_rank(self._c2.d, a1.data_ptr(), a1[0].numel(), dl, dl.stride(0), A, self._Wc, mb, mb.stride(0),
+                                                 G("convs.1.0.weight"), G("convs.1.0.bias"), B, buf, st)
             else:
                 self._c2.bwd_weight(a1.data_ptr(), a1[0].numel(), da2, G("convs.1.0.weight"), G("convs.1.0.bias"), B, ws, st)
             da1 = ws.get("da1", (B,) + self._c1.out_shape)
diff --git a/pytorch-a2c_amd/a2c_amd/ops.py b/pytorch-a2c_amd/a2c_amd/ops.py
--- a/pytorch-a2c_amd/a2c_amd/ops.py
+++ b/pytorch-a2c_amd/a2c_amd/ops.py
@@ -848,6 +848,20 @@
                                            st if st is not None else stream()), "a2c_conv2d_bwd_weight_rank")
 
 
+A1_PIECE_ROW_BYTES = 3 * 320 * 48
+
+
+def conv_bwd_weight_rank_pieces(d, in_ptr, in_bstride, pieces, dl, ld_dl, n_logits, Wc, maskbits, mask_row_bytes, dW, db, B, ws, st=None):
+    _chk(maskbits, "maskbits", torch.uint8)
+    if pieces is not None:
+        _chk(pieces, "pieces", torch.uint8)
+    check(lib().a2c_conv2d_bwd_weight_rank_pieces(ctypes.byref(d), in_ptr, in_bstride, 0 if pieces is None else pieces.data_ptr(),
+                                                  0 if pieces is None else pieces.stride(0), _p(dl), ld_dl, n_logits, _p(Wc),
+                                                  _p(maskbits), mask_row_bytes, _p(dW), _p(db), B, ws.data_ptr(),
+                                                  ws.numel() * ws.element_size(), st if st is not None else stream()),
+          "a2c_conv2d_bwd_weight_rank_pieces")
+
+
 def conv_bwd_weight_frames(d, fstore, slot_stride, T, nvalid, dout, dW, db, B, ws, st=None):
     _chk(fstore, "frame_store", torch.uint8); _chk(nvalid, "nvalid", torch.int32)
     check(lib().a2c_conv2d_bwd_weight_frames(ctypes.byref(d), _p(fstore), slot_stride, T, _p(nvalid), _p(dout), _p(dW), _p(db),
diff --git a/pytorch-a2c_amd/a2c_amd/runner.py b/pytorch-a2c_amd/a2c_amd/runner.py
--- a/pytorch-a2c_amd/a2c_amd/runner.py
+++ b/pytorch-a2c_amd/a2c_amd/runner.py
@@ -278,7 +278,9 @@
         net._stash = None
         net._stash_frames = None
         net._stash_lm = False
+        net._stash_pc = False
         self._lm_written = False
+        self._pc_written = False
         if hasattr(net, "_cells_done"):
             net._cells_done = -1
         self._stash_bufs = None
@@ -316,7 +318,8 @@
             ops.store_u32_system(dev_phase, 0)
         if stash_all:
             if getattr(self, "_lm_written", False):
-                net.stash_commit(self.datas["states"], N, frames=getattr(self, "_frames_written", None), lanemask=True)
+                net.stash_commit(self.datas["states"], N, frames=getattr(self, "_frames_written", None), lanemask=True,
+                                 **({"pieces": True} if getattr(self, "_pc_written", False) else {}))
             else:
                 net.stash_commit(self.datas["states"], N, frames=getattr(self, "_frames_written", None))
 
@@ -842,6 +845,7 @@
         lazy = fs is not None and bool(try_key(hyps, "lazy_states", False)) and ring
         lm = self._stash_bufs[3] if (ring and self._stash_bufs is not None and len(self._stash_bufs) > 3) else None
         mb = self._stash_bufs[4] if (lm is not None and len(self._stash_bufs) > 4) else None
+        pc = self._stash_bufs[5] if (mb is not None and len(self._stash_bufs) > 5) else None
         ops.a3c_rollout(st, B=B, C=C, H=H, W=W, n_actions=net.output_space, states=D["states"].data_ptr(),
                         bookmark=bm.data_ptr(), wfrag1=net._c1.wf.data_ptr(), bias1=P("convs.0.0.bias").data_ptr(),
                         wfrag2=net._c2.wf.data_ptr(), bias2=P("convs.1.0.bias").data_ptr(), Wc=net._Wc.data_ptr(),
@@ -863,7 +867,8 @@
                         nvalid_carry=0 if fs is None else fs[2][env0:env0 + B].data_ptr(), states_lazy=int(lazy),
                         tagged=getattr(pool, "dev_tagged", 0), tagged_stride=int(pool.header.tagged_stride),
                         tagged_chunks=int(pool.header.tagged_chunks), a1_lanemask_rows=0 if lm is None else lm.data_ptr(),
-                        a2_maskbit_rows=0 if mb is None else mb.data_ptr())
+                        a2_maskbit_rows=0 if mb is None else mb.data_ptr(), a1_piece_rows=0 if pc is None else pc.data_ptr())
+        self._pc_written = (pc is not None) and (getattr(self, "_pc_written", False) or slot0 == 0)
         self._lm_written = (lm is not None) and (getattr(self, "_lm_written", False) or slot0 == 0)
         if lazy:
             self._states_stale = True
diff --git a/pytorch-a2c_amd/csrc/conv.hip b/pytorch-a2c_amd/csrc/conv.hip
--- a/pytorch-a2c_amd/csrc/conv.hip
+++ b/pytorch-a2c_amd/csrc/conv.hip
@@ -2558,10 +2558,12 @@
 constexpr int C2_0 = P0 + 3 * PQ, CQ = 4096, X2_0 = C2_0 + 3 * CQ;
 constexpr int A_0 = X2_0 + 3 * CQ, AQ = 6656, AROW = 208;
 constexpr int ZERO = A_0 + 3 * AQ, LDS_BYTES = ZERO + 32;
+constexpr int P1_0 = LDS_BYTES, LDS_BYTES_PC = P1_0 + 3 * PQ, SCR_BYTES_PC = 16384, PC_ROW = 3 * PQ;
 }
 struct WgradX6P {
   const float* in; long in_bs; const float* dout; float* slab; int B;
   const float* dl; long ldl; int nlog; const float* Wc; const unsigned char* a2b; long a2b_row;
+  const unsigned char* pc; long pc_bs;
 };
 __device__ __forceinline__ void wx_split2(float a, float b, unsigned int o[3]) {
   const __bf16 a0 = (__bf16)a, b0 = (__bf16)b;
@@ -2573,19 +2575,20 @@
   o[1] = (unsigned int)__builtin_bit_cast(unsigned short, a1) | ((unsigned int)__builtin_bit_cast(unsigned short, b1) << 16);
   o[2] = (unsigned int)__builtin_bit_cast(unsigned short, a2) | ((unsigned int)__builtin_bit_cast(unsigned short, b2) << 16);
 }
-template <bool RANK>
+template <bool RANK, bool PIECES = false>
 __global__ __launch_bounds__(wx::NT) void wgrad_x6_kernel(WgradX6P p) {
   using namespace wx;
   typedef const void __attribute__((address_space(1)))* gptr_t;
   typedef void __attribute__((address_space(3)))* lptr_t;
-  __shared__ __attribute__((aligned(16))) unsigned char scrw[SCR_BYTES];
+  constexpr int SDO = PIECES ? 0 : SCR_DO;
+  __shared__ __attribute__((aligned(16))) unsigned char scrw[PIECES ? SCR_BYTES_PC : SCR_BYTES];
   extern __shared__ __attribute__((aligned(16))) unsigned char ldsw[];
   const int tid = threadIdx.x, lane = tid & 63, w = tid >> 6;
   const int l16 = lane & 15, g = lane >> 4;
   const int wq = w & 3, th = w >> 2;
   const float* __restrict__ sa1 = reinterpret_cast<const float*>(scrw + SCR_A1);
-  const float* __restrict__ sdo = reinterpret_cast<const float*>(scrw + SCR_DO);
-  for (int i = tid; i < LDS_BYTES / 16; i += NT) *reinterpret_cast<u32x4x*>(ldsw + i * 16) = (u32x4x){0u, 0u, 0u, 0u};
+  const float* __restrict__ sdo = reinterpret_cast<const float*>(scrw + SDO);
+  for (int i = tid + (PIECES ? C2_0 / 16 : 0); i < LDS_BYTES / 16; i += NT) *reinterpret_cast<u32x4x*>(ldsw + i * 16) = (u32x4x){0u, 0u, 0u, 0u};
   int b0[2], b2[2], t0[2], t2[2], ncol[2];
   const int qs2 = g == 0 ? PQ : (g == 3 ? 0 : CQ);
 #pragma unroll
@@ -2606,19 +2609,28 @@
     for (int tt = 0; tt < 2; ++tt) acc[mt][tt] = acs[mt][tt] = (f32x4){0.f, 0.f, 0.f, 0.f};
   float dbacc = 0.f;
   const int bco = tid & 31, bpart = tid >> 5;
-  auto dma = [&](long b) {
+  auto dma = [&](long b, int pset) {
     const float* __restrict__ ga = p.in + b * p.in_bs;
     const float* __restrict__ gd = p.dout + b * 2592L;
-#pragma unroll
-    for (int i = 0; i < 4; ++i) {
-      if (i < 3 || w == 0)
-        __builtin_amdgcn_global_load_lds((gptr_t)(ga + (long)(i * NT + tid) * 4), (lptr_t)(scrw + SCR_A1 + (i * NT + w * 64) * 16), 16, 0, 0);
+    if (PIECES) {
+      const unsigned char* __restrict__ gp = p.pc + b * p.pc_bs;
+#pragma unroll
+      for (int i = 0; i < 6; ++i) {
+        if (i < 5 || w < 5)
+          __builtin_amdgcn_global_load_lds((gptr_t)(gp + (long)(i * NT + tid) * 16), (lptr_t)(ldsw + pset + (i * NT + w * 64) * 16), 16, 0, 0);
+      }
+    } else {
+#pragma unroll
+      for (int i = 0; i < 4; ++i) {
+        if (i < 3 || w == 0)
+          __builtin_amdgcn_global_load_lds((gptr_t)(ga + (long)(i * NT + tid) * 4), (lptr_t)(scrw + SCR_A1 + (i * NT + w * 64) * 16), 16, 0, 0);
+      }
     }
     if (!RANK) {
 #pragma unroll
       for (int i = 0; i < 2; ++i) {
         const int c = min(i * NT + tid, 647);
-        __builtin_amdgcn_global_load_lds((gptr_t)(gd + (long)c * 4), (lptr_t)(scrw + SCR_DO + (i * NT + w * 64) * 16), 16, 0, 0);
+        __builtin_amdgcn_global_load_lds((gptr_t)(gd + (long)c * 4), (lptr_t)(scrw + SDO + (i * NT + w * 64) * 16), 16, 0, 0);
       }
     }
   };
@@ -2637,7 +2649,7 @@
     for (int j = 0; j < 6; ++j) mbv[RANK ? j : 0] = p.a2b[bn * p.a2b_row + (min(tid + 512 * j, 2591) >> 3)];
   };
   auto form = [&]() {
-    float* __restrict__ dst = reinterpret_cast<float*>(scrw + SCR_DO);
+    float* __restrict__ dst = reinterpret_cast<float*>(scrw + SDO);
 #pragma unroll
     for (int j = 0; j < 6; ++j) {
       const int e = tid + 512 * j;
@@ -2667,11 +2679,28 @@
     form();
     raw(b + gridDim.x < p.B ? b + gridDim.x : b);
   }
-  if (b < p.B) dma(b);
+  int pc = P0;
+  if (b < p.B) dma(b, pc);
   for (; b < p.B; b += gridDim.x) {
     asm volatile("s_waitcnt vmcnt(0)" ::: "memory");
     __syncthreads();
-    {
+    if (PIECES) {
+      if (tid < 384) {
+        const int q = tid >> 7, r = tid & 127, ci = r >> 3, ky = (r >> 1) & 3, kxl = r & 1;
+        const unsigned char* __restrict__ src = ldsw + pc + q * PQ + (ci * 20 + ky) * PBLK + 32 + 4 * kxl;
+        unsigned int t[9];
+#pragma unroll
+        for (int j = 0; j < 9; ++j) t[j] = *reinterpret_cast<const unsigned int*>(src + 2 * j * PBLK);
+        const int n = ci * 16 + ky * 4 + kxl;
+        *reinterpret_cast<u32x4x*>(ldsw + C2_0 + q * CQ + n * 16) =
+            (u32x4x){(t[0] & 0xffffu) | (t[1] << 16), (t[2] & 0xffffu) | (t[3] << 16), (t[4] & 0xffffu) | (t[5] << 16), (t[6] & 0xffffu) | (t[7] << 16)};
+        *reinterpret_cast<u32x4x*>(ldsw + C2_0 + q * CQ + (n + 2) * 16) =
+            (u32x4x){(t[0] >> 16) | (t[1] & 0xffff0000u), (t[2] >> 16) | (t[3] & 0xffff0000u), (t[4] >> 16) | (t[5] & 0xffff0000u),
+                     (t[6] >> 16) | (t[7] & 0xffff0000u)};
+        *reinterpret_cast<unsigned int*>(ldsw + X2_0 + q * CQ + n * 16) = t[8] & 0xffffu;
+        *reinterpret_cast<unsigned int*>(ldsw + X2_0 + q * CQ + (n + 2) * 16) = t[8] >> 16;
+      }
+    } else {
       half_row(tid);
       if (tid < 128) half_row(512 + tid);
       if (tid >= 256) {
@@ -2714,7 +2743,8 @@
       const long b2 = b + 2L * gridDim.x;
       raw(b2 < p.B ? b2 : b);
     }
-    if (b + gridDim.x < p.B) dma(b + gridDim.x);
+    if (b + gridDim.x < p.B) dma(b + gridDim.x, pc ^ P1_0);
+    const int pcg = g == 0 ? pc : 0;
 #pragma unroll
     for (int s = 0; s < 3; ++s) {
       bf16x8x a[2][3], bf[2][3];
@@ -2727,8 +2757,8 @@
           asm volatile("ds_read_b128 %0, %1" : "=v"(ra[mt][q]) : "v"((unsigned)(unsigned long)(lptr_t)(ldsw + aaddr + mt * 16 * AROW + s * 64 + q * AQ)));
 #pragma unroll
       for (int tt = 0; tt < 2; ++tt) {
-        const int base = s == 0 ? b0[tt] : s == 1 ? b0[tt] + 8 * PBLK : b2[tt];
-        const int tail = s == 0 ? t0[tt] : s == 1 ? t0[tt] + 8 * PBLK : t2[tt];
+        const int base = (s == 0 ? b0[tt] : s == 1 ? b0[tt] + 8 * PBLK : b2[tt]) + (PIECES ? (s < 2 ? pc : pcg) : 0);
+        const int tail = (s == 0 ? t0[tt] : s == 1 ? t0[tt] + 8 * PBLK : t2[tt]) + (PIECES ? (s < 2 ? pc : pcg) : 0);
         const int qs = s == 2 ? qs2 : PQ;
 #pragma unroll
         for (int q = 0; q < 3; ++q) {
@@ -2760,6 +2790,7 @@
       WX_MM(acs, 2, 0) WX_MM(acs, 1, 1) WX_MM(acs, 0, 2) WX_MM(acs, 1, 0) WX_MM(acs, 0, 1) WX_MM(acc, 0, 0)
 #undef WX_MM
     }
+    if (PIECES) pc ^= P1_0;
   }
   float* sl = p.slab + (long)blockIdx.x * (32 * 256 + 32);
 #pragma unroll
@@ -4243,9 +4274,45 @@
   WgradX6P xp;
   xp.in = in; xp.in_bs = (long)in_bstride; xp.dout = nullptr; xp.slab = (float*)ws; xp.B = B;
   xp.dl = dl; xp.ldl = (long)ld_dl; xp.nlog = n_logits; xp.Wc = Wc; xp.a2b = maskbits; xp.a2b_row = (long)mask_row_bytes;
+  xp.pc = nullptr; xp.pc_bs = 0;
   hipLaunchKernelGGL(wgrad_x6_kernel<true>, dim3(grid), dim3(wx::NT), wx::LDS_BYTES, st, xp);
   A2C_CHECK_LAUNCH();
   const long nWx = 32L * 256, perx = nWx + 32;
+  hipLaunchKernelGGL(wgrad_reduce_kernel, dim3(a2c_grid_1d(perx, 256)), dim3(256), 0, st, (const float*)ws, grid, perx, nWx, dW, db);
+  A2C_CHECK_LAUNCH();
+  return A2C_OK;
+}
+
+int a2c_conv2d_bwd_weight_rank_pieces(const a2c_conv_desc* d, const float* in, int64_t in_bstride, const uint8_t* pieces,
+                                      int64_t pieces_bstride, const float* dl, int64_t ld_dl, int n_logits, const float* Wc,
+                                      const uint8_t* maskbits, int64_t mask_row_bytes, float* dW, float* db, int B, void* ws,
+                                      size_t ws_bytes, a2c_stream_t stream) {
+  if (!desc_ok(d) || B < 1 || (!in && !pieces) || !dl || !Wc || !maskbits || !dW || !db) return A2C_ERR_ARG;
+  if (!(d->Cin == 16 && d->Cout == 32 && d->H == 20 && d->W == 20 && d->ks == 4 && d->stride == 2 && d->pad == 0) || n_logits < 1 ||
+      n_logits > 4 || ld_dl < n_logits || mask_row_bytes < 324)
+    return A2C_ERR_ARG;
+  if (pieces && (((uintptr_t)pieces % 16) || pieces_bstride % 16 || pieces_bstride < wx::PC_ROW)) return A2C_ERR_ARG;
+  if (!pieces && (in_bstride % 4 || ((uintptr_t)in % 16) || in_bstride < 6400)) return A2C_ERR_ARG;
+  const long nWx = 32L * 256, perx = nWx + 32;
+  int grid = stream_grid() < B ? stream_grid() : B;
+  WgradPlan pl;
+  if (plan_wgrad(d, B, pl, true) && pl.run == 2 && pl.grid < grid) grid = pl.grid;
+  if (!ws || ws_bytes < (size_t)grid * perx * 4) return A2C_ERR_WORKSPACE;
+  hipStream_t st = a2c_s(stream);
+  static bool attrp = false;
+  if (!attrp) {
+    if (hipFuncSetAttribute((const void*)wgrad_x6_kernel<true, false>, hipFuncAttributeMaxDynamicSharedMemorySize, wx::LDS_BYTES) != hipSuccess ||
+        hipFuncSetAttribute((const void*)wgrad_x6_kernel<true, true>, hipFuncAttributeMaxDynamicSharedMemorySize, wx::LDS_BYTES_PC) != hipSuccess)
+      return A2C_ERR_LAUNCH;
+    attrp = true;
+  }
+  WgradX6P xp;
+  xp.in = in; xp.in_bs = (long)in_bstride; xp.dout = nullptr; xp.slab = (float*)ws; xp.B = B;
+  xp.dl = dl; xp.ldl = (long)ld_dl; xp.nlog = n_logits; xp.Wc = Wc; xp.a2b = maskbits; xp.a2b_row = (long)mask_row_bytes;
+  xp.pc = pieces; xp.pc_bs = (long)pieces_bstride;
+  if (pieces) hipLaunchKernelGGL((wgrad_x6_kernel<true, true>), dim3(grid), dim3(wx::NT), wx::LDS_BYTES_PC, st, xp);
+  else hipLaunchKernelGGL((wgrad_x6_kernel<true, false>), dim3(grid), dim3(wx::NT), wx::LDS_BYTES, st, xp);
+  A2C_CHECK_LAUNCH();
   hipLaunchKernelGGL(wgrad_reduce_kernel, dim3(a2c_grid_1d(perx, 256)), dim3(256), 0, st, (const float*)ws, grid, perx, nWx, dW, db);
   A2C_CHECK_LAUNCH();
   return A2C_OK;
@@ -4298,6 +4365,7 @@
       WgradX6P xp;
       xp.in = in; xp.in_bs = (long)in_bstride; xp.dout = dout; xp.slab = (float*)ws; xp.B = B;
       xp.dl = nullptr; xp.ldl = 0; xp.nlog = 0; xp.Wc = nullptr; xp.a2b = nullptr; xp.a2b_row = 0;
+      xp.pc = nullptr; xp.pc_bs = 0;
       hipLaunchKernelGGL(wgrad_x6_kernel<false>, dim3(grid), dim3(wx::NT), wx::LDS_BYTES, st, xp);
       A2C_CHECK_LAUNCH();
       const long nWx = 32L * 256, perx = nWx + 32;
diff --git a/pytorch-a2c_amd/csrc/step.hip b/pytorch-a2c_amd/csrc/step.hip
--- a/pytorch-a2c_amd/csrc/step.hip
+++ b/pytorch-a2c_amd/csrc/step.hip
@@ -38,6 +38,7 @@
   float* a2_rows;
   unsigned long long* a1_lm;
   unsigned char* a2_mb;
+  unsigned char* a1_pc;
   float* heads_rows; long heads_rows_ld;
   unsigned char* fstore; long fs_slot_stride;
   int* nvalid; int* nvalid_carry;
@@ -130,6 +131,16 @@
   return __builtin_bit_cast(bf16x8, r);
 }
 __device__ __forceinline__ unsigned short bf16_bits(float x) { return __builtin_bit_cast(unsigned short, (__bf16)x); }
+__device__ __forceinline__ void pc_split2(float a, float b, unsigned int o[3]) {
+  const __bf16 a0 = (__bf16)a, b0 = (__bf16)b;
+  const float ra = a - (float)a0, rb = b - (float)b0;
+  const __bf16 a1 = (__bf16)ra, b1 = (__bf16)rb;
+  const float sa = ra - (float)a1, sb = rb - (float)b1;
+  const __bf16 a2 = (__bf16)sa, b2 = (__bf16)sb;
+  o[0] = (unsigned int)__builtin_bit_cast(unsigned short, a0) | ((unsigned int)__builtin_bit_cast(unsigned short, b0) << 16);
+  o[1] = (unsigned int)__builtin_bit_cast(unsigned short, a1) | ((unsigned int)__builtin_bit_cast(unsigned short, b1) << 16);
+  o[2] = (unsigned int)__builtin_bit_cast(unsigned short, a2) | ((unsigned int)__builtin_bit_cast(unsigned short, b2) << 16);
+}
 
 template <bool OUT, bool U8, bool PERSIST, int HNT = HN>
 __global__ __launch_bounds__(NT) __attribute__((amdgpu_waves_per_eu(2, 2))) void a3c_step_kernel(StepP p) {
@@ -1109,6 +1120,33 @@
           }
         }
       }
+      if (p.x.a1_pc != nullptr && p.x.a1_rows != nullptr && t < T) {
+        unsigned char* __restrict__ pco = p.x.a1_pc + (row + t) * 46080L;
+        for (int q = sid; q < 960; q += sn) {
+          const int blk = q / 3, c = q - blk * 3, ch = blk / 20;
+          const float* __restrict__ src = a1 + ch * p.PLANE2 + (blk - ch * 20) * 20;
+          float e[8];
+          if (c < 2) {
+#pragma unroll
+            for (int m = 0; m < 4; ++m) {
+              const float4 v = *reinterpret_cast<const float4*>(src + 4 * m);
+              e[2 * m] = c ? v.y : v.x; e[2 * m + 1] = c ? v.w : v.z;
+            }
+          } else {
+            const float4 v = *reinterpret_cast<const float4*>(src + 16);
+            e[0] = v.x; e[1] = v.z; e[2] = v.y; e[3] = v.w; e[4] = e[5] = e[6] = e[7] = 0.f;
+          }
+          u32x4 o[3];
+#pragma unroll
+          for (int m = 0; m < 4; ++m) {
+            unsigned int s3[3];
+            pc_split2(e[2 * m], e[2 * m + 1], s3);
+            o[0][m] = s3[0]; o[1][m] = s3[1]; o[2][m] = s3[2];
+          }
+#pragma unroll
+          for (int k = 0; k < 3; ++k) __builtin_nontemporal_store(o[k], reinterpret_cast<u32x4*>(pco + k * 15360) + q);
+        }
+      }
       if (p.x.a2_rows != nullptr && t < T) {
         float* __restrict__ a2o = p.x.a2_rows + (row + t) * (long)p.F;
         unsigned char* __restrict__ mbo = (p.x.a2_mb != nullptr && (p.F & 7) == 0) ? p.x.a2_mb + (row + t) * (long)(p.F >> 3) : nullptr;
@@ -1298,6 +1336,7 @@
   p.x.a1_rows = r->a1_rows; p.x.a2_rows = r->a2_rows;
   p.x.a1_lm = (r->a1_rows != nullptr) ? (unsigned long long*)r->a1_lanemask_rows : nullptr;
   p.x.a2_mb = (r->a2_rows != nullptr) ? r->a2_maskbit_rows : nullptr;
+  p.x.a1_pc = (r->a1_rows != nullptr) ? r->a1_piece_rows : nullptr;
   p.x.heads_rows = r->heads_rows; p.x.heads_rows_ld = (long)r->heads_rows_ld;
   p.x.fstore = r->frame_store; p.x.fs_slot_stride = (long)r->frame_store_slot_stride;
   p.x.nvalid = r->nvalid_rows; p.x.nvalid_carry = r->nvalid_carry;
@@ -1328,6 +1367,7 @@
   if ((r->a1_rows || r->a2_rows) && ((p.OH1 * p.OW1) % 4 || (((uintptr_t)r->a1_rows | (uintptr_t)r->a2_rows) % 16))) return A2C_ERR_ARG;
   if (r->a1_lanemask_rows && (!r->a1_rows || ((uintptr_t)r->a1_lanemask_rows % 8) || (16 * p.OH1 * p.OW1) % 256)) return A2C_ERR_ARG;
   if (r->a2_maskbit_rows && (!r->a2_rows || p.F % 8)) return A2C_ERR_ARG;
+  if (r->a1_piece_rows && (!r->a1_rows || ((uintptr_t)r->a1_piece_rows % 16) || p.OH1 != 20 || p.OW1 != 20)) return A2C_ERR_ARG;
   if ((((uintptr_t)r->states | (uintptr_t)r->bookmark | (uintptr_t)r->frames | (uintptr_t)a.wfrag2 | (uintptr_t)a.Wc) % 16) ||
       (((uintptr_t)r->cmd | (uintptr_t)r->rec) % 8))
     return A2C_ERR_ARG;
@@ -1355,7 +1395,7 @@
     }
     return A2C_OK;
   }
-  if (p.x.states_lazy || p.x.a1_lm || p.x.a2_mb) return A2C_ERR_ARG;
+  if (p.x.states_lazy || p.x.a1_lm || p.x.a2_mb || p.x.a1_pc) return A2C_ERR_ARG;
   const size_t lds = step_lds(p);
   const int grid = a.B < cus ? a.B : cus;
   if (a.n_actions + 1 <= 4) hipLaunchKernelGGL((a3c_step_kernel<true, true, true, 4>), dim3(grid), dim3(NT), lds, a2c_s(stream), p);
diff --git a/pytorch-a2c_amd/csrc/torch_ops_abi.inc b/pytorch-a2c_amd/csrc/torch_ops_abi.inc
--- a/pytorch-a2c_amd/csrc/torch_ops_abi.inc
+++ b/pytorch-a2c_amd/csrc/torch_ops_abi.inc
@@ -289,6 +289,20 @@
   d0.OH = (int)ints[7];
   d0.OW = (int)ints[8];
   ok(a2c_conv2d_bwd_weight_rank(&d0, (const float *)abi_ptr(bufs, offs, 0, "a2c_conv2d_bwd_weight_rank"), (int64_t)ints[9], (const float *)abi_ptr(bufs, offs, 1, "a2c_conv2d_bwd_weight_rank"), (int64_t)ints[10], (int)ints[11], (const float *)abi_ptr(bufs, offs, 2, "a2c_conv2d_bwd_weight_rank"), (const uint8_t *)abi_ptr(bufs, offs, 3, "a2c_conv2d_bwd_weight_rank"), (int64_t)ints[12], (float *)abi_ptr(bufs, offs, 4, "a2c_conv2d_bwd_weight_rank"), (float *)abi_ptr(bufs, offs, 5, "a2c_conv2d_bwd_weight_rank"), (int)ints[13], (void *)abi_ptr(bufs, offs, 6, "a2c_conv2d_bwd_weight_rank"), (size_t)ints[14], cur_stream()), "a2c_conv2d_bwd_weight_rank");
+}
+void abi_conv2d_bwd_weight_rank_pieces(at::TensorList bufs, at::IntArrayRef offs, at::IntArrayRef ints, at::ArrayRef<double> flts) {
+  abi_counts(bufs, offs, ints, flts, 8, 16, 0, "a2c_conv2d_bwd_weight_rank_pieces");
+  a2c_conv_desc d0;
+  d0.Cin = (int)ints[0];
+  d0.H = (int)ints[1];
+  d0.W = (int)ints[2];
+  d0.Cout = (int)ints[3];
+  d0.ks = (int)ints[4];
+  d0.stride = (int)ints[5];
+  d0.pad = (int)ints[6];
+  d0.OH = (int)ints[7];
+  d0.OW = (int)ints[8];
+  ok(a2c_conv2d_bwd_weight_rank_pieces(&d0, (const float *)abi_ptr(bufs, offs, 0, "a2c_conv2d_bwd_weight_rank_pieces"), (int64_t)ints[9], (const uint8_t *)abi_ptr(bufs, offs, 1, "a2c_conv2d_bwd_weight_rank_pieces"), (int64_t)ints[10], (const float *)abi_ptr(bufs, offs, 2, "a2c_conv2d_bwd_weight_rank_pieces"), (int64_t)ints[11], (int)ints[12], (const float *)abi_ptr(bufs, offs, 3, "a2c_conv2d_bwd_weight_rank_pieces"), (const uint8_t *)abi_ptr(bufs, offs, 4, "a2c_conv2d_bwd_weight_rank_pieces"), (int64_t)ints[13], (float *)abi_ptr(bufs, offs, 5, "a2c_conv2d_bwd_weight_rank_pieces"), (float *)abi_ptr(bufs, offs, 6, "a2c_conv2d_bwd_weight_rank_pieces"), (int)ints[14], (void *)abi_ptr(bufs, offs, 7, "a2c_conv2d_bwd_weight_rank_pieces"), (size_t)ints[15], cur_stream()), "a2c_conv2d_bwd_weight_rank_pieces");
 }
 void abi_conv2d_bwd_data_signs(at::TensorList bufs, at::IntArrayRef offs, at::IntArrayRef ints, at::ArrayRef<double> flts) {
   abi_counts(bufs, offs, ints, flts, 4, 11, 0, "a2c_conv2d_bwd_data_signs");
@@ -545,6 +559,7 @@
   m.def("abi_conv2d_bwd_data_lanemask(Tensor(a!)[] bufs, int[] offs, int[] ints, float[] floats) -> ()"); \
   m.def("abi_conv2d_bwd_data_lanemask_rank(Tensor(a!)[] bufs, int[] offs, int[] ints, float[] floats) -> ()"); \
   m.def("abi_conv2d_bwd_weight_rank(Tensor(a!)[] bufs, int[] offs, int[] ints, float[] floats) -> ()"); \
+  m.def("abi_conv2d_bwd_weight_rank_pieces(Tensor(a!)[] bufs, int[] offs, int[] ints, float[] floats) -> ()"); \
   m.def("abi_conv2d_bwd_data_signs(Tensor(a!)[] bufs, int[] offs, int[] ints, float[] floats) -> ()"); \
   m.def("abi_conv2d_bwd_data_w1_frames(Tensor(a!)[] bufs, int[] offs, int[] ints, float[] floats) -> ()"); \
   m.def("abi_conv2d_bwd_data_w1(Tensor(a!)[] bufs, int[] offs, int[] ints, float[] floats) -> ()"); \
@@ -629,6 +644,7 @@
   m.impl("abi_conv2d_bwd_data_lanemask", &abi_conv2d_bwd_data_lanemask); \
   m.impl("abi_conv2d_bwd_data_lanemask_rank", &abi_conv2d_bwd_data_lanemask_rank); \
   m.impl("abi_conv2d_bwd_weight_rank", &abi_conv2d_bwd_weight_rank); \
+  m.impl("abi_conv2d_bwd_weight_rank_pieces", &abi_conv2d_bwd_weight_rank_pieces); \
   m.impl("abi_conv2d_bwd_data_signs", &abi_conv2d_bwd_data_signs); \
   m.impl("abi_conv2d_bwd_data_w1_frames", &abi_conv2d_bwd_data_w1_frames); \
   m.impl("abi_conv2d_bwd_data_w1", &abi_conv2d_bwd_data_w1); \
```
